# Keluaa/Armon.jl

Measured on AMD Instinct MI355X. Metric: Mcells/sec per sweep (fp64), higher is better.
Workload: dtype f64; 1 GPU; Sod 16384x16384 fp64, GAD+minmod+euler_2nd, Sequential X,Y splitting, nghost 4, 1x1 tiles of 16384x16384 cells (strong scaling); arithmetic=tuned (shared 1-ulp reciprocals + FMA; within the reference's golden tolerance), cells_per_gpu=268435456, transport=single block, device=AMD GPU gfx950 (gfx950:sramecc+:xnack-, 256 CUs), halo_exchange_downgraded=False, full=False

## Files before the change

### armon.jl_amd/_lib.py

```python
import ctypes as C
import os

_HERE = os.path.dirname(os.path.abspath(__file__))
LIB_PATH = os.environ.get("ARMON_HIP_LIB") or os.path.join(_HERE, "libarmon_hip.so")

FIELDS = ("x", "y", "rho", "u", "v", "E", "p", "c", "g", "us", "ps",
          "work_1", "work_2", "work_3", "work_4", "mask")


class SolverException(Exception):

    def __init__(self, category, msg):
        super().__init__(f"{category}: {msg}")
        self.category = category
        self.msg = msg


def solver_error(category, msg):
    raise SolverException(category, msg)


class Range(C.Structure):
    _fields_ = [("col_start", C.c_int64), ("col_step", C.c_int64), ("col_len", C.c_int64),
                ("row_start", C.c_int64), ("row_len", C.c_int64)]
# ... 41 lines not shown


class ProfileBin(C.Structure):
    _fields_ = [("n", C.c_uint64), ("n_bad", C.c_uint64), ("sum", (C.c_int64 * 3) * 5),
                ("rho_min", C.c_uint64), ("rho_max", C.c_uint64), ("p_min", C.c_uint64), ("p_max", C.c_uint64),
                ("reserved", C.c_uint64 * 3)]


class ProfileSpec(C.Structure):
    _fields_ = [("kind", C.c_int32), ("eos", C.c_int32), ("nbins", C.c_int64), ("width", C.c_int64),
                ("cx", C.c_double), ("cy", C.c_double), ("dx", C.c_double), ("dy", C.c_double), ("inv_dr", C.c_double),
                ("gamma", C.c_double), ("scale_exp", C.c_int32 * 5)]


class ExactSpec(C.Structure):
    _fields_ = [("form", C.c_int32), ("coord", C.c_int32), ("samples", C.c_int32), ("eos", C.c_int32), ("global_nx", C.c_int64),
                ("cx", C.c_double), ("cy", C.c_double), ("dx", C.c_double), ("dy", C.c_double), ("gamma", C.c_double),
                ("coord_min", C.c_double), ("coord_max", C.c_double), ("scale_exp", (C.c_int32 * 2) * 4),
                ("time", C.c_double), ("side", (C.c_double * 4) * 2), ("star", C.c_double * 4), ("speed", C.c_double * 5),
                ("g1", C.c_double), ("g2", C.c_double * 2), ("g3", C.c_double),
                ("inv_scale", C.c_double), ("M", C.c_int64), ("outer", C.c_double * 3), ("table", C.c_void_p)]


class ExactNorm(C.Structure):
    _fields_ = [("n", C.c_uint64), ("n_bad", C.c_uint64), ("sum_d", C.c_int64 * 3), ("sum_abs", C.c_int64 * 3),
                ("sum_sq", C.c_int64 * 3), ("max_abs", C.c_uint64), ("max_abs_at", C.c_uint64), ("reserved", C.c_uint64 * 3)]


class HistoryRecord(C.Structure):
    _fields_ = [("n", C.c_uint64), ("n_bad", C.c_uint64), ("sum", (C.c_int64 * 3) * 6), ("ext", (C.c_uint64 * 2) * 8),
                ("reserved", C.c_uint64 * 4)]


class HistorySpec(C.Structure):
    _fields_ = [("eos", C.c_int32), ("reserved", C.c_int32), ("gamma", C.c_double), ("global_nx", C.c_int64),
                ("scale_exp", C.c_int32 * 6)]


class DeriveSpec(C.Structure):
    _fields_ = [("nq", C.c_int32), ("quantity", C.c_int32 * 8), ("reduce", C.c_int32 * 8), ("eos", C.c_int32),
                ("neighbours", C.c_int32), ("gamma", C.c_double), ("dx", C.c_double), ("dy", C.c_double)]


class Region(C.Structure):
    _fields_ = [("kind", C.c_int32), ("reserved", C.c_int32), ("a", C.c_double * 4),
                ("rho", C.c_double), ("u", C.c_double), ("v", C.c_double), ("E", C.c_double)]


class RegionF32(C.Structure):
    _fields_ = [("kind", C.c_int32), ("reserved", C.c_int32), ("a", C.c_float * 4),
                ("rho", C.c_float), ("u", C.c_float), ("v", C.c_float), ("E", C.c_float)]


class HaloDesc(C.Structure):
    _fields_ = [("nx", C.c_int64), ("ny", C.c_int64), ("nghost", C.c_int32), ("nvars", C.c_int32),
                ("vars", C.c_void_p * 8)]


class CyclePlan(C.Structure):
    _fields_ = [("n_sweeps", C.c_int32), ("emit_p", C.c_int32), ("emit_dt", C.c_int32), ("overlap", C.c_int32),
                ("axis", C.c_int32 * 4), ("dt", C.c_double * 4), ("next_axis", C.c_int32), ("event_slot", C.c_int32),
                ("event_ctx", C.c_void_p), ("dt_host", C.c_void_p), ("dt_event_slot", C.c_int32), ("reserved", C.c_int32)]


class TileCycle(C.Structure):
    _fields_ = [("x", SweepDesc), ("y", SweepDesc)]


MGPU_ID_BYTES = 256

_lib = None

_dp, _i64, _dbl, _ci, _vp = C.c_void_p, C.c_int64, C.c_double, C.c_int, C.c_void_p
SIGNATURES = {
    "armon_hip_flt_size": (_ci, []),
    "armon_hip_idx_size": (_ci, []),
    "armon_hip_version": (C.c_char_p, []),
    "armon_hip_last_error": (C.c_char_p, []),
    "armon_hip_device_count": (_ci, [C.POINTER(_ci)]),
    "armon_hip_init": (_ci, [_ci, _vp, C.POINTER(_vp)]),
    "armon_hip_destroy": (_ci, [_vp]),
    "armon_hip_sync": (_ci, [_vp]),
    "armon_hip_device_memory_info": (_ci, [_vp, C.POINTER(C.c_size_t), C.POINTER(C.c_size_t)]),
    "armon_hip_device_name": (_ci, [_vp, C.c_char_p, C.c_size_t]),
    "armon_hip_stream": (_vp, [_vp]),
    "armon_hip_set_tuning": (_ci, [_vp, C.c_char_p, _ci]),
    "armon_hip_get_tuning": (_ci, [_vp, C.c_char_p, C.POINTER(_ci)]),
    "armon_hip_malloc": (_ci, [_vp, C.c_size_t, C.POINTER(_vp)]),
    "armon_hip_free": (_ci, [_vp, _vp]),
    "armon_hip_memcpy": (_ci, [_vp, _vp, _vp, C.c_size_t, _ci]),
    "armon_hip_memset": (_ci, [_vp, _vp, _ci, C.c_size_t]),
    "armon_hip_malloc_host": (_ci, [_vp, C.c_size_t, C.POINTER(_vp)]),
    "armon_hip_free_host": (_ci, [_vp, _vp]),
    "armon_hip_memcpy_async": (_ci, [_vp, _vp, _vp, C.c_size_t, _ci]),
    "armon_hip_event_sync": (_ci, [_vp, _ci]),
    "armon_hip_stream_copy4": (_ci, [_vp, C.POINTER(_vp * 4), C.POINTER(_vp * 4), C.c_size_t]),
    "armon_hip_timer_start": (_ci, [_vp]),
    "armon_hip_timer_stop": (_ci, [_vp, C.POINTER(_dbl)]),
    "armon_hip_event_record": (_ci, [_vp, _ci]),
    "armon_hip_event_elapsed_ms": (_ci, [_vp, _ci, _ci, C.POINTER(_dbl)]),
    "armon_hip_perfect_gas_EOS": (_ci, [_vp, Range, _dbl] + [_dp] * 7),
    "armon_hip_bizarrium_EOS": (_ci, [_vp, Range] + [_dp] * 7),
    "armon_hip_acoustic": (_ci, [_vp, Range, _i64] + [_dp] * 6),
    "armon_hip_acoustic_GAD": (_ci, [_vp, Range, _i64, _dbl, _dbl] + [_dp] * 6 + [_ci]),
    "armon_hip_cell_update": (_ci, [_vp, Range, _i64, _dbl, _dbl] + [_dp] * 5),
    "armon_hip_advection_first_order": (_ci, [_vp, Range, _i64, _dbl] + [_dp] * 9),
    "armon_hip_advection_second_order": (_ci, [_vp, Range, _i64, _dbl, _dbl] + [_dp] * 9),
    "armon_hip_euler_projection": (_ci, [_vp, Range, _i64, _dbl, _dbl] + [_dp] * 9),
    "armon_hip_boundary_conditions": (_ci, [_vp, Range, _i64, _ci, _dbl, _dbl] + [_dp] * 7),
    "armon_hip_pack_to_array": (_ci, [_vp, Range, _ci, _i64, _dp, _ci, C.POINTER(_dp)]),
    "armon_hip_unpack_from_array": (_ci, [_vp, Range, _ci, _i64, _dp, _ci, C.POINTER(_dp)]),
    "armon_hip_dtCFL_async": (_ci, [_vp, Range, _dbl, _dbl] + [_dp] * 4),
    "armon_hip_dtCFL": (_ci, [_vp, Range, _dbl, _dbl] + [_dp] * 3 + [C.POINTER(_dbl)]),
    "armon_hip_conservation_vars": (_ci, [_vp, Range, _dbl, _dp, _dp, C.POINTER(_dbl * 2)]),
    "armon_hip_init_test": (_ci, [_vp, Range, _ci, _i64, _i64, _ci, C.POINTER(_i64 * 2),
                                  C.POINTER(_i64 * 2), C.POINTER(_dbl * 2), C.POINTER(_dbl * 2),
                                  _dbl, C.POINTER(BlockDataPtrs)]),
    "armon_hip_init_regions": (_ci, [_vp, Range, _i64, _ci, C.POINTER(_i64 * 2), C.POINTER(_dbl * 2), C.POINTER(_dbl * 2), _ci,
                                     C.POINTER(_dbl * 4), _ci, C.POINTER(Region)] + [_dp] * 4),
    "armon_hip_init_regions_f32": (_ci, [_vp, Range, _i64, _ci, C.POINTER(_i64 * 2), C.POINTER(C.c_float * 2),
                                         C.POINTER(C.c_float * 2), _ci, C.POINTER(C.c_float * 4), _ci, C.POINTER(RegionF32)]
                                   + [_dp] * 4),
    "armon_hip_coarsen": (_ci, [_vp, _i64, _ci] + [_i64] * 4 + [_dp] * 6),
    "armon_hip_derive": (_ci, [_vp, _i64, _ci] + [_i64] * 4 + [_dp] * 4 + [C.POINTER(DeriveSpec), _dp]),
    "armon_hip_gather_strided": (_ci, [_vp, _i64, _ci, C.POINTER(_dp), _i64, _i64, _i64, _dp]),
    "armon_hip_state_pack": (_ci, [_vp, _i64, _ci, _i64, _i64, _ci, C.POINTER(_dp)] + [_i64] * 6 + [_dp, _dp]),
    "armon_hip_state_unpack": (_ci, [_vp, _i64, _ci, _i64, _i64, _ci, C.POINTER(_dp)] + [_i64] * 6 + [_dp, _dp]),
    "armon_hip_plane_encode_bound": (C.c_uint64, [_ci, _i64, _i64]),
    "armon_hip_plane_encode": (_ci, [_vp, _dp, _ci, _i64, _i64, _dp, C.c_uint64, _dp]),
    "armon_hip_plane_decode": (_ci, [_vp, _dp, C.c_uint64] + [_i64] * 6 + [_dp, _dp]),
    "armon_hip_state_diff_reset": (_ci, [_vp, _ci, _dp]),
    "armon_hip_state_compare": (_ci, [_vp, _i64, _ci, _i64, _i64, _ci, C.POINTER(_dp)] + [_i64] * 6 + [_dp, _dbl, _dbl, _dp, _dp]),
    "armon_hip_profile_reset": (_ci, [_vp, _i64, _dp]),
    "armon_hip_profile": (_ci, [_vp, _i64, _ci, _i64, _i64] + [_dp] * 4 + [_i64] * 6 + [C.POINTER(ProfileSpec), _dp]),
    "armon_hip_profile_bounds": (_ci, [_vp, _i64, _ci, _i64, _i64] + [_dp] * 4 + [_i64] * 6 + [C.POINTER(ProfileSpec), _dp]),
    "armon_hip_exact_norms_reset": (_ci, [_vp, _dp]),
    "armon_hip_exact_norms": (_ci, [_vp, _i64, _ci, _i64, _i64] + [_dp] * 4 + [_i64] * 6 + [C.POINTER(ExactSpec), _dp]),
    "armon_hip_exact_fill": (_ci, [_vp, _i64, _ci, _i64, _i64] + [_dp] * 4 + [_i64] * 6 + [C.POINTER(ExactSpec)]),
    "armon_hip_history_create": (_ci, [_vp, _ci, _ci, C.POINTER(_vp)]),
    "armon_hip_history_destroy": (_ci, [_vp, _vp]),
    "armon_hip_history_set_gauges": (_ci, [_vp, _vp, C.POINTER(_i64), _ci]),
    "armon_hip_history_sample": (_ci, [_vp, _vp, _ci, C.POINTER(HistorySpec), _i64, _ci, _i64, _i64] + [_dp] * 4 + [_i64] * 6),
    "armon_hip_history_read": (_ci, [_vp, _vp, _ci, _ci, _dp, _dp]),
    "armon_hip_sweep": (_ci, [_vp, C.POINTER(SweepDesc)]),
    "armon_hip_dt_state_step": (_ci, [_vp, _vp, _vp, _dbl, _dbl, _i64, _ci, _dbl]),
    "armon_hip_dt_state_step_f32": (_ci, [_vp, _vp, _vp, _dbl, _dbl, _i64, _ci, _dbl]),
    "armon_hip_graph_begin": (_ci, [_vp]),
    "armon_hip_graph_end": (_ci, [_vp, C.POINTER(_vp)]),
    "armon_hip_graph_launch": (_ci, [_vp, _vp]),
    "armon_hip_graph_destroy": (_ci, [_vp]),
    "armon_hip_tune_placement": (_ci, [_vp, C.POINTER(SweepDesc), C.POINTER(SweepDesc), C.POINTER(_vp), _ci,
                                       C.c_size_t, _ci, C.POINTER(_ci * 8), C.POINTER(_dbl)]),
    "armon_hip_cycle_xy": (_ci, [_vp, C.POINTER(SweepDesc), C.POINTER(SweepDesc)]),
    "armon_hip_choose_placement": (_ci, [_vp, C.POINTER(SweepDesc), C.POINTER(SweepDesc), C.POINTER(_vp), _ci,
                                         C.c_size_t, _ci, _dbl, C.POINTER(_ci * 8), C.POINTER(_dbl), C.POINTER(_ci)]),
    "armon_hip_mgpu_init": (_ci, [_ci, _ci, C.POINTER(_ci), C.POINTER(_vp)]),
    "armon_hip_mgpu_unique_id": (_ci, [_vp]),
    "armon_hip_mgpu_init_rank": (_ci, [_ci, _ci, _ci, _ci, _vp, _vp, C.POINTER(_vp)]),
    "armon_hip_mgpu_prepare_rank": (_ci, [_ci, _ci, _ci, _ci, _vp, C.POINTER(_vp)]),
    "armon_hip_mgpu_connect": (_ci, [_vp, _vp]),
    "armon_hip_mgpu_destroy": (_ci, [_vp]),
    "armon_hip_mgpu_set_periodic": (_ci, [_vp, _ci, _ci]),
    "armon_hip_mgpu_force_peer_copy": (_ci, [_vp, _ci]),
    "armon_hip_mgpu_set_chaos": (_ci, [_vp, C.c_uint, C.c_uint64]),
    "armon_hip_mgpu_n_local": (_ci, [_vp]),
    "armon_hip_mgpu_ctx": (_vp, [_vp, _ci]),
    "armon_hip_mgpu_tile_info": (_ci, [_vp, _ci, C.POINTER(_ci), C.POINTER(_ci * 2), C.POINTER(_ci * 4)]),
    "armon_hip_halo_exchange_start": (_ci, [_vp, _ci, C.POINTER(HaloDesc)]),
    "armon_hip_halo_exchange_finish": (_ci, [_vp, _ci, C.POINTER(HaloDesc)]),
    "armon_hip_halo_exchange": (_ci, [_vp, _ci, C.POINTER(HaloDesc)]),
    "armon_hip_dt_allreduce": (_ci, [_vp, C.POINTER(_vp)]),
    "armon_hip_mgpu_edge_ctx": (_vp, [_vp, _ci]),
    "armon_hip_mgpu_edge_dt": (_vp, [_vp, _ci]),
    "armon_hip_halo_exchange_finish_edge": (_ci, [_vp, _ci, C.POINTER(HaloDesc)]),
    "armon_hip_mgpu_edge_join": (_ci, [_vp, C.POINTER(_vp)]),
    "armon_hip_mgpu_allreduce_host": (_ci, [_vp, _ci, _ci, C.POINTER(_dbl)]),
    "armon_hip_mgpu_cycle": (_ci, [_vp, C.POINTER(CyclePlan), C.POINTER(TileCycle)]),
    "armon_hip_mgpu_drain": (_ci, [_vp, C.POINTER(TileCycle)]),
    "armon_hip_mgpu_set_threads": (_ci, [_vp, _ci]),
    "armon_hip_mgpu_sync": (_ci, [_vp]),
    "armon_hip_halo_ranges": (_ci, [_i64, _i64, _ci, _ci, C.POINTER(Range), C.POINTER(Range), C.POINTER(_i64)]),
}


def _add_f32_signatures():
    flt = C.c_float
    for name in ("perfect_gas_EOS", "bizarrium_EOS", "acoustic", "acoustic_GAD", "cell_update",
                 "advection_first_order", "advection_second_order", "euler_projection", "boundary_conditions",
                 "pack_to_array", "unpack_from_array", "dtCFL_async", "dtCFL", "conservation_vars", "init_test",
                 "coarsen", "gather_strided", "state_pack", "state_unpack", "plane_encode", "plane_decode"):
        res, args = SIGNATURES["armon_hip_" + name]
        conv = []
        for a in args:
            if a is _dbl:
                conv.append(flt)
            elif a is C.POINTER(_dbl):
                conv.append(C.POINTER(flt))
            elif a is C.POINTER(_dbl * 2):
                conv.append(C.POINTER(flt * 2))
            else:
                conv.append(a)
        SIGNATURES["armon_hip_" + name + "_f32"] = (res, conv)
    for name in ("halo_exchange_start", "halo_exchange_finish", "halo_exchange", "dt_allreduce",
                 "halo_exchange_finish_edge", "mgpu_edge_join", "mgpu_cycle", "mgpu_drain"):
        SIGNATURES["armon_hip_" + name + "_f32"] = SIGNATURES["armon_hip_" + name]
    SIGNATURES["armon_hip_sweep_f32"] = SIGNATURES["armon_hip_sweep"]
    SIGNATURES["armon_hip_state_compare_f32"] = SIGNATURES["armon_hip_state_compare"]
    SIGNATURES["armon_hip_derive_f32"] = SIGNATURES["armon_hip_derive"]
    SIGNATURES["armon_hip_profile_f32"] = SIGNATURES["armon_hip_profile"]
    SIGNATURES["armon_hip_profile_bounds_f32"] = SIGNATURES["armon_hip_profile_bounds"]
    SIGNATURES["armon_hip_exact_norms_f32"] = SIGNATURES["armon_hip_exact_norms"]
    SIGNATURES["armon_hip_exact_fill_f32"] = SIGNATURES["armon_hip_exact_fill"]
    SIGNATURES["armon_hip_history_sample_f32"] = SIGNATURES["armon_hip_history_sample"]
    SIGNATURES["armon_hip_tune_placement_f32"] = SIGNATURES["armon_hip_tune_placement"]
    SIGNATURES["armon_hip_choose_placement_f32"] = SIGNATURES["armon_hip_choose_placement"]


_add_f32_signatures()


def load_at(path):
    if not os.path.exists(path):
        raise RuntimeError(
            f"{path} is missing: build it with `python armon.jl_amd/build.py` "
            "(there is no CPU fallback for the device backend)")
    L = C.CDLL(path)
    for name, (res, args) in SIGNATURES.items():
        fn = getattr(L, name)
        fn.restype = res
        fn.argtypes = args
    if L.armon_hip_flt_size() != 8 or L.armon_hip_idx_size() != 8:
        raise RuntimeError("libarmon_hip.so: unexpected flt_size/idx_size")
    return L


def lib():
    global _lib
    if _lib is None:
        _lib = load_at(LIB_PATH)
    return _lib


ALT_LIB_PATH = os.path.join(_HERE, "libarmon_hip_alt.so")
_alt = None


class alt_kernels:

    def __enter__(self):
        global _lib, _alt
        if _alt is None:
            _alt = load_at(ALT_LIB_PATH)
        self._saved, _lib = _lib, _alt
        return _alt

    def __exit__(self, *exc):
        global _lib
        _lib = self._saved
        return False


def check(rc):
    if rc != 0:
        msg = lib().armon_hip_last_error().decode(errors="replace")
        raise SolverException("cpp" if rc != 4 else "time", f"[{rc}] {msg}")
```

### armon.jl_amd/blocking.py

```python
from dataclasses import dataclass
from enum import IntEnum

from ._lib import Range


class Axis(IntEnum):
    X = 1
    Y = 2


class Side(IntEnum):
    Left = 1
    Right = 2
    Bottom = 3
    Top = 4


def first_sides():
    return (Side.Left, Side.Bottom)


def first_side(axis):
    return Side.Left if axis == Axis.X else Side.Bottom


def last_side(axis):
    return Side.Right if axis == Axis.X else Side.Top


def sides_along(axis):
    return (first_side(axis), last_side(axis))


def axis_of(side):
    return Axis.X if side in (Side.Left, Side.Right) else Axis.Y


def opposite_of(side):
    return {Side.Left: Side.Right, Side.Right: Side.Left, Side.Bottom: Side.Top, Side.Top: Side.Bottom}[side]


@dataclass(frozen=True)
class StepRange:
    first: int
    step: int
    last: int

    def __len__(self):
        if self.step > 0:
            return max(0, (self.last - self.first) // self.step + 1)
        return max(0, (self.first - self.last) // (-self.step) + 1)

    def __iter__(self):
        return iter(range(self.first, self.last + (1 if self.step > 0 else -1), self.step))

    @property
    def stop(self):
        n = len(self)
        return self.first + (n - 1) * self.step if n else self.first - self.step

    def shift(self, n=1):
        return StepRange(self.first + self.step * n, self.step, self.last + self.step * n)

    def expand(self, n=1):
        return StepRange(self.first, self.step, self.last + self.step * n)

    def prepend(self, n=1):
        return StepRange(self.first - self.step * n, self.step, self.last)

    def inflate(self, n=1):
        return StepRange(self.first - self.step * n, self.step, self.last + self.step * n)


@dataclass(frozen=True)
class DomainRange:
    col: StepRange
    row: StepRange

    def __len__(self):
        return len(self.col) * len(self.row)

    @property
    def size(self):
        return (len(self.row), len(self.col))

    def first(self):
        return self.col.first + self.row.first - 1

    def last(self):
        return self.col.stop + self.row.stop - 1

    def __contains__(self, x):
        if not (self.first() <= x <= self.last()):
            return False
        ix = x - self.col.first + 1
        idc = ix // self.col.step
        ix -= idc * self.col.step
        return self.row.first <= ix <= self.row.stop

    def __iter__(self):
        for j in self.col:
            for i in self.row:
                yield j + i - 1

    def _along(self, axis, fname, n):
        if axis == Axis.X:
            return DomainRange(self.col, getattr(self.row, fname)(n))
        return DomainRange(getattr(self.col, fname)(n), self.row)

    def shift_dir(self, axis, n=1):
        return self._along(axis, "shift", n)

    def prepend_dir(self, axis, n=1):
        return self._along(axis, "prepend", n)

    def expand_dir(self, axis, n=1):
        return self._along(axis, "expand", n)

    def inflate_dir(self, axis, n=1):
        return self._along(axis, "inflate", n)

    def to_c(self):
        assert self.row.step == 1
        return Range(self.col.first - 1, self.col.step, len(self.col), self.row.first - 1, len(self.row))


@dataclass(frozen=True)
class BlockSize:
    size: tuple
    ghosts: int

    @property
    def real_size(self):
        return (self.size[0] - 2 * self.ghosts, self.size[1] - 2 * self.ghosts)

    @property
    def n_cells(self):
        return self.size[0] * self.size[1]

    def domain_range(self, bottom_left=(0, 0), top_right=(0, 0)):
        g, row = self.ghosts, self.size[0]
        block_start = row * (g - 1) + g

        def block_idx(I):
            return block_start + I[1] * row + I[0]

        first_I = (bottom_left[0] + 1, bottom_left[1] + 1)
        last_I = (top_right[0] + self.real_size[0], top_right[1] + self.real_size[1])
        col = StepRange(block_idx(first_I), row, block_idx(last_I))
        rowr = StepRange(1, 1, last_I[0] - first_I[0] + 1)
        return DomainRange(col, rowr)

    def position(self, i):
        iy, ix = divmod(i - 1, self.size[0])
        return (ix - self.ghosts + 1, iy - self.ghosts + 1)

    def lin_position(self, I):
        return (I[1] + self.ghosts - 1) * self.size[0] + (I[0] + self.ghosts)

    def is_ghost(self, i, o=0):
        I = self.position(i)
        rs = self.real_size
        return not all(1 - o <= I[d] <= rs[d] + o for d in range(2))

    def border_domain(self, side, single_strip=True):
        rs = self.real_size
        if side == Side.Left:
            bl, tr = (0, 0), (1 - rs[0], 0)
        elif side == Side.Right:
            bl, tr = (rs[0] - 1, 0), (0, 0)
        elif side == Side.Bottom:
            bl, tr = (0, 0), (0, 1 - rs[1])
        else:
            bl, tr = (0, rs[1] - 1), (0, 0)
        domain = self.domain_range(bl, tr)
        if single_strip:
            return domain
        if side in first_sides():
            return domain.expand_dir(axis_of(side), self.ghosts - 1)
        return domain.prepend_dir(axis_of(side), self.ghosts - 1)

    def ghost_domain(self, side, single_strip=True):
        domain = self.border_domain(side)
        domain = domain.shift_dir(axis_of(side), -self.ghosts if side in first_sides() else self.ghosts)
        if single_strip:
            return domain
        if side in first_sides():
            return domain.expand_dir(axis_of(side), self.ghosts - 1)
        return domain.prepend_dir(axis_of(side), self.ghosts - 1)

    def stride_along(self, axis):
        return 1 if axis == Axis.X else self.size[0]

    def size_along(self, axis_or_side):
        ax = axis_or_side if isinstance(axis_or_side, Axis) else axis_of(axis_or_side)
        return self.size[int(ax) - 1]

    def real_size_along(self, axis_or_side):
        ax = axis_or_side if isinstance(axis_or_side, Axis) else axis_of(axis_or_side)
        return self.real_size[int(ax) - 1]

    def real_face_size(self, axis_or_side):
        rs = self.real_size
        return (rs[0] * rs[1]) // self.real_size_along(axis_or_side)


@dataclass(frozen=True)
class StepsRanges:
    direction: Axis
    real_domain: tuple
    full_domain: tuple
    EOS: tuple
    fluxes: tuple
    cell_update: tuple
    advection: tuple
    projection: tuple


def compute_steps_ranges(axis, ghosts, projection_stencil_width):
    extra = projection_stencil_width
    real = ((0, 0), (0, 0))
    full = ((-ghosts, -ghosts), (ghosts, ghosts))
    if axis == Axis.X:
        fl = ((-extra, 0), (extra + 1, 0))
        cu = ((-extra, 0), (extra, 0))
        ad = ((0, 0), (1, 0))
    else:
        fl = ((0, -extra), (0, extra + 1))
        cu = ((0, -extra), (0, extra))
        ad = ((0, 0), (0, 1))
    return StepsRanges(axis, real, full, real, fl, cu, ad, real)
```

### armon.jl_amd/csrc/common.hpp

```cpp
#pragma once

#include <hip/hip_runtime.h>

#include <cstdarg>
#include <cstdint>
#include <cstdio>
#include <cstring>

#include "../../include/armon_hip.h"

struct armon_graph;
struct armon_ctx {
    int device = 0;
    hipStream_t stream = nullptr;
    bool owns_stream = false;
    double* partials = nullptr;
    size_t partials_cap = 0;
    double* scalars = nullptr;
    double* host_scalars = nullptr;
    hipEvent_t ev_start = nullptr, ev_stop = nullptr;
    hipEvent_t* ev_pool = nullptr;
    int n_cu = 256;
    int tune_xs_niter = 0;
    int tune_y_seg = 0;
    int tune_align = 1;
    int tune_y_cols1 = 0;
    int tune_x_xcd = -1;
    int tune_x_rows = 0;
    int tune_copy_nt = 0;
    int tune_y_sx = 0;
    int tune_profile_wgs = 0;
    int64_t seg_nx = -1, seg_ny = -1;
    int seg_lag = -1, seg_cols = -1, seg_value = 0;
    int live_graphs = 0;
    armon_graph* graphs = nullptr;
    bool capturing = false;
};

namespace armon {

void set_error(const char* fmt, ...);

inline int fail_hip(hipError_t e, const char* what)
{
    set_error("%s: %s", what, hipGetErrorString(e));
    return ARMON_ERR_HIP;
}

#define ARMON_HIP_TRY(expr)                                             \
    do {                                                                \
        hipError_t e_ = (expr);                                         \
        if (e_ != hipSuccess) return ::armon::fail_hip(e_, #expr);      \
    } while (0)

#define ARMON_REQUIRE(cond, ...)                                        \
    do {                                                                \
        if (!(cond)) {                                                  \
            ::armon::set_error(__VA_ARGS__);                            \
            return ARMON_ERR_INVALID_ARG;                               \
        }                                                               \
    } while (0)

inline int check_launch(const char* name)
{
    hipError_t e = hipGetLastError();
    if (e != hipSuccess) {
        set_error("launch of %s failed: %s", name, hipGetErrorString(e));
        return ARMON_ERR_HIP;
    }
    return ARMON_OK;
}

inline bool range_ok(const armon_range& r)
{
    return r.col_len >= 0 && r.row_len >= 0 && r.col_start + r.row_start >= 0 && r.col_step >= 0;
}
inline bool range_empty(const armon_range& r) { return r.col_len == 0 || r.row_len == 0; }

constexpr int kBlock = 256;

inline void range_grid(const armon_range& r, int cells_per_thread, dim3& grid, dim3& block)
{
    block = dim3(kBlock, 1, 1);
    int64_t per_block = (int64_t)kBlock * cells_per_thread;
    int64_t gx = (r.row_len + 15 + per_block - 1) / per_block;
    int64_t gy = r.col_len < 65535 ? r.col_len : 65535;
    grid = dim3((unsigned)gx, (unsigned)gy, 1);
}

int ensure_partials(armon_ctx* ctx, size_t n);
template <typename T>
int pack_pair(armon_ctx* ctx, const armon_range r[2], int nghost, int64_t face, T* const array[2], int nvars, T* const* vars, bool pack);
void disown_graphs(armon_ctx* ctx);

}
```

### armon.jl_amd/csrc/context.hip

```cpp
#include "common.hpp"

#include <cstdlib>

namespace armon {

static thread_local char g_error[512] = "";

void set_error(const char* fmt, ...)
{
    va_list ap;
    va_start(ap, fmt);
    vsnprintf(g_error, sizeof(g_error), fmt, ap);
    va_end(ap);
}

int ensure_partials(armon_ctx* ctx, size_t n)
{
    if (n <= ctx->partials_cap) return ARMON_OK;
    ARMON_REQUIRE(!ctx->capturing, "the reduction scratch would have to grow (%zu -> %zu doubles) inside a stream capture: "
                  "run this launch once before armon_hip_graph_begin", ctx->partials_cap, n);
    ARMON_REQUIRE(ctx->live_graphs == 0, "the reduction scratch would have to grow (%zu -> %zu doubles) while %d captured graph(s) of "
                  "this context point into it: destroy them first, or run the larger launch before capturing",
                  ctx->partials_cap, n, ctx->live_graphs);
    ARMON_HIP_TRY(hipStreamSynchronize(ctx->stream));
    if (ctx->partials) ARMON_HIP_TRY(hipFree(ctx->partials));
    ctx->partials = nullptr;
    ctx->partials_cap = 0;
    ARMON_HIP_TRY(hipMalloc((void**)&ctx->partials, n * sizeof(double)));
    ctx->partials_cap = n;
    return ARMON_OK;
}

}

using namespace armon;

extern "C" {

int armon_hip_flt_size(void) { return (int)sizeof(double); }
int armon_hip_idx_size(void) { return (int)sizeof(int64_t); }
const char* armon_hip_version(void) { return "armon_hip 0.1.0 (gfx950)"; }
const char* armon_hip_last_error(void) { return g_error; }

int armon_hip_device_count(int* count)
{
    ARMON_REQUIRE(count, "count is NULL");
    hipError_t e = hipGetDeviceCount(count);
    if (e != hipSuccess) {
        *count = 0;
        return fail_hip(e, "hipGetDeviceCount");
    }
    return ARMON_OK;
}

int armon_hip_init(int device_id, void* stream, armon_ctx** out)
{
    ARMON_REQUIRE(out, "ctx out pointer is NULL");
    *out = nullptr;
    int n = 0;
    hipError_t e = hipGetDeviceCount(&n);
    if (e != hipSuccess || n == 0) {
        set_error("no HIP device available (%s)", e != hipSuccess ? hipGetErrorString(e) : "count = 0");
        return ARMON_ERR_NO_DEVICE;
    }
    ARMON_REQUIRE(device_id >= 0 && device_id < n, "device_id %d out of range [0,%d)", device_id, n);
    ARMON_HIP_TRY(hipSetDevice(device_id));

    hipDeviceProp_t prop;
    ARMON_HIP_TRY(hipGetDeviceProperties(&prop, device_id));
    if (strncmp(prop.gcnArchName, "gfx950", 6) != 0) {
        set_error("device %d is %s; this library holds gfx950 code objects only", device_id, prop.gcnArchName);
        return ARMON_ERR_NO_DEVICE;
    }

    armon_ctx* ctx = new armon_ctx();
    ctx->device = device_id;
    ctx->n_cu = prop.multiProcessorCount;
    if (stream) {
        ctx->stream = (hipStream_t)stream;
        ctx->owns_stream = false;
    } else {
        e = hipStreamCreateWithFlags(&ctx->stream, hipStreamNonBlocking);
        if (e != hipSuccess) { delete ctx; return fail_hip(e, "hipStreamCreate"); }
        ctx->owns_stream = true;
    }
    if ((e = hipMalloc((void**)&ctx->scalars, 16 * sizeof(double))) != hipSuccess ||
        (e = hipHostMalloc((void**)&ctx->host_scalars, 16 * sizeof(double), hipHostMallocDefault)) != hipSuccess ||
        (e = hipEventCreate(&ctx->ev_start)) != hipSuccess ||
        (e = hipEventCreate(&ctx->ev_stop)) != hipSuccess) {
        armon_hip_destroy(ctx);
        return fail_hip(e, "context allocation");
    }
    int rc = ensure_partials(ctx, 8192);
    if (rc != ARMON_OK) { armon_hip_destroy(ctx); return rc; }
    for (const char* knob : {"ARMON_XS_NITER", "ARMON_Y_SEG", "ARMON_SWEEP_ALIGN", "ARMON_Y_COLS1", "ARMON_X_XCD", "ARMON_X_ROWS", "ARMON_Y_SX", "ARMON_COPY_NT"}) {
        const char* v = getenv(knob);
        if (v && *v) (void)armon_hip_set_tuning(ctx, knob, atoi(v));
    }
    *out = ctx;
    return ARMON_OK;
}

int armon_hip_set_tuning(armon_ctx* ctx, const char* knob, int value)
{
    ARMON_REQUIRE(ctx && knob, "NULL argument");
    if (!strcmp(knob, "ARMON_XS_NITER")) ctx->tune_xs_niter = value > 0 ? value : 0;
    else if (!strcmp(knob, "ARMON_Y_SEG")) ctx->tune_y_seg = value > 0 ? value : 0;
    else if (!strcmp(knob, "ARMON_SWEEP_ALIGN")) ctx->tune_align = value < 0 ? 1 : (value != 0);
    else if (!strcmp(knob, "ARMON_Y_COLS1")) ctx->tune_y_cols1 = value > 0;
    else if (!strcmp(knob, "ARMON_X_XCD")) ctx->tune_x_xcd = value < 0 ? -1 : (value > 0);
    else if (!strcmp(knob, "ARMON_X_ROWS")) ctx->tune_x_rows = (value == 1 || value == 2) ? value : 0;
    else if (!strcmp(knob, "ARMON_Y_SX")) ctx->tune_y_sx = (value == 1 || value == 2) ? value : 0;
    else if (!strcmp(knob, "ARMON_COPY_NT")) ctx->tune_copy_nt = value & 3;
    else if (!strcmp(knob, "PROFILE_WGS")) ctx->tune_profile_wgs = value > 0 ? value : 0;
    else ARMON_REQUIRE(false, "unknown tuning knob '%s'", knob);
    return ARMON_OK;
}

int armon_hip_get_tuning(armon_ctx* ctx, const char* knob, int* value)
{
    ARMON_REQUIRE(ctx && knob && value, "NULL argument");
    if (!strcmp(knob, "ARMON_XS_NITER")) *value = ctx->tune_xs_niter;
    else if (!strcmp(knob, "ARMON_Y_SEG")) *value = ctx->tune_y_seg;
    else if (!strcmp(knob, "ARMON_SWEEP_ALIGN")) *value = ctx->tune_align;
    else if (!strcmp(knob, "ARMON_Y_COLS1")) *value = ctx->tune_y_cols1;
    else if (!strcmp(knob, "ARMON_X_XCD")) *value = ctx->tune_x_xcd;
    else if (!strcmp(knob, "ARMON_X_ROWS")) *value = ctx->tune_x_rows;
    else if (!strcmp(knob, "ARMON_Y_SX")) *value = ctx->tune_y_sx;
    else if (!strcmp(knob, "ARMON_COPY_NT")) *value = ctx->tune_copy_nt;
    else if (!strcmp(knob, "PROFILE_WGS")) *value = ctx->tune_profile_wgs;
    else if (!strcmp(knob, "Y_RUN_ROWS")) *value = ctx->tune_y_seg > 0 ? ctx->tune_y_seg : ctx->seg_value;
    else ARMON_REQUIRE(false, "unknown tuning knob '%s'", knob);
    return ARMON_OK;
}

int armon_hip_destroy(armon_ctx* ctx)
{
    if (!ctx) return ARMON_OK;
    (void)hipSetDevice(ctx->device);
    if (ctx->stream) (void)hipStreamSynchronize(ctx->stream);
    disown_graphs(ctx);
    if (ctx->partials) (void)hipFree(ctx->partials);
    if (ctx->scalars) (void)hipFree(ctx->scalars);
    if (ctx->host_scalars) (void)hipHostFree(ctx->host_scalars);
    if (ctx->ev_pool) {
        for (int i = 0; i < ARMON_HIP_MAX_EVENTS; i++)
            if (ctx->ev_pool[i]) (void)hipEventDestroy(ctx->ev_pool[i]);
        delete[] ctx->ev_pool;
    }
    if (ctx->ev_start) (void)hipEventDestroy(ctx->ev_start);
    if (ctx->ev_stop) (void)hipEventDestroy(ctx->ev_stop);
    if (ctx->owns_stream && ctx->stream) (void)hipStreamDestroy(ctx->stream);
    delete ctx;
    return ARMON_OK;
}

int armon_hip_sync(armon_ctx* ctx)
{
    ARMON_REQUIRE(ctx, "ctx is NULL");
    ARMON_HIP_TRY(hipStreamSynchronize(ctx->stream));
    return ARMON_OK;
}

void* armon_hip_stream(armon_ctx* ctx) { return ctx ? (void*)ctx->stream : nullptr; }

int armon_hip_device_memory_info(armon_ctx* ctx, size_t* free_bytes, size_t* total_bytes)
{
    ARMON_REQUIRE(ctx && free_bytes && total_bytes, "NULL argument");
    ARMON_HIP_TRY(hipSetDevice(ctx->device));
    ARMON_HIP_TRY(hipMemGetInfo(free_bytes, total_bytes));
    return ARMON_OK;
}

int armon_hip_device_name(armon_ctx* ctx, char* buf, size_t buf_len)
{
    ARMON_REQUIRE(ctx && buf && buf_len > 0, "NULL argument");
    hipDeviceProp_t prop;
    ARMON_HIP_TRY(hipGetDeviceProperties(&prop, ctx->device));
    snprintf(buf, buf_len, "%s (%s, %d CUs)", prop.name[0] ? prop.name : "AMD GPU gfx950", prop.gcnArchName, prop.multiProcessorCount);
    return ARMON_OK;
}

int armon_hip_malloc(armon_ctx* ctx, size_t bytes, void** ptr)
{
    ARMON_REQUIRE(ctx && ptr, "NULL argument");
    *ptr = nullptr;
    if (bytes == 0) return ARMON_OK;
    ARMON_HIP_TRY(hipSetDevice(ctx->device));
    ARMON_HIP_TRY(hipMalloc(ptr, bytes));
    return ARMON_OK;
}

int armon_hip_free(armon_ctx* ctx, void* ptr)
{
    ARMON_REQUIRE(ctx, "ctx is NULL");
    if (!ptr) return ARMON_OK;
    ARMON_HIP_TRY(hipStreamSynchronize(ctx->stream));
    ARMON_HIP_TRY(hipFree(ptr));
    return ARMON_OK;
}

int armon_hip_memcpy(armon_ctx* ctx, void* dst, const void* src, size_t bytes, int kind)
{
    ARMON_REQUIRE(ctx, "ctx is NULL");
    if (bytes == 0) return ARMON_OK;
    ARMON_REQUIRE(dst && src, "NULL pointer in memcpy");
    hipMemcpyKind k;
    switch (kind) {
    case ARMON_MEMCPY_H2D: k = hipMemcpyHostToDevice; break;
    case ARMON_MEMCPY_D2H: k = hipMemcpyDeviceToHost; break;
    case ARMON_MEMCPY_D2D: k = hipMemcpyDeviceToDevice; break;
    default: ARMON_REQUIRE(false, "unknown memcpy kind %d", kind);
    }
    ARMON_HIP_TRY(hipMemcpyAsync(dst, src, bytes, k, ctx->stream));
    if (k != hipMemcpyDeviceToDevice) ARMON_HIP_TRY(hipStreamSynchronize(ctx->stream));
    return ARMON_OK;
}

int armon_hip_malloc_host(armon_ctx* ctx, size_t bytes, void** ptr)
{
    ARMON_REQUIRE(ctx && ptr, "NULL argument");
    *ptr = nullptr;
    if (bytes == 0) return ARMON_OK;
    ARMON_HIP_TRY(hipHostMalloc(ptr, bytes, hipHostMallocDefault));
    return ARMON_OK;
}

int armon_hip_free_host(armon_ctx* ctx, void* ptr)
{
    ARMON_REQUIRE(ctx, "ctx is NULL");
    if (ptr) ARMON_HIP_TRY(hipHostFree(ptr));
    return ARMON_OK;
}

int armon_hip_memcpy_async(armon_ctx* ctx, void* dst, const void* src, size_t bytes, int kind)
{
    ARMON_REQUIRE(ctx, "ctx is NULL");
    if (bytes == 0) return ARMON_OK;
    ARMON_REQUIRE(dst && src, "NULL pointer in memcpy_async");
    hipMemcpyKind k;
    switch (kind) {
    case ARMON_MEMCPY_H2D: k = hipMemcpyHostToDevice; break;
    case ARMON_MEMCPY_D2H: k = hipMemcpyDeviceToHost; break;
    case ARMON_MEMCPY_D2D: k = hipMemcpyDeviceToDevice; break;
    default: ARMON_REQUIRE(false, "unknown memcpy kind %d", kind);
    }
    ARMON_HIP_TRY(hipMemcpyAsync(dst, src, bytes, k, ctx->stream));
    return ARMON_OK;
}

int armon_hip_memset(armon_ctx* ctx, void* dst, int byte_value, size_t bytes)
{
    ARMON_REQUIRE(ctx, "ctx is NULL");
    if (bytes == 0) return ARMON_OK;
    ARMON_REQUIRE(dst, "NULL pointer in memset");
    ARMON_HIP_TRY(hipMemsetAsync(dst, byte_value, bytes, ctx->stream));
    return ARMON_OK;
}

}

namespace {
struct copy4_args { const double2* in[4]; double2* out[4]; };

typedef double vdouble2 __attribute__((ext_vector_type(2)));
template <int NT>
__global__ void __launch_bounds__(256) k_stream_copy4(copy4_args p, size_t n2)
{
    const size_t i = (size_t)blockIdx.x * 256 + threadIdx.x;
    if (i >= n2) return;
    vdouble2 v[4];
#pragma unroll
    for (int k = 0; k < 4; k++) {
        const vdouble2* q = reinterpret_cast<const vdouble2*>(p.in[k] + i);
        v[k] = (NT & 1) ? __builtin_nontemporal_load(q) : *q;
    }
#pragma unroll
    for (int k = 0; k < 4; k++) {
        vdouble2* q = reinterpret_cast<vdouble2*>(p.out[k] + i);
        if (NT & 2) __builtin_nontemporal_store(v[k], q);
        else *q = v[k];
// ... 79 lines not shown
```

### armon.jl_amd/csrc/fused_sweep.hpp

```cpp
#pragma once
#include "sweep_device.hpp"
#include "sweep_y_kernel.hpp"
#include "sweep_x_kernel.hpp"

namespace {

#ifdef ARMON_ALT_KERNELS
#include "fused_sweep_alt_kernels.hpp"
#endif

struct y_shape {
    int cols = 1;
    int block = kYBlock;
    bool sx = false;
};
y_shape y_launch_shape(const armon_ctx* ctx, const ARMON_SWEEP_DESC* d)
{
    y_shape s;
    if (std::is_same<real, float>::value && !d->exact && d->nx % 2 == 0 && d->nghost % 2 == 0 && d->nx >= 2 && !ctx->tune_y_cols1)
        s.cols = 2;
    if (ctx->tune_align != 0 && ctx->tune_y_sx != 2 && !d->exact) {
        const uintptr_t outs = (uintptr_t)d->rho_out | (uintptr_t)d->u_out | (uintptr_t)d->v_out | (uintptr_t)d->E_out;
        const int64_t row_len = d->nx + 2 * (int64_t)d->nghost;
        s.sx = outs % 64 == 0 && ((row_len * (int64_t)sizeof(real)) % 64 != 0 || ctx->tune_y_sx == 1);
    }
    s.block = s.sx ? kYSxBlock : kYBlock;
    return s;
}

template <class PIPE, bool TRACK>
int launch(armon_ctx* ctx, const sweep_args& a, int axis, const y_shape& ys, int64_t* n_blocks)
{
    const int64_t n_out = a.o_hi - a.o_lo;
    if (axis == ARMON_AXIS_Y) {
        const int64_t per_block = (int64_t)ys.block * ys.cols;
        dim3 grid((unsigned)((a.nx + a.xshift + per_block - 1) / per_block), (unsigned)((n_out + a.seg - 1) / a.seg));
        *n_blocks = (int64_t)grid.x * grid.y;
        if constexpr (std::is_same<real, float>::value && !PIPE::kExact) {
            if (ys.cols == 2) {
                if (ys.sx)
                    hipLaunchKernelGGL((k_sweep_y<PIPE, TRACK, kYSxBlock, true, 2>), grid, dim3(ys.block), 0, ctx->stream, a);
                else
                    hipLaunchKernelGGL((k_sweep_y<PIPE, TRACK, kYBlock, false, 2>), grid, dim3(ys.block), 0, ctx->stream, a);
                return check_launch("sweep_y2");
            }
        }
        if constexpr (!PIPE::kExact) {
            if (ys.sx) {
                hipLaunchKernelGGL((k_sweep_y<PIPE, TRACK, kYSxBlock, true>), grid, dim3(ys.block), 0, ctx->stream, a);
                return check_launch("sweep_y (store exchange)");
            }
        }
        hipLaunchKernelGGL((k_sweep_y<PIPE, TRACK>), grid, dim3(ys.block), 0, ctx->stream, a);
        return check_launch("sweep_y");
    }
#if defined(ARMON_ALT_KERNELS) && !defined(ARMON_ONLY_HEADLINE)
    if (a.x_kernel == 2) {
        dim3 grid((unsigned)((n_out + a.seg - 1) / a.seg), (unsigned)((a.ny + kXRows - 1) / kXRows));
        *n_blocks = (int64_t)grid.x * grid.y;
        const size_t lds = (size_t)(a.emit ? 6 : 4) * kXRows * (kXChunk + 1) * sizeof(real);
        hipLaunchKernelGGL((k_sweep_x_lds<PIPE, kXChunk, TRACK>), grid, dim3(kXRows), lds, ctx->stream, a);
        return check_launch("sweep_x_lds");
    }
#endif
    int niter = 1;
#if defined(ARMON_ALT_KERNELS) && !defined(ARMON_ONLY_HEADLINE)
    if (ctx->tune_xs_niter > 1) niter = ctx->tune_xs_niter;
#elif defined(ARMON_XS_MULTI)
    niter = ctx->tune_xs_niter > 0 ? ctx->tune_xs_niter : 2;
#endif
    const bool k1 = a.x_kernel == 3;
    if (a.x_kernel == 0 && a.o_hi - a.o_lo <= 8) {
        const int64_t per_block = 16 - 2 * PIPE::LAG;
        dim3 grid((unsigned)((a.o_hi - a.x_first + per_block - 1) / per_block), (unsigned)((a.ny + 4 * kXSRows - 1) / (4 * kXSRows)));
        *n_blocks = (int64_t)grid.x * grid.y * kXSRows;
        sweep_args b = a;
        b.gx = (int32_t)grid.x;
        b.gy = (int32_t)grid.y;
        hipLaunchKernelGGL((k_sweep_x_dpp<PIPE::SCHEME, PIPE::LIM, PIPE::PROJ, PIPE::EOS, PIPE::kExact, 1, TRACK, true, 1>),
                           grid, dim3(64, kXSRows), 0, ctx->stream, b, 1);
        return check_launch("sweep_x_dpp (narrow)");
    }
    const int halo = k1 ? PIPE::LAG : 4;
    const int64_t per_block = (int64_t)niter * (64 * (k1 ? 1 : 2) - 2 * halo);
    const int64_t x_lowest = a.x_row_align ? a.o_lo - (64 / (int64_t)sizeof(real) - 1) : a.x_first;
    dim3 grid((unsigned)((a.o_hi - x_lowest + per_block - 1) / per_block), (unsigned)((a.ny + kXSRows - 1) / kXSRows));
    if (a.x_wg_along_x && !k1 && niter == 1)
        grid = dim3((unsigned)((a.o_hi - x_lowest + kXSRows * per_block - 1) / (kXSRows * per_block)), (unsigned)a.ny);
    *n_blocks = (int64_t)grid.x * grid.y * kXSRows;
    sweep_args b = a;
    b.gx = (int32_t)grid.x;
    b.gy = (int32_t)grid.y;
#if defined(ARMON_ALT_KERNELS) && !defined(ARMON_ONLY_HEADLINE)
    if (k1)
        hipLaunchKernelGGL((k_sweep_x_dpp<PIPE::SCHEME, PIPE::LIM, PIPE::PROJ, PIPE::EOS, PIPE::kExact, 1, TRACK, false>),
                           grid, dim3(64, kXSRows), 0, ctx->stream, b, niter);
    else if (niter > 1)
        hipLaunchKernelGGL((k_sweep_x_dpp<PIPE::SCHEME, PIPE::LIM, PIPE::PROJ, PIPE::EOS, PIPE::kExact, 2, TRACK, false>),
                           grid, dim3(64, kXSRows), 0, ctx->stream, b, niter);
    else
#endif
#ifdef ARMON_XS_MULTI
        hipLaunchKernelGGL((k_sweep_x_dpp<PIPE::SCHEME, PIPE::LIM, PIPE::PROJ, PIPE::EOS, PIPE::kExact, 2, TRACK, false>),
                           grid, dim3(64, kXSRows), 0, ctx->stream, b, niter);
#else
        hipLaunchKernelGGL((k_sweep_x_dpp<PIPE::SCHEME, PIPE::LIM, PIPE::PROJ, PIPE::EOS, PIPE::kExact, 2, TRACK, true>),
                           grid, dim3(64, kXSRows), 0, ctx->stream, b, niter);
#endif
    return check_launch("sweep_x_dpp");
}

int y_run_length(int n_cu, int64_t nx, int64_t ny, int lag, int cols_per_lane, int block)
{
    const double slots = (double)n_cu * ARMON_Y_WAVES * 4 / (block / 64);
    const int64_t cols = (nx + 16 + (int64_t)block * cols_per_lane - 1) / ((int64_t)block * cols_per_lane);
    int best = (int)(ny < 32 ? ny : 32);
    double best_cost = 1e300;
    for (int64_t nruns = 1; nruns <= ny; nruns++) {
        const int64_t seg = (ny + nruns - 1) / nruns;
        if (seg < 32) break;
        if ((ny + seg - 1) / seg != nruns) continue;
        const double rounds = (double)(cols * nruns) / slots;
        const bool full_single_round = rounds <= 1. && rounds >= 0.93;
        if (rounds < 2. && !full_single_round) continue;
        const double cost = (full_single_round ? 1. : 0.5 * (rounds + std::ceil(rounds))) * (double)(seg + 2 * lag);
        if (cost < best_cost) {
            best_cost = cost;
            best = (int)seg;
        }
    }
    return best;
}

int64_t max_blocks(const sweep_args& a)
{
    const int64_t by = (a.nx + 16 + kYBlock - 1) / kYBlock * ((a.ny + a.seg - 1) / a.seg);
#ifdef ARMON_ALT_KERNELS
    const int64_t bx_lds = (a.nx + a.seg - 1) / a.seg * ((a.ny + kXRows - 1) / kXRows);
#else
    const int64_t bx_lds = 0;
#endif
    const int64_t bx_dpp = ((a.nx + 8) / 56 + 1 + kXSRows) * ((a.ny + kXSRows - 1) / kXSRows) * kXSRows;
    int64_t m = by > bx_lds ? by : bx_lds;
    m = m > bx_dpp ? m : bx_dpp;
    return m + kFoldBlocks;
}

template <class PIPE>
int dispatch_track(armon_ctx* ctx, const sweep_args& a, int axis, const y_shape& ys, bool track, int64_t* n_blocks)
{
    if (track) return launch<PIPE, true>(ctx, a, axis, ys, n_blocks);
    return launch<PIPE, false>(ctx, a, axis, ys, n_blocks);
}

template <int SCHEME, int LIM, int PROJ, int EOS>
int dispatch_exact(armon_ctx* ctx, const sweep_args& a, int axis, const y_shape& ys, bool exact, bool track, int64_t* nb)
{
    if (exact) return dispatch_track<fused::Pipe<SCHEME, LIM, PROJ, EOS, real>>(ctx, a, axis, ys, track, nb);
    return dispatch_track<fused::PipeFast<SCHEME, LIM, PROJ, EOS, real>>(ctx, a, axis, ys, track, nb);
}

template <int SCHEME, int LIM, int PROJ>
int dispatch_eos(armon_ctx* ctx, const sweep_args& a, int axis, const y_shape& ys, int eos, bool exact, bool track, int64_t* nb)
{
    if (eos == ARMON_EOS_BIZARRIUM)
        return dispatch_exact<SCHEME, LIM, PROJ, ARMON_EOS_BIZARRIUM>(ctx, a, axis, ys, exact, track, nb);
    return dispatch_exact<SCHEME, LIM, PROJ, ARMON_EOS_PERFECT_GAS>(ctx, a, axis, ys, exact, track, nb);
}

template <int SCHEME, int LIM>
int dispatch_proj(armon_ctx* ctx, const sweep_args& a, int axis, const y_shape& ys, int eos, int proj, bool exact, bool track, int64_t* nb)
{
    if (proj == ARMON_PROJECTION_EULER_2ND)
        return dispatch_eos<SCHEME, LIM, ARMON_PROJECTION_EULER_2ND>(ctx, a, axis, ys, eos, exact, track, nb);
    return dispatch_eos<SCHEME, LIM, ARMON_PROJECTION_EULER>(ctx, a, axis, ys, eos, exact, track, nb);
}

}

extern "C" int ARMON_SWEEP_FN(armon_ctx* ctx, const ARMON_SWEEP_DESC* d)
{
    ARMON_REQUIRE(ctx && d, "NULL argument");
    ARMON_REQUIRE(d->axis == ARMON_AXIS_X || d->axis == ARMON_AXIS_Y, "invalid axis %d", d->axis);
    ARMON_REQUIRE(d->scheme == ARMON_SCHEME_GODUNOV || d->scheme == ARMON_SCHEME_GAD, "unknown scheme %d", d->scheme);
    ARMON_REQUIRE(d->projection == ARMON_PROJECTION_EULER || d->projection == ARMON_PROJECTION_EULER_2ND,
                  "unknown projection %d", d->projection);
    ARMON_REQUIRE(d->eos == ARMON_EOS_PERFECT_GAS || d->eos == ARMON_EOS_BIZARRIUM, "unknown EOS %d", d->eos);
    ARMON_REQUIRE(d->scheme != ARMON_SCHEME_GAD || (d->limiter >= ARMON_LIMITER_NONE && d->limiter <= ARMON_LIMITER_SUPERBEE),
                  "unknown limiter tag %d", d->limiter);
    ARMON_REQUIRE(d->nx > 0 && d->ny > 0, "empty block %lld x %lld", (long long)d->nx, (long long)d->ny);
    ARMON_REQUIRE(d->ny < (1ll << 30) && d->nx < (1ll << 30), "block too large (%lld x %lld)", (long long)d->nx, (long long)d->ny);
    const int lag = (d->scheme == ARMON_SCHEME_GAD ? 1 : 0) + (d->projection == ARMON_PROJECTION_EULER_2ND ? 1 : 0) + 2;
    ARMON_REQUIRE(d->nghost >= lag, "nghost = %d but this scheme/projection reads %d cells past the block", d->nghost, lag);
    const int64_t n_axis = d->axis == ARMON_AXIS_X ? d->nx : d->ny;
    ARMON_REQUIRE(!(d->bc_low || d->bc_high) || n_axis >= lag,
                  "mirror boundary needs at least %d cells along the sweep axis", lag);
    ARMON_REQUIRE(!d->bc_low || (std::fabs(d->u_factor_low) == 1. && std::fabs(d->v_factor_low) == 1.),
                  "mirror factors of the low side must be +1 or -1 (got %g, %g)", d->u_factor_low, d->v_factor_low);
    ARMON_REQUIRE(!d->bc_high || (std::fabs(d->u_factor_high) == 1. && std::fabs(d->v_factor_high) == 1.),
                  "mirror factors of the high side must be +1 or -1 (got %g, %g)", d->u_factor_high, d->v_factor_high);
    ARMON_REQUIRE(d->rho_in && d->u_in && d->v_in && d->E_in && d->rho_out && d->u_out && d->v_out && d->E_out,
                  "NULL state array");
    ARMON_REQUIRE(d->rho_in != d->rho_out && d->u_in != d->u_out && d->v_in != d->v_out && d->E_in != d->E_out,
                  "in and out arrays must not alias (ping-pong)");
#ifdef ARMON_ALT_KERNELS
    ARMON_REQUIRE(d->x_kernel == 0 || d->x_kernel == 2 || d->x_kernel == 3, "unknown x_kernel form %d", d->x_kernel);
#else
    ARMON_REQUIRE(d->x_kernel == 0, "x_kernel form %d is a measured alternative: only libarmon_hip_alt.so (-DARMON_ALT_KERNELS) carries it",
                  d->x_kernel);
#endif
    ARMON_REQUIRE(!d->dt_state || d->x_kernel == 0 || d->x_kernel == 3,
                  "dt_state is not honoured by x_kernel form %d (only the DPP X sweeps and the Y march read it)", d->x_kernel);
    const bool exact = d->exact != 0;
    const bool track = d->dt_cfl_out != nullptr;
    ARMON_REQUIRE(!track || (d->cfl_dx > 0 && d->cfl_dy > 0), "dt_cfl_out needs cfl_dx, cfl_dy > 0");

    sweep_args a;
    a.nx = d->nx;
    a.ny = d->ny;
    a.row_len = d->nx + 2 * (int64_t)d->nghost;
    a.g = d->nghost;
    a.bc_low = d->bc_low;
    a.bc_high = d->bc_high;
    a.emit = (d->p_out ? 1 : 0) | (d->c_out ? 2 : 0);
    a.dt = (real)d->dt;
    a.dx = (real)d->dx;
    a.gamma = (real)d->gamma;
    a.inv_dx = real(1) / a.dx;
    a.dt_dx = a.dt / a.dx;
    const bool X = d->axis == ARMON_AXIS_X;
    a.fa_low = (real)(X ? d->u_factor_low : d->v_factor_low);
    a.ft_low = (real)(X ? d->v_factor_low : d->u_factor_low);
    a.fa_high = (real)(X ? d->u_factor_high : d->v_factor_high);
    a.ft_high = (real)(X ? d->v_factor_high : d->u_factor_high);
    a.rho_in = d->rho_in;
    a.ua_in = X ? d->u_in : d->v_in;
    a.ut_in = X ? d->v_in : d->u_in;
    a.E_in = d->E_in;
    a.rho_out = d->rho_out;
    a.ua_out = X ? d->u_out : d->v_out;
    a.ut_out = X ? d->v_out : d->u_out;
    a.E_out = d->E_out;
    a.p_out = d->p_out;
    a.c_out = d->c_out;
    a.st = d->dt_state;
    const bool align = ctx->tune_align != 0;
    const y_shape ys = X ? y_shape{} : y_launch_shape(ctx, d);
    a.y_sx = ys.sx;
    if (X) {
        a.seg = 512;
    } else if (ctx->tune_y_seg > 0) {
        a.seg = ctx->tune_y_seg;
    } else {
        if (ctx->seg_nx != d->nx || ctx->seg_ny != n_axis || ctx->seg_lag != lag || ctx->seg_cols != ys.cols * ys.block) {
            ctx->seg_value = y_run_length(ctx->n_cu, d->nx, n_axis, lag, ys.cols, ys.block);
            ctx->seg_cols = ys.cols * ys.block;
            ctx->seg_nx = d->nx;
            ctx->seg_ny = n_axis;
            ctx->seg_lag = lag;
        }
        a.seg = ctx->seg_value;
    }
    ARMON_REQUIRE(X || a.row_len * (int64_t)sizeof(real) * (a.seg + 2 * lag + 16) < (1ll << 32),
                  "block too wide for 32-bit row offsets (%lld cells per row, runs of %d rows)", (long long)d->nx, a.seg);
    a.x_kernel = d->x_kernel;
    a.o_lo = 0;
    a.o_hi = n_axis;
    if (d->out_hi != 0) {
        ARMON_REQUIRE(d->out_lo >= 0 && d->out_lo < d->out_hi && d->out_hi <= n_axis,
                      "invalid partial sweep [%lld, %lld) of %lld cells", (long long)d->out_lo, (long long)d->out_hi, (long long)n_axis);
        a.o_lo = d->out_lo;
        a.o_hi = d->out_hi;
    }
    a.xshift = (X || !align) ? 0 : d->nghost % 16;
    a.x_first = X ? (align ? a.o_lo - (a.o_lo + d->nghost) % 8 : a.o_lo) : 0;
    const bool want_along_x = ctx->tune_x_rows == 2 || (ctx->tune_x_rows == 0 && sizeof(real) == 4);
    const bool along_x = X && want_along_x && d->ny <= 65535 && ctx->tune_x_xcd <= 0;
    const bool eight_xcds = ctx->n_cu == 256;
    a.xcd_remap = (ctx->tune_x_xcd < 0 ? sizeof(real) == 8 : ctx->tune_x_xcd != 0) && !along_x && eight_xcds;
    a.x_row_align = 0;
#ifndef ARMON_XS_MULTI
    {
        const uintptr_t bases = (uintptr_t)d->rho_in | (uintptr_t)d->u_in | (uintptr_t)d->v_in | (uintptr_t)d->E_in |
                                (uintptr_t)d->rho_out | (uintptr_t)d->u_out | (uintptr_t)d->v_out | (uintptr_t)d->E_out |
                                (uintptr_t)d->p_out | (uintptr_t)d->c_out;
        a.x_row_align = X && align && d->x_kernel == 0 && ctx->tune_xs_niter <= 1 && a.row_len % (64 / (int64_t)sizeof(real)) != 0 &&
                        bases % 64 == 0;
    }
#endif
    a.x_wg_along_x = along_x ? 1 : 0;
    a.partials = nullptr;
    if (track) {
        int rc = ensure_partials(ctx, (size_t)(2 * max_blocks(a)));
        if (rc != ARMON_OK) return rc;
        a.partials = reinterpret_cast<real*>(ctx->partials);
    }

    int64_t n_blocks = 0;
    int rc;
#ifdef ARMON_ONLY_HEADLINE
#ifndef ARMON_ONLY_EOS
#define ARMON_ONLY_EOS ARMON_EOS_PERFECT_GAS
#endif
    ARMON_REQUIRE(d->scheme == ARMON_SCHEME_GAD && d->limiter == ARMON_LIMITER_MINMOD && d->projection == ARMON_PROJECTION_EULER_2ND &&
                  d->eos == ARMON_ONLY_EOS && d->x_kernel == 0, "headline-only variant build");
    rc = dispatch_exact<ARMON_SCHEME_GAD, ARMON_LIMITER_MINMOD, ARMON_PROJECTION_EULER_2ND, ARMON_ONLY_EOS>(ctx, a, d->axis, ys, exact, track, &n_blocks);
    if (rc != ARMON_OK || !track) return rc;
    return fold_dt_launch(ctx, a.partials, n_blocks, (real)d->cfl_dx, (real)d->cfl_dy, d->dt_cfl_out, d->dt_accumulate, d->dt_state);
#else
    if (d->scheme == ARMON_SCHEME_GODUNOV) {
        rc = dispatch_proj<ARMON_SCHEME_GODUNOV, ARMON_LIMITER_NONE>(ctx, a, d->axis, ys, d->eos, d->projection, exact, track, &n_blocks);
    } else {
        switch (d->limiter) {
        case ARMON_LIMITER_MINMOD:
            rc = dispatch_proj<ARMON_SCHEME_GAD, ARMON_LIMITER_MINMOD>(ctx, a, d->axis, ys, d->eos, d->projection, exact, track, &n_blocks);
            break;
        case ARMON_LIMITER_SUPERBEE:
            rc = dispatch_proj<ARMON_SCHEME_GAD, ARMON_LIMITER_SUPERBEE>(ctx, a, d->axis, ys, d->eos, d->projection, exact, track, &n_blocks);
            break;
        default:
            rc = dispatch_proj<ARMON_SCHEME_GAD, ARMON_LIMITER_NONE>(ctx, a, d->axis, ys, d->eos, d->projection, exact, track, &n_blocks);
        }
    }
    if (rc != ARMON_OK || !track) return rc;
    return fold_dt_launch(ctx, a.partials, n_blocks, (real)d->cfl_dx, (real)d->cfl_dy, d->dt_cfl_out, d->dt_accumulate, d->dt_state);
#endif
}

#if defined(ARMON_CYCLE_FN) && !defined(ARMON_ALT_KERNELS)
extern "C" int ARMON_CYCLE_FN(armon_ctx* ctx, const ARMON_SWEEP_DESC* x, const ARMON_SWEEP_DESC* y)
{
    ARMON_REQUIRE(ctx && x && y, "NULL argument");
    ARMON_REQUIRE(false, "the whole-cycle kernel is a measured alternative (slower than the two sweeps, DESIGN.md section 4.2): "
                         "only libarmon_hip_alt.so (-DARMON_ALT_KERNELS) carries it");
    return ARMON_ERR_INVALID_ARG;
}
#endif
#if defined(ARMON_CYCLE_FN) && defined(ARMON_ALT_KERNELS)
#include "fused_sweep_alt_cycle.hpp"
#endif
```

### armon.jl_amd/csrc/fused_sweep_f64.hip

```cpp
#define ARMON_SWEEP_REAL double
#define ARMON_SWEEP_FN armon_hip_sweep
#define ARMON_SWEEP_DESC armon_sweep_desc
#define ARMON_CYCLE_FN armon_hip_cycle_xy
#include "fused_sweep.hpp"
```

### armon.jl_amd/csrc/placement.hip

```cpp
#include "common.hpp"

#include <cstdint>
#include <utility>
#include <vector>

using namespace armon;

namespace {

template <typename real>
__global__ void __launch_bounds__(256) k_fill_uniform(real* __restrict__ p, size_t n, real value)
{
    const size_t i = (size_t)blockIdx.x * 256 + threadIdx.x;
    if (i < n) p[i] = value;
}

template <class DESC, class SWEEP, class PREPARE, class STOP>
int placement_search(armon_ctx* ctx, SWEEP sweep, const DESC* x_desc, const DESC* y_desc, void* const* pool, int n_pool,
                     int tries, int* best, double* times_ms, int* tries_done, PREPARE prepare, STOP stop)
{
    hipEvent_t e0 = nullptr, e1 = nullptr;
    auto cleanup = [&]() {
        if (e0) (void)hipEventDestroy(e0);
        if (e1) (void)hipEventDestroy(e1);
    };
#define PLACEMENT_TRY(expr) do { hipError_t e_ = (expr); if (e_ != hipSuccess) { cleanup(); return fail_hip(e_, #expr); } } while (0)
    PLACEMENT_TRY(hipEventCreate(&e0));
    PLACEMENT_TRY(hipEventCreate(&e1));
    std::vector<int> idx(n_pool);
    std::vector<double> seen;
    double best_ms = 1e300;
    uint64_t rng = 0x9E3779B97F4A7C15ull;
    int t = 0;
    for (; t < tries; t++) {
        for (int k = 0; k < n_pool; k++) idx[k] = k;
        if (t > 0)
            for (int k = 0; k < 8; k++) {
                rng ^= rng << 13; rng ^= rng >> 7; rng ^= rng << 17;
                std::swap(idx[k], idx[k + (int)(rng % (uint64_t)(n_pool - k))]);
            }
        int rc = prepare(idx.data());
        if (rc != ARMON_OK) { cleanup(); return rc; }
        DESC dx = *x_desc, dy = *y_desc;
        using ptr_t = decltype(dx.rho_out);
        auto P = [&](int role) { return static_cast<ptr_t>(pool[idx[role]]); };
        dx.rho_in = P(0); dx.u_in = P(1); dx.v_in = P(2); dx.E_in = P(3);
        dx.rho_out = P(4); dx.u_out = P(5); dx.v_out = P(6); dx.E_out = P(7);
        dy.rho_in = P(4); dy.u_in = P(5); dy.v_in = P(6); dy.E_in = P(7);
        dy.rho_out = P(0); dy.u_out = P(1); dy.v_out = P(2); dy.E_out = P(3);
        double ms_min = 1e300;
        for (int rep = 0; rep < 3; rep++) {
            PLACEMENT_TRY(hipEventRecord(e0, ctx->stream));
            rc = sweep(ctx, &dx);
            if (rc == ARMON_OK) rc = sweep(ctx, &dy);
            if (rc != ARMON_OK) { cleanup(); return rc; }
            PLACEMENT_TRY(hipEventRecord(e1, ctx->stream));
            PLACEMENT_TRY(hipEventSynchronize(e1));
            float ms = 0.f;
            PLACEMENT_TRY(hipEventElapsedTime(&ms, e0, e1));
            if (rep > 0 && ms < ms_min) ms_min = ms;
        }
        if (times_ms) times_ms[t] = ms_min;
        seen.push_back(ms_min);
        if (ms_min < best_ms) {
            best_ms = ms_min;
            for (int k = 0; k < 8; k++) best[k] = idx[k];
        }
        if (stop(seen, best_ms)) { t++; break; }
    }
#undef PLACEMENT_TRY
    if (tries_done) *tries_done = t;
    cleanup();
    return ARMON_OK;
}

template <class DESC, class SWEEP>
int tune_placement(armon_ctx* ctx, SWEEP sweep, const DESC* x_desc, const DESC* y_desc, void* const* pool, int n_pool,
                   size_t bytes, int tries, int* picks, double* times_ms)
{
    ARMON_REQUIRE(ctx && x_desc && y_desc && pool && picks, "NULL argument");
    ARMON_REQUIRE(n_pool >= 8 && tries >= 1 && bytes > 0, "need at least 8 vectors and 1 try (n_pool = %d, tries = %d)", n_pool, tries);
    for (int k = 0; k < n_pool; k++) ARMON_REQUIRE(pool[k], "pool[%d] is NULL", k);
    void* master[4] = {nullptr, nullptr, nullptr, nullptr};
    bool parked = false;
    auto cleanup = [&]() {
        if (parked) {
            for (int k = 0; k < 4; k++)
                (void)hipMemcpyAsync(pool[k], master[k], bytes, hipMemcpyDeviceToDevice, ctx->stream);
            (void)hipStreamSynchronize(ctx->stream);
        }
        for (void* m : master)
            if (m) (void)hipFree(m);
    };
#define TUNE_TRY(expr) do { hipError_t e_ = (expr); if (e_ != hipSuccess) { cleanup(); return fail_hip(e_, #expr); } } while (0)
    for (int k = 0; k < 4; k++) {
        TUNE_TRY(hipMalloc(&master[k], bytes));
        TUNE_TRY(hipMemcpyAsync(master[k], pool[k], bytes, hipMemcpyDeviceToDevice, ctx->stream));
    }
    parked = true;
    auto copy_in = [&](const int* idx, const char* what) {
        for (int k = 0; k < 4; k++) {
            hipError_t e = hipMemcpyAsync(pool[idx[k]], master[k], bytes, hipMemcpyDeviceToDevice, ctx->stream);
            if (e != hipSuccess) return fail_hip(e, what);
        }
        return (int)ARMON_OK;
    };
    int best[8] = {};
    int rc = placement_search(ctx, sweep, x_desc, y_desc, pool, n_pool, tries, best, times_ms, nullptr,
                              [&](const int* idx) { return copy_in(idx, "hipMemcpyAsync(pool[idx[k]], master[k], bytes, hipMemcpyDeviceToDevice, ctx->stream)"); },
                              [](const std::vector<double>&, double) { return false; });
    if (rc == ARMON_OK) rc = copy_in(best, "hipMemcpyAsync(pool[best[k]], master[k], bytes, hipMemcpyDeviceToDevice, ctx->stream)");
    if (rc != ARMON_OK) { cleanup(); return rc; }
    TUNE_TRY(hipStreamSynchronize(ctx->stream));
#undef TUNE_TRY
    for (int k = 0; k < 8; k++) picks[k] = best[k];
    parked = false;
    cleanup();
    return ARMON_OK;
}

template <typename real, class DESC, class SWEEP>
int choose_placement(armon_ctx* ctx, SWEEP sweep, const DESC* x_desc, const DESC* y_desc, void* const* pool, int n_pool,
                     size_t bytes, int tries, double tolerance, int* picks, double* times_ms, int* tries_done)
{
    ARMON_REQUIRE(ctx && x_desc && y_desc && pool && picks, "NULL argument");
    ARMON_REQUIRE(n_pool >= 8 && tries >= 1 && bytes >= sizeof(real), "need at least 8 vectors and 1 try (n_pool = %d, tries = %d)", n_pool, tries);
    for (int k = 0; k < n_pool; k++) ARMON_REQUIRE(pool[k], "pool[%d] is NULL", k);
    const size_t n = bytes / sizeof(real);
    const real uniform[4] = {real(1), real(0), real(0), real(2.5)};
    auto fill = [&](const int* idx) {
        for (int k = 0; k < 4; k++)
            hipLaunchKernelGGL(k_fill_uniform<real>, dim3((unsigned)((n + 255) / 256)), dim3(256), 0, ctx->stream,
                               static_cast<real*>(pool[idx[k]]), n, uniform[k]);
        return (int)ARMON_OK;
    };
    auto plateau = [&](const std::vector<double>& seen, double best_ms) {
        int near = 0;
        double worst = 0;
        for (double v : seen) {
            near += v <= best_ms * (1. + tolerance);
            worst = v > worst ? v : worst;
        }
        return tolerance > 0 && seen.size() >= 12 && near >= 2 && best_ms <= 0.93 * worst;
    };
    int best[8] = {};
    int rc = placement_search(ctx, sweep, x_desc, y_desc, pool, n_pool, tries, best, times_ms, tries_done, fill, plateau);
    if (rc != ARMON_OK) return rc;
    for (int k = 0; k < 8; k++) picks[k] = best[k];
    return ARMON_OK;
}

}

extern "C" int armon_hip_tune_placement(armon_ctx* ctx, const armon_sweep_desc* x_desc, const armon_sweep_desc* y_desc,
                                        void* const* pool, int n_pool, size_t bytes, int tries, int* picks, double* times_ms)
{
    return tune_placement(ctx, armon_hip_sweep, x_desc, y_desc, pool, n_pool, bytes, tries, picks, times_ms);
}

extern "C" int armon_hip_tune_placement_f32(armon_ctx* ctx, const armon_sweep_desc_f32* x_desc, const armon_sweep_desc_f32* y_desc,
                                            void* const* pool, int n_pool, size_t bytes, int tries, int* picks, double* times_ms)
{
    return tune_placement(ctx, armon_hip_sweep_f32, x_desc, y_desc, pool, n_pool, bytes, tries, picks, times_ms);
}

extern "C" int armon_hip_choose_placement(armon_ctx* ctx, const armon_sweep_desc* x_desc, const armon_sweep_desc* y_desc,
                                          void* const* pool, int n_pool, size_t bytes, int tries, double tolerance, int* picks,
                                          double* times_ms, int* tries_done)
{
    return choose_placement<double>(ctx, armon_hip_sweep, x_desc, y_desc, pool, n_pool, bytes, tries, tolerance, picks, times_ms,
                                    tries_done);
}

extern "C" int armon_hip_choose_placement_f32(armon_ctx* ctx, const armon_sweep_desc_f32* x_desc, const armon_sweep_desc_f32* y_desc,
                                              void* const* pool, int n_pool, size_t bytes, int tries, double tolerance, int* picks,
                                              double* times_ms, int* tries_done)
{
    return choose_placement<float>(ctx, armon_hip_sweep_f32, x_desc, y_desc, pool, n_pool, bytes, tries, tolerance, picks,
                                   times_ms, tries_done);
}
```

### armon.jl_amd/csrc/sweep_device.hpp

```cpp
#pragma once
#include "common.hpp"
#include "dt_state.hpp"
#include "reduce.hpp"
#include "sweep_pipeline.hpp"
#include "sweep_spatial.hpp"

#include <cmath>
#include <cstdint>
#include <cstdlib>
#include <type_traits>
#include <utility>

using namespace armon;

#ifndef ARMON_SWEEP_REAL
#error "include through fused_sweep_f64.hip / fused_sweep_f32.hip"
#endif

namespace {

using real = ARMON_SWEEP_REAL;
using vec2 = std::conditional<std::is_same<real, double>::value, double2, float2>::type;

#ifdef ARMON_NT
#define ARMON_NT_X ARMON_NT
#define ARMON_NT_Y ARMON_NT
#endif
#ifndef ARMON_NT_X
#define ARMON_NT_X 3
#endif
#ifndef ARMON_NT_Y
#define ARMON_NT_Y 2
#endif
typedef real vreal2 __attribute__((ext_vector_type(2)));
template <bool NT = false>
__device__ __forceinline__ vec2 ld2(const real* p)
{
    const vreal2* q = reinterpret_cast<const vreal2*>(p);
    const vreal2 v = NT ? __builtin_nontemporal_load(q) : *q;
    return vec2{v.x, v.y};
}
constexpr bool x_nt_loads(int eos, bool exact)
{
    return (ARMON_NT_X & 1) && sizeof(real) == 8 && eos == ARMON_EOS_PERFECT_GAS && !exact;
}
__device__ __forceinline__ void st2(real* p, real x, real y)
{
    vreal2* q = reinterpret_cast<vreal2*>(p);
    const vreal2 v = {x, y};
    if (ARMON_NT_X & 2) __builtin_nontemporal_store(v, q);
    else *q = v;
}

struct sweep_args {
    int64_t nx, ny, row_len;
    int32_t g;
    int32_t bc_low, bc_high;
    int32_t emit;
    int32_t seg;
    int32_t x_kernel;
    int64_t o_lo, o_hi;
    int64_t x_first;
    int32_t xshift;
    int32_t xcd_remap;
    int32_t gx = 0, gy = 0;
    int32_t x_wg_along_x = 0;
    int32_t x_row_align = 0;
    int32_t y_sx = 0;
    armon_dt_state* st = nullptr;
    real dt, dx, gamma;
    real inv_dx, dt_dx;
    real fa_low, ft_low, fa_high, ft_high;
    const real *rho_in, *ua_in, *ut_in, *E_in;
    real *rho_out, *ua_out, *ut_out, *E_out;
    real *p_out, *c_out;
    real* partials;
    int32_t bc_low_t = 0, bc_high_t = 0;
    real tu_low = 1, tv_low = 1, tu_high = 1, tv_high = 1;
};

__device__ __forceinline__ int64_t bc_source(const sweep_args& a, int64_t n, int64_t j, real& fa, real& ft)
{
    fa = 1;
    ft = 1;
    if (j < 0 && a.bc_low) {
        fa = a.fa_low;
        ft = a.ft_low;
        return -1 - j;
    }
    if (j >= n && a.bc_high) {
        fa = a.fa_high;
        ft = a.ft_high;
        return 2 * n - 1 - j;
    }
    return j;
}

__device__ __forceinline__ bool sweep_begin(sweep_args& a)
{
    if (a.st) {
        const auto* st = (const __attribute__((address_space(4))) armon_dt_state*)a.st;
        if (st->done) return false;
        a.dt = (real)st->current_dt * a.dt;
        a.dt_dx = a.dt / a.dx;
        if (!st->emit_p) a.emit &= ~1;
    }
    return true;
}

template <int... Is, class F>
__device__ __forceinline__ void static_for(std::integer_sequence<int, Is...>, F&& f)
{
    (f(std::integral_constant<int, Is>{}), ...);
}

typedef unsigned int v2u __attribute__((ext_vector_type(2)));
using rsrc_t = __amdgpu_buffer_rsrc_t;

__device__ __forceinline__ rsrc_t make_rsrc(const void* p)
{
    return __builtin_amdgcn_make_buffer_rsrc(const_cast<void*>(p), 0, 0xFFFFFFFFu, 0x00020000);
}
#ifndef ARMON_Y_AUX_LD
#define ARMON_Y_AUX_LD ((ARMON_NT_Y & 1) ? 2 : 0)
#endif
#ifndef ARMON_Y_AUX_ST
#define ARMON_Y_AUX_ST ((ARMON_NT_Y & 2) ? 2 : 0)
#endif
constexpr int kAuxLoad = ARMON_Y_AUX_LD, kAuxStore = ARMON_Y_AUX_ST;
template <typename T> __device__ __forceinline__ T buf_load(rsrc_t r, unsigned voff, unsigned soff);
template <>
__device__ __forceinline__ double buf_load<double>(rsrc_t r, unsigned voff, unsigned soff)
{
    const v2u v = __builtin_amdgcn_raw_buffer_load_b64(r, voff, soff, kAuxLoad);
    return __builtin_bit_cast(double, v);
}
template <>
__device__ __forceinline__ float buf_load<float>(rsrc_t r, unsigned voff, unsigned soff)
{
    return __builtin_bit_cast(float, __builtin_amdgcn_raw_buffer_load_b32(r, voff, soff, kAuxLoad));
}
__device__ __forceinline__ float2 buf_load2(rsrc_t r, unsigned voff, unsigned soff)
{
    typedef float v2f __attribute__((ext_vector_type(2)));
    const v2f v = __builtin_bit_cast(v2f, __builtin_amdgcn_raw_buffer_load_b64(r, voff, soff, kAuxLoad));
    return float2{v.x, v.y};
}
__device__ __forceinline__ void buf_store2(rsrc_t r, unsigned voff, unsigned soff, float x, float y)
{
    const v2u v = {__builtin_bit_cast(unsigned int, x), __builtin_bit_cast(unsigned int, y)};
    __builtin_amdgcn_raw_buffer_store_b64(v, r, voff, soff, kAuxStore);
}
__device__ __forceinline__ void buf_store(rsrc_t r, unsigned voff, unsigned soff, double x)
{
    __builtin_amdgcn_raw_buffer_store_b64(__builtin_bit_cast(v2u, x), r, voff, soff, kAuxStore);
}
__device__ __forceinline__ void buf_store(rsrc_t r, unsigned voff, unsigned soff, float x)
{
    __builtin_amdgcn_raw_buffer_store_b32(__builtin_bit_cast(unsigned int, x), r, voff, soff, kAuxStore);
}

struct cfl_track {
    real au = 0, av = 0;
    __device__ __forceinline__ void add(real u, real v, real c)
    {
#ifdef ARMON_CFL_PLAIN_MAX
        au = phys::mx(au, phys::abs_(phys::mx(phys::abs_(u + c), phys::abs_(u - c))));
        av = phys::mx(av, phys::abs_(phys::mx(phys::abs_(v + c), phys::abs_(v - c))));
#else
#ifdef ARMON_CFL_TWO_SUMS
        au = phys::amax(au, phys::abs_(phys::mx(phys::abs_(u + c), phys::abs_(u - c))));
        av = phys::amax(av, phys::abs_(phys::mx(phys::abs_(v + c), phys::abs_(v - c))));
#else
        au = phys::amax(au, phys::abs_(u) + phys::abs_(c));
        av = phys::amax(av, phys::abs_(v) + phys::abs_(c));
#endif
#endif
    }
};

template <int NWAVES>
__device__ __forceinline__ void cfl_block_store(const cfl_track& t, real* partials, int64_t block, int tid)
{
    __shared__ real lds[NWAVES];
    const real au = red::block_reduce<red::op_max, NWAVES>(t.au, lds, tid);
    const real av = red::block_reduce<red::op_max, NWAVES>(t.av, lds, tid);
    if (tid == 0) {
        partials[2 * block] = au;
        partials[2 * block + 1] = av;
    }
}

constexpr int kFoldBlocks = 512;

__global__ void __launch_bounds__(256)
k_fold_pairs(const real* __restrict__ partials, int64_t n, real* __restrict__ out)
{
    __shared__ real lds[4];
    real au = 0, av = 0;
    for (int64_t k = (int64_t)blockIdx.x * blockDim.x + threadIdx.x; k < n; k += (int64_t)gridDim.x * blockDim.x) {
        const vec2 v = ld2(partials + 2 * k);
        au = phys::amax(au, v.x);
        av = phys::amax(av, v.y);
    }
    au = red::block_reduce<red::op_max, 4>(au, lds, threadIdx.x);
    av = red::block_reduce<red::op_max, 4>(av, lds, threadIdx.x);
    if (threadIdx.x == 0) {
        out[2 * blockIdx.x] = au;
        out[2 * blockIdx.x + 1] = av;
    }
}

__global__ void __launch_bounds__(256)
k_fold_dt(const real* __restrict__ partials, int64_t n_blocks, real dx, real dy, real* __restrict__ out,
          int accumulate, armon_dt_state* st = nullptr)
{
    if (st && st->done) return;
    __shared__ real lds[4];
    real au = 0, av = 0;
    for (int64_t k = threadIdx.x; k < n_blocks; k += blockDim.x) {
        au = phys::amax(au, partials[2 * k]);
        av = phys::amax(av, partials[2 * k + 1]);
    }
    au = red::block_reduce<red::op_max, 4>(au, lds, threadIdx.x);
    av = red::block_reduce<red::op_max, 4>(av, lds, threadIdx.x);
    if (threadIdx.x == 0) {
        const real dt = phys::mn_nan(dx / au, dy / av);
        out[0] = accumulate ? phys::mn_nan(out[0], dt) : dt;
        if (st && st->auto_step && !accumulate)
            dt_state_step<real>(st, dt, (real)st->cfl, (real)st->maxtime, st->maxcycle, st->cst_dt, (real)st->Dt);
    }
}

int fold_dt_launch(armon_ctx* ctx, real* partials, int64_t n, real dx, real dy, real* out, int accumulate,
                   armon_dt_state* st = nullptr)
{
    if (n > 16384) {
        real* level1 = partials + 2 * n;
        hipLaunchKernelGGL(k_fold_pairs, dim3(kFoldBlocks), dim3(256), 0, ctx->stream, partials, n, level1);
        int rc = check_launch("fold_pairs");
        if (rc != ARMON_OK) return rc;
        partials = level1;
        n = kFoldBlocks;
    }
    hipLaunchKernelGGL(k_fold_dt, dim3(1), dim3(256), 0, ctx->stream, partials, n, dx, dy, out, accumulate, st);
    return check_launch("fold_dt");
}

}
```

### armon.jl_amd/csrc/sweep_x_kernel.hpp

```cpp
#pragma once
#include "sweep_device.hpp"

namespace {

#ifndef ARMON_XS_ROWS
#define ARMON_XS_ROWS 4
#endif
constexpr int kXSRows = ARMON_XS_ROWS;
#ifndef ARMON_X_PRIO
#define ARMON_X_PRIO 3
#endif
constexpr int kXSNiter = 1;
template <int SCHEME, int LIM, int PROJ, int EOS, bool EXACT, int K, bool TRACK, bool SINGLE, int ROW = 0>
__device__ __forceinline__ void sweep_x_dpp_body(const sweep_args& a, int niter)
{
    using SW = fused::SpatialSweep<SCHEME, LIM, PROJ, EOS, EXACT, K, real, ROW>;
    using St = fused::Strip<K, real>;
    constexpr int LAG = SW::LAG;
    static_assert(ROW == 0 || K == 1, "the narrow form holds one cell per lane");
    constexpr int HALO = (K == 1) ? LAG : 4;
    static_assert(LAG <= 4, "strip halo");
    constexpr int WIDTH = ROW ? 16 : 64 * K;
    constexpr int STRIDE = WIDTH - 2 * HALO;
    constexpr int RW = ROW ? 4 : 1;

    const int lane = ROW ? (threadIdx.x & 15) : threadIdx.x;
    unsigned vbx = blockIdx.x, vby = blockIdx.y;
    if (a.xcd_remap) {
        const unsigned G = (unsigned)a.gx, chunk = vby & ~7u;
        if (chunk + 8 <= (unsigned)a.gy) {
            const unsigned local = (vby - chunk) * G + vbx;
            vby = chunk + (local & 7u);
            vbx = local >> 3;
        }
    }
    const bool along_x = SINGLE && ROW == 0 && a.x_wg_along_x;
    const int64_t strip0 = along_x ? (int64_t)vbx * kXSRows + threadIdx.y : (int64_t)vbx * niter;
    const int64_t row_r = along_x ? (int64_t)vby
                                  : ((int64_t)vby * kXSRows + threadIdx.y) * RW + (ROW ? (threadIdx.x >> 4) : 0);
    const bool row_ok = row_r < a.ny;
    const int64_t row = row_ok ? row_r : a.ny - 1;
    const int64_t row_off = (row + a.g) * a.row_len + a.g;
    const real* in[4] = {a.rho_in + row_off, a.ua_in + row_off, a.ut_in + row_off, a.E_in + row_off};
    real* out[4] = {a.rho_out + row_off, a.ua_out + row_off, a.ut_out + row_off, a.E_out + row_off};
    bool vec_ok = (K == 2) && (a.row_len % 2 == 0) && ((a.x_first + a.g) % 2 == 0);
    int64_t x_first = a.x_first;
    if (ROW == 0 && a.x_row_align) {
        x_first = a.o_lo - __builtin_amdgcn_readfirstlane((int)(row_off + a.o_lo) & (64 / (int)sizeof(real) - 1));
        vec_ok = (K == 2);
    }

    SW sw{a.dt, a.dx, a.gamma, a.inv_dx, a.dt_dx};
    cfl_track cfl;
    const int64_t w_first = x_first + strip0 * STRIDE;
    St buf[2][4];
    auto load_strip = [&](auto slot, int it) {
        constexpr int B = decltype(slot)::value;
        St& rho = buf[B][0];
        St& ua = buf[B][1];
        St& ut = buf[B][2];
        St& E = buf[B][3];
        const int64_t cb = w_first + (int64_t)it * STRIDE - HALO;
        const int64_t j0 = cb + (int64_t)lane * K;
        const bool interior = cb >= 0 && cb + WIDTH <= a.nx;
        if (interior && (K == 1 || vec_ok)) {
            if (K == 2) {
                constexpr bool NT = x_nt_loads(EOS, EXACT);
                const vec2 r = ld2<NT>(in[0] + j0);
                const vec2 u = ld2<NT>(in[1] + j0);
                const vec2 v = ld2<NT>(in[2] + j0);
                const vec2 e = ld2<NT>(in[3] + j0);
                rho.v[0] = r.x; rho.v[K - 1] = r.y;
                ua.v[0] = u.x; ua.v[K - 1] = u.y;
                ut.v[0] = v.x; ut.v[K - 1] = v.y;
                E.v[0] = e.x; E.v[K - 1] = e.y;
            } else {
                rho.v[0] = in[0][j0]; ua.v[0] = in[1][j0]; ut.v[0] = in[2][j0]; E.v[0] = in[3][j0];
            }
        } else {
#pragma unroll
            for (int k = 0; k < K; k++) {
                int64_t j = j0 + k;
                j = j < -(int64_t)a.g ? -(int64_t)a.g : (j > a.nx + a.g - 1 ? a.nx + a.g - 1 : j);
                real fa, ft;
                const int64_t src = bc_source(a, a.nx, j, fa, ft);
                rho.v[k] = in[0][src];
                ua.v[k] = in[1][src] * fa;
                ut.v[k] = in[2][src] * ft;
                E.v[k] = in[3][src];
            }
        }
    };
    auto strip_exists = [&](int it) { return it < niter && w_first + (int64_t)it * STRIDE < a.o_hi; };
    auto do_strip = [&](auto slot, int it) {
        constexpr int B = decltype(slot)::value;
        if (!SINGLE && strip_exists(it + 1)) load_strip(std::integral_constant<int, 1 - B>{}, it + 1);
        const int64_t w0 = w_first + (int64_t)it * STRIDE;
        const int64_t j0 = w0 - HALO + (int64_t)lane * K;

        St o_rho, o_u, o_v, o_E, p, cs;
#ifdef ARMON_PROBE_NOCOMPUTE
        o_rho = buf[B][0]; o_u = buf[B][1]; o_v = buf[B][2]; o_E = buf[B][3]; p = buf[B][0]; cs = buf[B][0];
#else
        sw.run(buf[B][0], buf[B][1], buf[B][2], buf[B][3], o_rho, o_u, o_v, o_E, p, cs);
#endif

        const int64_t hi = (w0 + STRIDE < a.o_hi) ? w0 + STRIDE : a.o_hi;
        const int64_t lo = w0 > a.o_lo ? w0 : a.o_lo;
        if (K == 2 && vec_ok && j0 >= lo && j0 + 1 < hi) {
            st2(out[0] + j0, o_rho.v[0], o_rho.v[K - 1]);
            st2(out[1] + j0, o_u.v[0], o_u.v[K - 1]);
            st2(out[2] + j0, o_v.v[0], o_v.v[K - 1]);
            st2(out[3] + j0, o_E.v[0], o_E.v[K - 1]);
            if (a.emit) {
                if (a.emit & 1) st2(a.p_out + row_off + j0, p.v[0], p.v[K - 1]);
                if (a.emit & 2) st2(a.c_out + row_off + j0, cs.v[0], cs.v[K - 1]);
            }
            if (TRACK) {
                cfl.add(o_u.v[0], o_v.v[0], cs.v[0]);
                cfl.add(o_u.v[K - 1], o_v.v[K - 1], cs.v[K - 1]);
            }
        } else {
#pragma unroll
            for (int k = 0; k < K; k++) {
                const int64_t j = j0 + k;
                if (j >= lo && j < hi) {
                    out[0][j] = o_rho.v[k];
                    out[1][j] = o_u.v[k];
                    out[2][j] = o_v.v[k];
                    out[3][j] = o_E.v[k];
                    if (a.emit & 1) (a.p_out + row_off)[j] = p.v[k];
                    if (a.emit & 2) (a.c_out + row_off)[j] = cs.v[k];
                    if (TRACK) cfl.add(o_u.v[k], o_v.v[k], cs.v[k]);
                }
            }
        }
    };
    if (SINGLE) {
        if (row_ok && strip_exists(0)) {
            load_strip(std::integral_constant<int, 0>{}, 0);
#if ARMON_X_PRIO
            __builtin_amdgcn_s_setprio(0);
#endif
            do_strip(std::integral_constant<int, 0>{}, 0);
        }
    } else if (row_ok && strip_exists(0)) {
        load_strip(std::integral_constant<int, 0>{}, 0);
#if ARMON_X_PRIO
        __builtin_amdgcn_s_setprio(0);
#endif
        for (int it = 0; strip_exists(it); it += 2) {
            do_strip(std::integral_constant<int, 0>{}, it);
            if (!strip_exists(it + 1)) break;
            do_strip(std::integral_constant<int, 1>{}, it + 1);
        }
    }
    if (TRACK) {
        const real au = red::wave_reduce<red::op_max>(cfl.au), av = red::wave_reduce<red::op_max>(cfl.av);
        if (threadIdx.x == 0) {
            const int64_t wave_id = ((int64_t)blockIdx.y * a.gx + blockIdx.x) * kXSRows + threadIdx.y;
            st2(a.partials + 2 * wave_id, au, av);
        }
    }
}

#ifndef ARMON_XS_WAVES
#define ARMON_XS_WAVES 1
#endif
#ifndef ARMON_X_PRELOAD
#define ARMON_X_PRELOAD 1
#endif
__device__ __forceinline__ void preload_x_args(const sweep_args& a, int niter)
{
#if ARMON_X_PRELOAD
    asm volatile("" ::"s"(a.nx), "s"(a.ny), "s"(a.row_len), "s"(a.g), "s"(a.bc_low), "s"(a.bc_high), "s"(a.emit), "s"(a.o_lo),
                 "s"(a.o_hi), "s"(a.x_first), "s"(a.xcd_remap), "s"(a.x_wg_along_x), "s"(a.x_row_align), "s"(niter), "s"(a.gx), "s"(a.gy));
    asm volatile("" ::"s"(a.dt), "s"(a.dx), "s"(a.gamma), "s"(a.inv_dx), "s"(a.dt_dx), "s"(a.rho_in), "s"(a.ua_in), "s"(a.ut_in),
                 "s"(a.E_in), "s"(a.rho_out), "s"(a.ua_out), "s"(a.ut_out), "s"(a.E_out));
#endif
}

template <int SCHEME, int LIM, int PROJ, int EOS, bool EXACT, int K, bool TRACK, bool SINGLE = true, int ROW = 0>
__global__ void __launch_bounds__(64 * kXSRows, ARMON_XS_WAVES)
k_sweep_x_dpp(sweep_args a, int niter)
{
#if ARMON_X_PRIO
    __builtin_amdgcn_s_setprio(ARMON_X_PRIO);
#endif
    preload_x_args(a, niter);
    if (!sweep_begin(a)) return;
    sweep_x_dpp_body<SCHEME, LIM, PROJ, EOS, EXACT, K, TRACK, SINGLE, ROW>(a, niter);
}

}
```

### armon.jl_amd/csrc/sweep_y_kernel.hpp

```cpp
#pragma once
#include "sweep_device.hpp"

namespace {

#ifndef ARMON_Y_BLOCK
#define ARMON_Y_BLOCK 256
#endif
constexpr int kYBlock = ARMON_Y_BLOCK;
constexpr int kYSxBlock = 512;
#ifndef ARMON_Y_PF
#define ARMON_Y_PF 4
#endif
#ifndef ARMON_Y_PRIO
#define ARMON_Y_PRIO 0
#endif
#ifndef ARMON_Y_WAVES
#define ARMON_Y_WAVES 2
#endif

template <int COLS, class PIPE> struct y_lane;
template <class PIPE> struct y_lane<1, PIPE> {
    using V = real;
    using pipe_t = PIPE;
    using lds_t = real;
    static __device__ __forceinline__ V load(rsrc_t r, unsigned voff, unsigned soff) { return buf_load<real>(r, voff, soff); }
    static __device__ __forceinline__ void store(rsrc_t r, unsigned voff, unsigned soff, V v) { buf_store(r, voff, soff, v); }
    static __device__ __forceinline__ void track(cfl_track& t, const V& u, const V& v, const V& c) { t.add(u, v, c); }
};
template <class PIPE> struct y_lane<2, PIPE> {
    using V = fused::fast::float2v;
    using pipe_t = fused::PipeFast<PIPE::SCHEME, PIPE::LIM, PIPE::PROJ, PIPE::EOS, V>;
    using lds_t = float2;
    static __device__ __forceinline__ void store(rsrc_t r, unsigned voff, unsigned soff, V v) { buf_store2(r, voff, soff, v.x, v.y); }
    static __device__ __forceinline__ void store(rsrc_t r, unsigned voff, unsigned soff, float2 q) { buf_store2(r, voff, soff, q.x, q.y); }
    static __device__ __forceinline__ void track(cfl_track& t, const V& u, const V& v, const V& c)
    {
        t.add(u.x, v.x, c.x);
        t.add(u.y, v.y, c.y);
    }
};

template <class PIPE, bool TRACK, int BLOCK = kYBlock, bool SX = false, int COLS = 1>
__global__ void __launch_bounds__(BLOCK, ARMON_Y_WAVES)
k_sweep_y(sweep_args a)
{
    if (!sweep_begin(a)) return;
    using lane_t = y_lane<COLS, PIPE>;
    using V = typename lane_t::V;
    constexpr int LAG = PIPE::LAG;
    constexpr int PF = ARMON_Y_PF;
    const int nx = (int)a.nx, ny = (int)a.ny, g = a.g;
    const int xr = (int)(blockIdx.x * BLOCK + threadIdx.x) * COLS - a.xshift;
    const bool active = xr >= 0 && xr < nx;
    const int x = active ? xr : (xr < 0 ? 0 : nx - COLS);
    const int o_hi = (int)a.o_hi;
    const int o0 = (int)a.o_lo + (int)blockIdx.y * a.seg;
    const int o1 = (o0 + a.seg < o_hi) ? o0 + a.seg : o_hi;
    const int jb = o0 - LAG, je = o1 + LAG;

    const unsigned colb = (unsigned)(x + g) * (unsigned)sizeof(real);
    const unsigned pitchb = (unsigned)a.row_len * (unsigned)sizeof(real);
    const int64_t in_base = (int64_t)(jb + g) * a.row_len, out_base = (int64_t)(o0 + g) * a.row_len;
    const rsrc_t r_rho = make_rsrc(a.rho_in + in_base), r_ua = make_rsrc(a.ua_in + in_base);
    const rsrc_t r_ut = make_rsrc(a.ut_in + in_base), r_E = make_rsrc(a.E_in + in_base);
    const rsrc_t w_rho = make_rsrc(a.rho_out + out_base), w_ua = make_rsrc(a.ua_out + out_base);
    const rsrc_t w_ut = make_rsrc(a.ut_out + out_base), w_E = make_rsrc(a.E_out + out_base);

    typename lane_t::pipe_t pipe(a.dt, a.dx, a.gamma, a.inv_dx, a.dt_dx);
    cfl_track cfl;

    int lj = jb;
    unsigned lo_off = 0;
    unsigned so_off = (unsigned)(jb - LAG - o0) * pitchb;

    __shared__ typename lane_t::lds_t sx_lds[SX ? 2 : 1][SX ? 4 : 1][SX ? BLOCK : 1];
    static_assert((BLOCK & (BLOCK - 1)) == 0, "the store exchange wraps columns with a mask");
    constexpr int kSec = 64 / (COLS * (int)sizeof(real));
    const int c0 = (int)(blockIdx.x * BLOCK) * COLS - a.xshift;
    int sx_r = (int)((((int64_t)(jb - LAG + g) * a.row_len + g + c0) >> (COLS - 1)) & (kSec - 1));
    const int sx_dr = (int)((a.row_len >> (COLS - 1)) & (kSec - 1));
    int sx_buf = 0;

    auto load = [&](auto slot, auto checked) {
        constexpr int K = decltype(slot)::value & 7;
        constexpr bool CHECKED = decltype(checked)::value;
        auto& dst = pipe.c[K];
        if constexpr (COLS == 2) {
            auto vec = [](float2 q) { return V{q.x, q.y}; };
            auto put = [&](unsigned off, real fa, real ft) {
                dst.rho = vec(buf_load2(r_rho, colb, off));
                dst.ua = vec(buf_load2(r_ua, colb, off)) * fa;
                dst.ut = vec(buf_load2(r_ut, colb, off)) * ft;
                dst.E = vec(buf_load2(r_E, colb, off));
            };
            if (CHECKED) {
                const bool m_lo = lj < 0 && a.bc_low, m_hi = lj >= ny && a.bc_high;
                const int src = m_lo ? -1 - lj : (m_hi ? 2 * ny - 1 - lj : lj);
                const unsigned off = (unsigned)(src - jb) * pitchb;
                const real fa = m_lo ? a.fa_low : (m_hi ? a.fa_high : real(1));
                const real ft = m_lo ? a.ft_low : (m_hi ? a.ft_high : real(1));
                put(off, fa, ft);
                if (lj + 1 < je) {
                    lj++;
                    lo_off += pitchb;
                }
            } else {
                dst.rho = vec(buf_load2(r_rho, colb, lo_off));
                dst.ua = vec(buf_load2(r_ua, colb, lo_off));
                dst.ut = vec(buf_load2(r_ut, colb, lo_off));
                dst.E = vec(buf_load2(r_E, colb, lo_off));
                lj++;
                lo_off += pitchb;
            }
        } else {
            if (CHECKED) {
                const bool m_lo = lj < 0 && a.bc_low, m_hi = lj >= ny && a.bc_high;
                const int src = m_lo ? -1 - lj : (m_hi ? 2 * ny - 1 - lj : lj);
                const unsigned off = (unsigned)(src - jb) * pitchb;
                const real fa = m_lo ? a.fa_low : (m_hi ? a.fa_high : real(1));
                const real ft = m_lo ? a.ft_low : (m_hi ? a.ft_high : real(1));
                dst.rho = lane_t::load(r_rho, colb, off);
                dst.ua = lane_t::load(r_ua, colb, off) * fa;
                dst.ut = lane_t::load(r_ut, colb, off) * ft;
                dst.E = lane_t::load(r_E, colb, off);
                if (lj + 1 < je) {
                    lj++;
                    lo_off += pitchb;
                }
            } else {
                dst.rho = lane_t::load(r_rho, colb, lo_off);
                dst.ua = lane_t::load(r_ua, colb, lo_off);
                dst.ut = lane_t::load(r_ut, colb, lo_off);
                dst.E = lane_t::load(r_E, colb, lo_off);
                lj++;
                lo_off += pitchb;
            }
        }
    };
    using std::integral_constant;
    auto step = [&](auto ph, auto checked, int j) {
        constexpr int PH8 = decltype(ph)::value;
        constexpr bool CHECKED = decltype(checked)::value;
#if ARMON_Y_PRIO
        __builtin_amdgcn_s_setprio(ARMON_Y_PRIO);
#endif
        load(integral_constant<int, PH8 + PF>{}, checked);
#if ARMON_Y_PRIO
        __builtin_amdgcn_s_setprio(0);
#endif
        V p, c, c_lag;
#ifdef ARMON_PROBE_NOCOMPUTE
        p = c = c_lag = V(real(0));
        const auto& cc = pipe.c[PH8 & 7];
        const fused::Out4<V> out{cc.rho, cc.ua, cc.ut, cc.E};
#else
        const fused::Out4<V> out = pipe.template advance<true, PH8>(p, c, c_lag);
#endif
        const int o = j - LAG;
        if (CHECKED) {
            if (a.emit && j >= o0 && j < o1 && active) {
                const unsigned off = so_off + LAG * pitchb;
                if (a.emit & 1) lane_t::store(make_rsrc(a.p_out + out_base), colb, off, p);
                if (a.emit & 2) lane_t::store(make_rsrc(a.c_out + out_base), colb, off, c);
            }
        }
        if (!CHECKED || (o >= o0 && o < o1)) {
            if constexpr (SX) {
                auto& L = sx_lds[sx_buf];
                if constexpr (COLS == 2) {
                    L[0][threadIdx.x] = float2{out.rho.x, out.rho.y};
                    L[1][threadIdx.x] = float2{out.ua.x, out.ua.y};
                    L[2][threadIdx.x] = float2{out.ut.x, out.ut.y};
                    L[3][threadIdx.x] = float2{out.E.x, out.E.y};
                } else {
                    L[0][threadIdx.x] = out.rho;
                    L[1][threadIdx.x] = out.ua;
                    L[2][threadIdx.x] = out.ut;
                    L[3][threadIdx.x] = out.E;
                }
                __syncthreads();
                const int ci = ((int)threadIdx.x - sx_r) & (BLOCK - 1);
                const int cx = c0 + COLS * ci;
                if (cx >= 0 && cx < nx) {
                    const unsigned cb = (unsigned)(cx + g) * (unsigned)sizeof(real);
                    if constexpr (COLS == 2) {
                        const float2 q0 = L[0][ci], q1 = L[1][ci], q2 = L[2][ci], q3 = L[3][ci];
                        lane_t::store(w_rho, cb, so_off, q0);
                        lane_t::store(w_ua, cb, so_off, q1);
                        lane_t::store(w_ut, cb, so_off, q2);
                        lane_t::store(w_E, cb, so_off, q3);
                    } else {
                        lane_t::store(w_rho, cb, so_off, L[0][ci]);
                        lane_t::store(w_ua, cb, so_off, L[1][ci]);
                        lane_t::store(w_ut, cb, so_off, L[2][ci]);
                        lane_t::store(w_E, cb, so_off, L[3][ci]);
                    }
                }
                sx_buf ^= 1;
            } else if (active) {
                lane_t::store(w_rho, colb, so_off, out.rho);
                lane_t::store(w_ua, colb, so_off, out.ua);
                lane_t::store(w_ut, colb, so_off, out.ut);
                lane_t::store(w_E, colb, so_off, out.E);
            }
            if (TRACK) lane_t::track(cfl, out.ut, out.ua, c_lag);
        }
        so_off += pitchb;
        sx_r = (sx_r + sx_dr) & (kSec - 1);
    };
    auto run = [&](auto checked, int t0, int t1) {
        for (int t = t0; t < t1; t += 8)
            static_for(std::make_integer_sequence<int, 8>{}, [&](auto ph) { step(ph, checked, jb + t + decltype(ph)::value); });
    };

    const int T = je - jb;
    const int T8 = (T + 7) & ~7;
    const int P = (2 * LAG + 7) & ~7;
    const int plain_end = (a.bc_high && ny < je ? ny : je) - jb - PF;
    int M = (T < plain_end ? T : plain_end) & ~7;
    if (M < P || (a.emit & 3)) M = P;

    const bool wave_idle = COLS == 1 && !SX && (int)(blockIdx.x * BLOCK + (threadIdx.x & ~63u)) - a.xshift >= nx;
    if (!wave_idle) {
        static_for(std::make_integer_sequence<int, PF>{}, [&](auto k) { load(k, std::true_type{}); });
        run(std::true_type{}, 0, P < T8 ? P : T8);
        run(std::false_type{}, P, M);
        run(std::true_type{}, M, T8);
    }

    if (TRACK) cfl_block_store<BLOCK / 64>(cfl, a.partials, (int64_t)blockIdx.y * gridDim.x + blockIdx.x, threadIdx.x);
}

}
```

### armon.jl_amd/device.py

```python
import ctypes as C

import numpy as np

from . import _lib
from ._lib import check


class HIPDevice:

    def __init__(self, device_id=0, stream=None):
        L = _lib.lib()
        ctx = C.c_void_p()
        check(L.armon_hip_init(int(device_id), C.c_void_p(stream) if stream else None, C.byref(ctx)))
        self._L = L
        self.ctx = ctx
        self.device_id = int(device_id)
        self.owns_ctx = True

    @classmethod
    def adopt(cls, ctx, device_id=0):
        d = cls.__new__(cls)
        d._L = _lib.lib()
        d.ctx = ctx if isinstance(ctx, C.c_void_p) else C.c_void_p(ctx)
        d.device_id = int(device_id)
        d.owns_ctx = False
        return d

    def close(self):
        if self.ctx:
            if self.owns_ctx:
                self._L.armon_hip_destroy(self.ctx)
            self.ctx = None

    def __del__(self):
        try:
            self.close()
        except Exception:
            pass

    def wait(self):
        check(self._L.armon_hip_sync(self.ctx))

    def memory_info(self):
        free, total = C.c_size_t(), C.c_size_t()
        check(self._L.armon_hip_device_memory_info(self.ctx, C.byref(free), C.byref(total)))
        return free.value, total.value

    @property
    def name(self):
        buf = C.create_string_buffer(256)
        check(self._L.armon_hip_device_name(self.ctx, buf, 256))
        return buf.value.decode()

    @property
    def stream(self):
        return self._L.armon_hip_stream(self.ctx)

    def timer_start(self):
        check(self._L.armon_hip_timer_start(self.ctx))

    def timer_stop(self):
        ms = C.c_double()
        check(self._L.armon_hip_timer_stop(self.ctx, C.byref(ms)))
        return ms.value

    def stream_copy4(self, src, dst, nbytes):
        a = (C.c_void_p * 4)(*[x.ptr for x in src])
        b = (C.c_void_p * 4)(*[x.ptr for x in dst])
        check(self._L.armon_hip_stream_copy4(self.ctx, C.byref(a), C.byref(b), int(nbytes)))

    def event_sync(self, slot):
        check(self._L.armon_hip_event_sync(self.ctx, int(slot)))

    def get_tuning(self, knob):
        v = C.c_int()
        check(self._L.armon_hip_get_tuning(self.ctx, knob.encode(), C.byref(v)))
        return v.value

    def y_run_rows(self):
        return self.get_tuning("Y_RUN_ROWS")

    def pinned(self, n, dtype=np.float64):
        return PinnedArray(self, n, dtype)

    def event_record(self, slot):
        check(self._L.armon_hip_event_record(self.ctx, int(slot)))

    def event_elapsed_ms(self, a, b):
        ms = C.c_double()
        check(self._L.armon_hip_event_elapsed_ms(self.ctx, int(a), int(b), C.byref(ms)))
        return ms.value

    def empty(self, n, dtype=np.float64):
        return DeviceArray(self, n, dtype)

    def zeros(self, n, dtype=np.float64):
        a = DeviceArray(self, n, dtype)
        a.fill_bytes(0)
        return a

    def from_host(self, host):
        host = np.ascontiguousarray(host)
        a = DeviceArray(self, host.size, host.dtype)
        a.copy_from_host(host)
        return a


class DeviceArray:

    def __init__(self, device, n, dtype=np.float64):
        self.device = device
        self.n = int(n)
        self.dtype = np.dtype(dtype)
        self.nbytes = self.n * self.dtype.itemsize
        p = C.c_void_p()
        check(device._L.armon_hip_malloc(device.ctx, self.nbytes, C.byref(p)))
        self.ptr = p.value or 0

    @classmethod
    def view(cls, owner, byte_offset, n, dtype):
        a = cls.__new__(cls)
        a.device, a.n, a.dtype = owner.device, int(n), np.dtype(dtype)
        a.nbytes = a.n * a.dtype.itemsize
        assert byte_offset % 256 == 0 and byte_offset + a.nbytes <= owner.nbytes
        a.ptr = owner.ptr + byte_offset
        a.owner = owner
        return a

    def __len__(self):
        return self.n

    @property
    def __cuda_array_interface__(self):
        return {"shape": (self.n,), "typestr": self.dtype.str, "data": (self.ptr, False), "version": 2}

    def free(self):
        if getattr(self, "owner", None) is not None:
            self.ptr, self.owner = 0, None
            return
        if self.ptr and self.device.ctx:
            self.device._L.armon_hip_free(self.device.ctx, C.c_void_p(self.ptr))
        self.ptr = 0

    def __del__(self):
        try:
            self.free()
        except Exception:
            pass

    def fill_bytes(self, byte):
        check(self.device._L.armon_hip_memset(self.device.ctx, C.c_void_p(self.ptr), byte, self.nbytes))

    def copy_from_host(self, host):
        host = np.ascontiguousarray(host, dtype=self.dtype)
        assert host.size == self.n, (host.size, self.n)
        check(self.device._L.armon_hip_memcpy(self.device.ctx, C.c_void_p(self.ptr),
                                              host.ctypes.data_as(C.c_void_p), self.nbytes,
                                              _lib_kind("H2D")))

    def to_host(self, out=None):
        if out is None:
            out = np.empty(self.n, dtype=self.dtype)
        assert out.size == self.n and out.dtype == self.dtype and out.flags["C_CONTIGUOUS"]
        check(self.device._L.armon_hip_memcpy(self.device.ctx, out.ctypes.data_as(C.c_void_p),
                                              C.c_void_p(self.ptr), self.nbytes, _lib_kind("D2H")))
        return out

    def copy_from_device(self, other):
        assert other.nbytes == self.nbytes
        check(self.device._L.armon_hip_memcpy(self.device.ctx, C.c_void_p(self.ptr),
                                              C.c_void_p(other.ptr), self.nbytes, _lib_kind("D2D")))


def _lib_kind(k):
    return {"H2D": 1, "D2H": 2, "D2D": 3}[k]


class PinnedArray:

    def __init__(self, device, n, dtype=np.float64):
        self.device, self.dtype = device, np.dtype(dtype)
        self.nbytes = int(n) * self.dtype.itemsize
        p = C.c_void_p()
        check(device._L.armon_hip_malloc_host(device.ctx, self.nbytes, C.byref(p)))
        self.ptr = p.value
        self.array = np.frombuffer((C.c_char * self.nbytes).from_address(self.ptr), dtype=self.dtype)

    def copy_from_device_async(self, src, n=None, dst_offset=0, src_offset=0):
        n = len(src) - src_offset if n is None else n
        sz = self.dtype.itemsize
        check(self.device._L.armon_hip_memcpy_async(self.device.ctx, C.c_void_p(self.ptr + dst_offset * sz),
                                                    C.c_void_p(src.ptr + src_offset * sz), n * sz, _lib_kind("D2H")))

    def copy_to_device_async(self, dst, n=None, src_offset=0, dst_offset=0):
        n = len(dst) - dst_offset if n is None else n
        sz = self.dtype.itemsize
        check(self.device._L.armon_hip_memcpy_async(self.device.ctx, C.c_void_p(dst.ptr + dst_offset * sz),
                                                    C.c_void_p(self.ptr + src_offset * sz), n * sz, _lib_kind("H2D")))

    def free(self):
        if self.ptr and self.device.ctx:
            self.array = None
            self.device._L.armon_hip_free_host(self.device.ctx, C.c_void_p(self.ptr))
        self.ptr = 0

    def __del__(self):
        try:
            self.free()
        except Exception:
            pass
```

### armon.jl_amd/solver.py

```python
import ctypes as C
import math
import time as _time
from dataclasses import dataclass, field

import numpy as np

from . import _lib
from ._lib import BlockDataPtrs, FIELDS, SweepDesc, check, solver_error
from .blocking import Axis, Side, first_side, last_side, sides_along
from .parameters import LIMITERS, PROC_NULL, PROJECTIONS, SCHEMES

MAIN_VARS = ("x", "y", "rho", "u", "v", "E", "p", "c", "g", "us", "ps")
SAVED_VARS = ("x", "y", "rho", "u", "v", "p")
COMM_VARS = ("rho", "u", "v", "E", "p", "c", "g")
STATE_VARS = ("rho", "u", "v", "E")


@dataclass
class SolverStats:
    final_time: float
    last_dt: float
    cycles: int
    solve_time: float
    cell_count: int
    giga_cells_per_sec: float
    data: object = None
    timer: object = None
    grid_log: object = None
    state_diffs: list = field(default_factory=list)
    profiles: list = field(default_factory=list)
    error_norms: list = field(default_factory=list)
    history: object = None
    images: list = field(default_factory=list)

    def __str__(self):
        return (f"Solver stats:\n - final time:  {self.final_time}\n - last Δt:     {self.last_dt}\n"
                f" - cycles:      {self.cycles}\n - performance: {self.giga_cells_per_sec} ×10⁹ cell-cycles/sec "
                f"({self.solve_time} sec, {self.cell_count} cells)")


class GlobalTimeStep:

    def __init__(self, params):
        self.params = params
        self.reset()

    def reset(self):
        p = self.params
        T = p.T
        self.cycle = 0
        self.time = T(0.)
        self.current_dt = T(p.Dt) if p.cst_dt else T(0.)
        self.next_cycle_dt = T(math.inf)

    def update_dt(self, new_dt):
        p = self.params
        T = p.T
        new_dt = T(new_dt)
        previous_dt = self.current_dt
        if not math.isfinite(new_dt) or new_dt <= 0:
            solver_error("time", f"Invalid time step for cycle {self.cycle}: {new_dt}")
        elif previous_dt == 0:
            new_dt = T(p.cfl) * new_dt
        else:
            new_dt = T(min(float(T(p.cfl) * new_dt), 1.05 * float(previous_dt)))
        self.next_cycle_dt = new_dt
        if self.current_dt == 0:
            self.current_dt = self.next_cycle_dt

    def next_cycle(self):
        p = self.params
        T = p.T
        self.cycle += 1
        self.time = T(self.time + self.current_dt)
        if p.cst_dt:
            self.current_dt = self.next_cycle_dt = T(p.Dt)
            return
        self.current_dt = self.next_cycle_dt
        self.next_cycle_dt = T(math.inf)


def split_axes(splitting, cycle):
    even = cycle % 2 == 0
    if splitting == "Sequential":
        return ((Axis.X, 1.0), (Axis.Y, 1.0))
    if splitting in ("Godunov", "SequentialSym"):
        return ((Axis.X, 1.0), (Axis.Y, 1.0)) if even else ((Axis.Y, 1.0), (Axis.X, 1.0))
    if splitting == "Strang":
        return (((Axis.X, 0.5), (Axis.Y, 1.0), (Axis.X, 0.5)) if even
                else ((Axis.Y, 0.5), (Axis.X, 1.0), (Axis.Y, 0.5)))
    if splitting == "X_only":
        return ((Axis.X, 1.0),)
    if splitting == "Y_only":
        return ((Axis.Y, 1.0),)
    solver_error("config", f"Unknown splitting method: '{splitting}'")


FUSED_FIELDS = ("x", "y", "rho", "u", "v", "E", "p")


class _Fields(dict):

    def __init__(self, grid, names):
        super().__init__()
        import weakref
        self._grid_ref = weakref.ref(grid)
        for f in names:
            self[f] = grid.params.device.empty(grid.size.n_cells, grid.params.data_type)

    def __missing__(self, key):
        if key not in FIELDS:
            raise KeyError(key)
        grid = self._grid_ref()
        a = grid.params.device.zeros(grid.size.n_cells, grid.params.data_type)
        if key == "mask" and grid.initialised:
            g = grid.size.ghosts
            nx, ny = grid.size.real_size
            m = np.zeros((ny + 2 * g, nx + 2 * g), dtype=grid.params.data_type)
            m[g:g + ny, g:g + nx] = 1
            a.copy_from_host(m.ravel())
        self[key] = a
        grid.lazy.add(key)
        return a


class BlockGrid:

    def __init__(self, params):
        self.params = params
        self.size = params.block_size
        dev = params.device
        n = self.size.n_cells
        dt_ = params.data_type
        self.initialised = False
        self.lazy = set()
        self.data = _Fields(self, FUSED_FIELDS if params.use_fused_sweep else FIELDS)
        self.alt = {f: dev.empty(n, dt_) for f in STATE_VARS} if params.use_fused_sweep else None
        self.placement = None
        self.global_dt = GlobalTimeStep(params)
        self.dt_scalar = dev.zeros(2, dt_)
        self.dt = DtReadback(params)
        self.dt_inflight = self.dt.inflight
        self.comm = None
        self.halo_prefetch = None
        self._coarse_xy = {}
        self.state_diffs = []
        self.profiles = []
        self.error_norms_taken = []
        self.history = None
        self.images = []

    def ptr(self, name):
        return C.c_void_p(self.data[name].ptr)

    def block_data_ptrs(self):
        bd = BlockDataPtrs()
        for f in FIELDS:
            if f in self.data:
                setattr(bd, f, self.data[f].ptr)
        return bd

    def release_scratch(self, names=("c", "g")):
        for f in names:
            if f in self.lazy and f in self.data:
                self.params.wait()
                self.data.pop(f).free()
                self.lazy.discard(f)

    def swap_state(self):
        for f in STATE_VARS:
            self.data[f], self.alt[f] = self.alt[f], self.data[f]

    def tune_placement(self, min_bytes=None, spare=None, keep_state=True):
        params, dev = self.params, self.params.device
        tries = params.placement_tries
        nbytes = self.data["rho"].nbytes
        if min_bytes is None:
            min_bytes = params.placement_min_bytes
        if spare is None:
            spare = 8
        if self.alt is None or tries <= 1 or nbytes < min_bytes:
            return None
        free, _total = dev.memory_info()
        spare = int(min(spare, (free * 0.8) // max(nbytes, 1) - (4 if keep_state else 0)))
        if spare < 1:
            return None
        dx = params.cell_size(0)
        dt = 1e-3 * dx
        n, dt_ = self.data["rho"].n, self.data["rho"].dtype
        pool = [self.data[f] for f in STATE_VARS] + [self.alt[f] for f in STATE_VARS]
        try:
            for _ in range(spare):
                pool.append(dev.empty(n, dt_))
        except _lib.SolverException:
            for v in pool[8:]:
                v.free()
            return None
        d_x = sweep_desc(params, self, Axis.X, dt, dx)
        d_y = sweep_desc(params, self, Axis.Y, dt, params.cell_size(1), emit_dt=True)
        rounds = max(1, params.placement_rounds) if not keep_state else 1
        fast_frac = 0.88 if np.dtype(params.data_type).itemsize == 4 else 0.93
        fast_ms = 2 * 8 * nbytes / (fast_frac * 6.29e12) * 1e3
        losers, all_times, report_rounds = [], [], 0
        best = pool[:8]
        while True:
            report_rounds += 1
            ptrs = (C.c_void_p * len(pool))(*[v.ptr for v in pool])
            picks, times, done = (C.c_int * 8)(), (C.c_double * tries)(), C.c_int(tries)
            try:
                if keep_state:
                    check(params.fn("tune_placement")(dev.ctx, C.byref(d_x), C.byref(d_y), ptrs, len(pool), nbytes, tries,
                                                      C.byref(picks), times))
                else:
                    check(params.fn("choose_placement")(dev.ctx, C.byref(d_x), C.byref(d_y), ptrs, len(pool), nbytes,
                                                        tries, 0.004, C.byref(picks), times, C.byref(done)))
            except _lib.SolverException:
                for k, f in enumerate(STATE_VARS):
                    self.data[f], self.alt[f] = best[k], best[4 + k]
                for v in pool[8:] + losers:
                    v.free()
                return None
            picks, times = list(picks), list(times)[:done.value]
            all_times.append([round(t, 3) for t in times])
            best = [pool[k] for k in picks]
            losers += [v for i, v in enumerate(pool) if i not in set(picks)]
            if min(times) <= fast_ms or report_rounds >= rounds:
                break
            free, _total = dev.memory_info()
            if free < (spare + 2) * nbytes:
                break
            try:
                pool = best + [dev.empty(n, dt_) for _ in range(spare)]
            except _lib.SolverException:
                break
        for k, f in enumerate(STATE_VARS):
            self.data[f], self.alt[f] = best[k], best[4 + k]
        for v in losers:
            v.free()
        flat = [t for r in all_times for t in r]
        self.placement = {"tries": len(flat), "max_tries": tries, "pool": 8 + spare, "rounds": report_rounds,
                          "x_plus_y_ms": all_times[0] if report_rounds == 1 else all_times,
                          "chosen_ms": round(min(all_times[-1]), 3), "fast_level_ms": round(fast_ms, 3),
                          "transient_GB": round((report_rounds * spare + (4 if keep_state else 0)) * nbytes / 1e9, 2)}
        return self.placement

    def device_to_host(self, names=MAIN_VARS):
        self.params.wait()
        return {f: self.data[f].to_host() for f in names}

    def gather(self, names, start, stride, count):
        params, dev = self.params, self.params.device
        names = tuple(names)
        out = dev.empty(max(len(names) * count, 1), params.data_type)
        try:
            vars_ = (C.c_void_p * len(names))(*[self.ptr(f) for f in names])
            check(params.fn("gather_strided")(dev.ctx, self.size.n_cells, len(names), vars_, int(start), int(stride),
                                              int(count), C.c_void_p(out.ptr)))
            host = out.to_host()[:len(names) * count].reshape(len(names), count)
        finally:
            out.free()
        return {f: host[k] for k, f in enumerate(names)}

    def coarse_coordinates(self, factor):
        from .parameters import coarse_shape
        if factor not in self._coarse_xy:
            fx, fy = factor
            nx, ny = self.size.real_size
            g, pitch = self.size.ghosts, self.size.size[0]
            cnx, cny = coarse_shape((nx, ny), factor)
            first = g * pitch + g
            xs = self.gather(("x",), first, min(fx, nx), cnx)["x"]
            ys = self.gather(("y",), first, min(fy, ny) * pitch, cny)["y"]
            x, y = np.broadcast_to(xs[None, :], (cny, cnx)).copy(), np.broadcast_to(ys[:, None], (cny, cnx)).copy()
            x.flags.writeable = y.flags.writeable = False
            self._coarse_xy[factor] = (x, y)
        return self._coarse_xy[factor]

    def coarsen(self, factor, with_p=True):
        from .parameters import coarse_shape, normalize_coarsen_factor
        params, dev = self.params, self.params.device
        factor = normalize_coarsen_factor(factor)
        if factor is None:
            solver_error("config", "coarsen needs a factor >= 1")
        fx, fy = factor
        nx, ny = self.size.real_size
        cnx, cny = coarse_shape((nx, ny), factor)
        names = STATE_VARS + (("p",) if with_p else ())
        out = dev.empty(len(names) * cnx * cny, params.data_type)
        try:
            check(params.fn("coarsen")(dev.ctx, self.size.size[0], self.size.ghosts, nx, ny, fx, fy,
                                       *[self.ptr(f) for f in STATE_VARS], self.ptr("p") if with_p else None,
                                       C.c_void_p(out.ptr)))
            planes = out.to_host().reshape(len(names), cny, cnx)
        finally:
            out.free()
        res = {f: planes[k] for k, f in enumerate(names)}
        res["x"], res["y"] = self.coarse_coordinates(factor)
        return res

    def state_digest(self, names=STATE_VARS):
        from . import checkpoint
        return checkpoint.state_digest([(self.params, self)], tuple(names))

    def save_state(self, path, band_rows=None, compress=None):
        from . import checkpoint
        return checkpoint.save([(self.params, self)], self.global_dt, self.dt, path, band_rows=band_rows, compress=compress)

    def load_state(self, path, band_rows=None):
        from . import checkpoint
        return checkpoint.load([(self.params, self)], self.global_dt, self.dt, path, band_rows=band_rows)

    def host_to_device(self, host):
        for f, a in host.items():
            self.data[f].copy_from_host(a)
        if "x" in host or "y" in host:
            self._coarse_xy.clear()

    def compare_state(self, ref, rtol=None, atol=0.0, names=None, limit=20, band_rows=None):
        from . import compare
        return compare.compare_state([(self.params, self)], ref, rtol=rtol, atol=atol, names=names, limit=limit, band_rows=band_rows)

    def profile(self, kind, bins=None, width=1, centre=None, dr=None, with_p=True, scale_exp=None):
        from . import profile
        self.params.wait()
        return profile.profile_state([(self.params, self)], kind, bins=bins, width=width, centre=centre, dr=dr, with_p=with_p,
                                     scale_exp=scale_exp)

    def derive(self, quantities, factor=1, reduce="mean"):
        from . import derived
        from .parameters import normalize_coarsen_factor
        self.params.wait()
        res = derived.derive_state([(self.params, self)], quantities, factor=factor, reduce=reduce, neighbours=[0])
        res["x"], res["y"] = self.coarse_coordinates(normalize_coarsen_factor(factor))
        return res

    def error_norms(self, reference=None, time=None, samples=1, coord_range=None, window=None, scale_exp=None):
        from . import analytic
        self.params.wait()
        return analytic.error_norms_state([(self.params, self)], reference, time=time, samples=samples, coord_range=coord_range,
                                          windows=None if window is None else [tuple(window)], scale_exp=scale_exp)

    def fill_exact(self, reference=None, time=None, samples=1, coord_range=None, window=None):
        from . import analytic
        self.params.wait()
        return analytic.fill_state([(self.params, self)], reference, time=time, samples=samples, coord_range=coord_range,
                                   windows=None if window is None else [tuple(window)])

    def history_sample(self, gauges=(), scale_exp=None):
        from . import history
        self.params.wait()
        return history.sample_state([(self.params, self)], gauges=gauges, scale_exp=scale_exp)

    def real_view(self, a):
        g = self.size.ghosts
        nx, ny = self.size.real_size
        return a.reshape(self.size.size[1], self.size.size[0])[g:g + ny, g:g + nx]

    def memory_required(self):
        n = self.size.n_cells * np.dtype(self.params.data_type).itemsize
        return n * (len(self.data) + (4 if self.alt else 0))



class _KernelSection:
    __slots__ = ("cbs", "name")

    def __init__(self, params, name):
        self.cbs = params.kernel_callbacks
        self.name = name

    def __enter__(self):
        for cb in self.cbs:
            cb.start(self.name)

    def __exit__(self, *exc):
        for cb in self.cbs:
            cb.end(self.name)
        return False


def _k(params, name):
    return _KernelSection(params, name)


def _range(params, corners):
    return params.block_size.domain_range(*corners).to_c()


def init_test(params, grid, tune=True):
    if tune and grid.placement is None:
        if params.use_fused_sweep:
            grid.tune_placement(keep_state=False)
        else:
            tune_staged_placement(params, grid)
    _init_test_kernel(params, grid)
    grid.initialised = True


def tune_staged_placement(params, grid, min_bytes=None):
    import random
    tries = params.placement_tries
    nbytes = grid.data["rho"].nbytes
    if min_bytes is None:
        min_bytes = params.placement_min_bytes
    if tries <= 1 or nbytes < min_bytes or params.use_MPI or any(n != PROC_NULL for n in params.neighbours.values()):
        return None
    dev = params.device
    vectors = [grid.data[f] for f in FIELDS]
    free, _total = dev.memory_info()
    try:
        n_spare = int(min(8, (free * 0.5) // max(nbytes, 1)))
        vectors += [dev.empty(vectors[0].n, vectors[0].dtype) for _ in range(max(n_spare, 0))]
    except _lib.SolverException:
        pass
    tries = min(12, params.placement_tries)
    rng = random.Random(0x5EED)
    dx = params.cell_size(0)
    dt = params.T(0.2) * dx
    times, perms = [], []
    callbacks, params.kernel_callbacks = params.kernel_callbacks, []
    for t in range(tries):
        perm = list(range(len(FIELDS))) if t == 0 else rng.sample(range(len(vectors)), len(FIELDS))
        for f, k in zip(FIELDS, perm):
            grid.data[f] = vectors[k]
        _init_test_kernel(params, grid)
        update_EOS(params, grid)
        dev.event_record(1002)
        for axis in (Axis.X, Axis.Y):
            update_EOS(params, grid, axis)
            block_ghost_exchange(params, grid, axis)
            numerical_fluxes(params, grid, axis, dt, params.cell_size(int(axis) - 1))
            cell_update(params, grid, axis, dt, params.cell_size(int(axis) - 1))
            projection_remap(params, grid, axis, dt, params.cell_size(int(axis) - 1))
        dev.event_record(1003)
        times.append(dev.event_elapsed_ms(1002, 1003))
        perms.append(perm)
    params.kernel_callbacks = callbacks
    k = times.index(min(times))
    for f, i in zip(FIELDS, perms[k]):
        grid.data[f] = vectors[i]
    for i, v in enumerate(vectors):
        if i not in perms[k]:
            v.free()
    grid.placement = {"staged": True, "tries": tries, "pool": len(vectors), "cycle_ms": [round(t, 3) for t in times], "chosen": k,
                      "chosen_ms": round(times[k], 3)}
    return grid.placement


def _init_test_kernel(params, grid):
    bs = params.block_size
    full = params.steps_ranges[Axis.X].full_domain
    gpos = (C.c_int64 * 2)(params.N_origin[0] - 1, params.N_origin[1] - 1)
    gN = (C.c_int64 * 2)(*params.global_grid)
    real = C.c_float if params.data_type == np.float32 else C.c_double
    origin = (real * 2)(*params.origin)
    dX = (real * 2)(params.cell_size(0), params.cell_size(1))
    bd = grid.block_data_ptrs()
    check(params.fn("init_test")(params.device.ctx, _range(params, full), params.test.tag,
                                   bs.size[0], bs.size[1], bs.ghosts, C.byref(gpos), C.byref(gN),
                                   C.byref(origin), C.byref(dX), params.test.r, C.byref(bd)))
    if getattr(params.test, "is_problem", False):
        from .problem import init_state
        init_state(params, grid)


def update_EOS(params, grid, axis=Axis.X):
    r = _range(params, params.steps_ranges[axis].EOS)
    p = grid.ptr
    if params.test.eos == "bizarrium":
        with _k(params, "bizarrium_EOS"):
            check(params.fn("bizarrium_EOS")(params.device.ctx, r, p("rho"), p("u"), p("v"), p("E"),
                                               p("p"), p("c"), p("g")))
    else:
        with _k(params, "perfect_gas_EOS"):
            check(params.fn("perfect_gas_EOS")(params.device.ctx, r, params.test.gamma, p("rho"), p("E"),
                                                 p("u"), p("v"), p("p"), p("c"), p("g")))


def boundary_conditions(params, grid, axis, side):
    bs = params.block_size
    uf, vf = params.test.boundary_condition(side)
    domain = bs.border_domain(side).to_c()
    incr = bs.stride_along(axis)
    if side in (Side.Left, Side.Bottom):
        incr = -incr
    p = grid.ptr
    check(params.fn("boundary_conditions")(params.device.ctx, domain, incr, bs.ghosts, uf, vf,
                                             p("rho"), p("u"), p("v"), p("p"), p("c"), p("g"), p("E")))


def block_ghost_exchange(params, grid, axis):
    remote = [s for s in sides_along(axis) if params.neighbours[s] != PROC_NULL]
    if remote:
        from .halo_exchange import exchange_sides
        exchange_sides(params, grid, axis, remote, COMM_VARS)
    for side in sides_along(axis):
        if params.neighbours[side] == PROC_NULL:
            boundary_conditions(params, grid, axis, side)


def numerical_fluxes(params, grid, axis, dt, dx):
    r = _range(params, params.steps_ranges[axis].fluxes)
    s = params.block_size.stride_along(axis)
    p = grid.ptr
    ua = p("u") if axis == Axis.X else p("v")
    if params.riemann_scheme == "GAD":
        with _k(params, "acoustic_GAD"):
            check(params.fn("acoustic_GAD")(params.device.ctx, r, s, dt, dx, p("us"), p("ps"), p("rho"), ua,
                                              p("p"), p("c"), LIMITERS[params.riemann_limiter]))
    else:
        with _k(params, "acoustic"):
            check(params.fn("acoustic")(params.device.ctx, r, s, p("us"), p("ps"), p("rho"), ua, p("p"), p("c")))


def cell_update(params, grid, axis, dt, dx):
    r = _range(params, params.steps_ranges[axis].cell_update)
    s = params.block_size.stride_along(axis)
    p = grid.ptr
    ua = p("u") if axis == Axis.X else p("v")
    with _k(params, "cell_update"):
        check(params.fn("cell_update")(params.device.ctx, r, s, dx, dt, p("us"), p("ps"), p("rho"), ua, p("E")))


def projection_remap(params, grid, axis, dt, dx):
    s = params.block_size.stride_along(axis)
    p = grid.ptr
    ra = _range(params, params.steps_ranges[axis].advection)
    w = (p("work_1"), p("work_2"), p("work_3"), p("work_4"))
    if params.projection_scheme == "euler_2nd":
        with _k(params, "advection_second_order"):
            check(params.fn("advection_second_order")(params.device.ctx, ra, s, dx, dt, p("us"), p("rho"),
                                                        p("u"), p("v"), p("E"), *w))
    else:
        with _k(params, "advection_first_order"):
            check(params.fn("advection_first_order")(params.device.ctx, ra, s, dt, p("us"), p("rho"),
                                                       p("u"), p("v"), p("E"), *w))
    rp = _range(params, params.steps_ranges[axis].projection)
    with _k(params, "euler_projection"):
        check(params.fn("euler_projection")(params.device.ctx, rp, s, dx, dt, p("us"), p("rho"), p("u"),
                                              p("v"), p("E"), *w))


def local_time_step(params, grid):
    r = _range(params, params.steps_ranges[Axis.X].real_domain)
    dx, dy = params.cell_size(0), params.cell_size(1)
    out = (C.c_float if params.data_type == np.float32 else C.c_double)()
    p = grid.ptr
    with _k(params, "dtCFL"):
        check(params.fn("dtCFL")(params.device.ctx, r, dx, dy, p("u"), p("v"), p("c"), C.byref(out)))
    return out.value


def conservation_vars(params, grid):
    r = _range(params, params.steps_ranges[Axis.X].real_domain)
    ds = params.cell_size(0) * params.cell_size(1)
    out = ((C.c_float if params.data_type == np.float32 else C.c_double) * 2)()
    check(params.fn("conservation_vars")(params.device.ctx, r, ds, grid.ptr("rho"), grid.ptr("E"), C.byref(out)))
    mass, energy = out[0], out[1]
    if params.use_MPI:
        from .halo_exchange import allreduce_sum
        mass, energy = allreduce_sum(params, (mass, energy))
    return mass, energy


def global_min(params, local_dt):
    if params.use_MPI:
        from .halo_exchange import allreduce_min
        return allreduce_min(params, local_dt)
    return local_dt



def sweep_lag(params):
    return 2 + (params.riemann_scheme == "GAD") + (params.projection_scheme == "euler_2nd")


def fused_sweep(params, grid, axis, dt, dx, emit_p=False, emit_c=False, emit_dt=False,
                out_range=None, dt_accumulate=False, swap=True, ctx=None, dt_out=None):
    d = sweep_desc(params, grid, axis, dt, dx, emit_p, emit_c, emit_dt, out_range, dt_accumulate)
    if emit_dt and dt_out is not None:
        d.dt_cfl_out = dt_out
    if ctx is not None:
        check(params.fn("sweep")(ctx, C.byref(d)))
    else:
        with _k(params, "sweep_x" if axis == Axis.X else "sweep_y"):
            check(params.fn("sweep")(params.device.ctx, C.byref(d)))
    if swap:
        grid.swap_state()


def sweep_desc(params, grid, axis, dt, dx, emit_p=False, emit_c=False, emit_dt=False, out_range=None,
               dt_accumulate=False):
    d = SweepDesc()
    d.axis = 0 if axis == Axis.X else 1
    d.scheme = SCHEMES[params.riemann_scheme]
    d.limiter = LIMITERS[params.riemann_limiter]
    d.projection = PROJECTIONS[params.projection_scheme]
    d.eos = 1 if params.test.eos == "bizarrium" else 0
    d.nghost = params.nghost
    lo, hi = first_side(axis), last_side(axis)
    d.bc_low = int(params.neighbours[lo] == PROC_NULL)
    d.bc_high = int(params.neighbours[hi] == PROC_NULL)
    d.exact = int(params.exact_arithmetic)
    d.x_kernel = int(getattr(params, "x_kernel", 0))
    d.nx, d.ny = params.N
    d.dt, d.dx, d.gamma = dt, dx, params.test.gamma
    d.u_factor_low, d.v_factor_low = params.test.boundary_condition(lo)
    d.u_factor_high, d.v_factor_high = params.test.boundary_condition(hi)
    d.rho_in, d.u_in, d.v_in, d.E_in = (grid.data[f].ptr for f in STATE_VARS)
    d.rho_out, d.u_out, d.v_out, d.E_out = (grid.alt[f].ptr for f in STATE_VARS)
    d.p_out = grid.data["p"].ptr if emit_p else None
    d.c_out = grid.data["c"].ptr if emit_c else None
    if emit_dt:
        d.dt_cfl_out = grid.dt_scalar.ptr
        d.cfl_dx = params.cell_size(0)
        d.cfl_dy = params.cell_size(1)
        d.dt_accumulate = int(dt_accumulate)
    if out_range is not None:
        d.out_lo, d.out_hi = out_range
    return d


def overlapped_sweep(tiles, link, axis, dt, dx, prefetched=None, **emit):
    p0 = tiles[0][0]
    lag = sweep_lag(p0)
    i_ax = int(axis) - 1
    handle = prefetched if prefetched is not None else link.start(sides_along(axis), STATE_VARS)
    late = []
    for k, (p, g) in enumerate(tiles):
        lo_r = p.neighbours[first_side(axis)] != PROC_NULL
        hi_r = p.neighbours[last_side(axis)] != PROC_NULL
        n = p.N[i_ax]
        if not (lo_r or hi_r):
            fused_sweep(p, g, axis, dt, dx, swap=False, **emit)
        elif n < 2 * lag + 1 or not p.overlap_halo:
            late.append((k, p, g, None))
        else:
            lo, hi = (lag if lo_r else 0), (n - lag if hi_r else n)
            fused_sweep(p, g, axis, dt, dx, out_range=(lo, hi), swap=False, **emit)
            late.append((k, p, g, ((0, lo), (hi, n))))
    on_edge = bool(late) and link.edges is not None and p0.edge_stream and all(strips is not None for *_, strips in late)
    if on_edge:
        link.finish_edge(handle)
    else:
        link.finish(handle)
    sz = np.dtype(p0.data_type).itemsize
    for k, p, g, strips in late:
        if strips is None:
            fused_sweep(p, g, axis, dt, dx, swap=False, **emit)
            continue
        for side, rng in enumerate(strips):
            if rng[0] == rng[1]:
                continue
            if on_edge:
                ctx, edge_dt = link.edges[k]
                fused_sweep(p, g, axis, dt, dx, out_range=rng, swap=False, ctx=ctx, dt_out=edge_dt + side * sz, **emit)
            else:
                fused_sweep(p, g, axis, dt, dx, out_range=rng, swap=False, dt_accumulate=True, **emit)
    if on_edge:
        link.edge_join(bool(emit.get("emit_dt")))
    for _, g in tiles:
        g.swap_state()


def rank_sweep(params, grid, axis, dt, dx, **emit):
    handle = None
    if grid.halo_prefetch is not None and grid.halo_prefetch[0] == axis:
        handle, grid.halo_prefetch = grid.halo_prefetch[1], None
    else:
        drain_halo(grid)
    overlapped_sweep([(params, grid)], grid.comm, axis, dt, dx, prefetched=handle, **emit)


def prefetch_halo(params, grid):
    if not (params.use_MPI and params.use_fused_sweep) or grid.comm is None or not params.overlap_halo:
        return
    axis = split_axes(params.axis_splitting, grid.global_dt.cycle + 1)[0][0]
    remote = [s for s in sides_along(axis) if params.neighbours[s] != PROC_NULL]
    if not remote or params.N[int(axis) - 1] < 2 * sweep_lag(params) + 1:
        return
    drain_halo(grid)
    grid.halo_prefetch = (axis, grid.comm.start(sides_along(axis), STATE_VARS))


def drain_halo(grid):
    if getattr(grid.comm, "native", False):
        grid.comm.drain()
    if grid.halo_prefetch is not None:
        grid.comm.finish(grid.halo_prefetch[1])
        grid.halo_prefetch = None



def next_time_step(params, grid):
    gdt = grid.global_dt
    if params.cst_dt:
        return
    gdt.update_dt(global_min(params, local_time_step(params, grid)))


DT_EVENT_SLOT = 1012


class DtReadback:

    def __init__(self, params):
        self.params, self.host, self.inflight = params, None, {}

    def landing(self):
        if self.host is None:
            self.host = self.params.device.pinned(2, self.params.data_type)
        return self.host

    def post(self, cycle, scalar):
        dev = self.params.device
        self.landing().copy_from_device_async(scalar, n=1, dst_offset=cycle & 1)
        dev.event_record(DT_EVENT_SLOT + (cycle & 1))
        self.inflight[cycle] = dev.ctx

    def take(self, cycle):
        check(self.params.device._L.armon_hip_event_sync(self.inflight.pop(cycle), DT_EVENT_SLOT + (cycle & 1)))
        return float(self.host.array[cycle & 1])

    def prime(self, cycle, value):
        dev = self.params.device
        self.landing().array[cycle & 1] = value
        dev.event_record(DT_EVENT_SLOT + (cycle & 1))
        self.inflight[cycle] = dev.ctx

    def free(self):
        if self.host is not None:
            self.host.free()
            self.host = None


def post_dt_readback(params, grid):
    if getattr(grid.comm, "stream_ordered", False):
        grid.comm.allreduce_min_device_async(grid.dt_scalar)
    grid.dt.post(grid.global_dt.cycle, grid.dt_scalar)


def take_dt_readback(params, grid, posted_in_cycle):
    local_dt = grid.dt.take(posted_in_cycle)
    if getattr(grid.comm, "stream_ordered", False):
        return local_dt
    return global_min(params, local_dt)


def native_cycle_usable(params):
    return params.use_fused_sweep and params.native_cycle and (not params.overlap_halo or params.edge_stream)


def _checkpoint(params, grid, label, axis=Axis.X):
    if not params.compare:
        return False
    from .io import step_checkpoint
    return step_checkpoint(params, grid, label, axis.name)


def solver_cycle(params, grid, last_cycle=True):
    gdt = grid.global_dt
    deferred = (gdt.cycle - 1) in grid.dt_inflight
    if gdt.cycle == 0:
        if _checkpoint(params, grid, "init_test"):
            return True
        update_EOS(params, grid)
        if _checkpoint(params, grid, "EOS_init"):
            return True
    if not deferred:
        next_time_step(params, grid)
        if params.use_fused_sweep and gdt.cycle == 0:
            grid.release_scratch()
    if _checkpoint(params, grid, "time_step"):
        return True
    if params.use_MPI and getattr(grid.comm, "native", False) and native_cycle_usable(params):
        grid.comm.native_cycle(gdt, last_cycle)
        return False
    sweeps = split_axes(params.axis_splitting, gdt.cycle)
    for k, (axis, dt_factor) in enumerate(sweeps):
        i_ax = int(axis) - 1
        dx = params.cell_size(i_ax)
        dt = gdt.current_dt * params.T(dt_factor)
        if params.use_fused_sweep:
            last = k == len(sweeps) - 1
            sweep = rank_sweep if params.use_MPI else fused_sweep
            sweep(params, grid, axis, dt, dx, emit_p=last and last_cycle, emit_dt=last and not params.cst_dt)
            if last and not last_cycle:
                prefetch_halo(params, grid)
            if last and not params.cst_dt:
                post_dt_readback(params, grid)
                if deferred:
                    gdt.update_dt(take_dt_readback(params, grid, gdt.cycle - 1))
        else:
            update_EOS(params, grid, axis)
            if _checkpoint(params, grid, "EOS", axis):
                return True
            block_ghost_exchange(params, grid, axis)
            if _checkpoint(params, grid, "boundary_conditions", axis):
                return True
            numerical_fluxes(params, grid, axis, dt, dx)
            if _checkpoint(params, grid, "numerical_fluxes", axis):
                return True
            cell_update(params, grid, axis, dt, dx)
            if _checkpoint(params, grid, "cell_update", axis):
                return True
            projection_remap(params, grid, axis, dt, dx)
            if _checkpoint(params, grid, "projection_remap", axis):
                return True
    return False


GRAPH_BATCH = 8
GRAPH_EVENT_SLOT = 1014


def graph_cycles_usable(params):
    if not (params.use_fused_sweep and params.graph_cycles):
        return False
    if params.checkpoint_step != 0 or params.checkpoint_at_end or params.restart_from is not None:
        return False
    if params.state_compare or params.compare_dir is not None:
        return False
    if params.state_profile:
        return False
    if params.exact_solution:
        return False
    if params.history_step != 0:
        return False
    if params.state_image:
        return False
    if params.use_MPI or any(n != PROC_NULL for n in params.neighbours.values()):
        return False
    if not params.device.owns_ctx:
        return False
    return params.silent > 1 and params.animation_step == 0 and not params.compare and not params.kernel_callbacks


def _graph_sweep_descs(params, grid, cycle_parity, state_ptr):
    descs = []
    sweeps = split_axes(params.axis_splitting, cycle_parity)
    for k, (axis, dt_factor) in enumerate(sweeps):
        last = k == len(sweeps) - 1
        d = sweep_desc(params, grid, axis, float(params.T(dt_factor)), params.cell_size(int(axis) - 1),
                       emit_p=last, emit_dt=last and not params.cst_dt)
        d.dt_state = state_ptr
        descs.append(d)
        grid.swap_state()
    return descs


def time_loop_graph(params, grid, _after_handover=None):
    dev, gdt, T = params.device, grid.global_dt, params.T
    gdt.reset()
    grid.dt_inflight.clear()
    params.wait()
    t1 = _time.perf_counter_ns()
    maxtime = T(params.maxtime)

    while gdt.time < maxtime and gdt.cycle < params.maxcycle and gdt.cycle < 2:
        if solver_cycle(params, grid, last_cycle=cycle_ends(params, gdt)):
            break
        gdt.next_cycle()
    n_parities = 1 if params.axis_splitting in ("Sequential", "X_only", "Y_only") else 2
    swaps_per_cycle = len(split_axes(params.axis_splitting, 0))
    if gdt.time < maxtime and gdt.cycle < params.maxcycle:
        L_prev = 0.0
        if not params.cst_dt:
            L_prev = take_dt_readback(params, grid, gdt.cycle - 1)
        auto = not params.cst_dt
        st = _lib.DtState(current_dt=float(gdt.current_dt), time=float(gdt.time), L_prev=float(L_prev), cycle=gdt.cycle,
                          done=0, invalid=0, emit_p=int(cycle_ends(params, gdt)), auto_step=int(auto), cst_dt=int(params.cst_dt),
                          maxcycle=params.maxcycle, cfl=float(params.cfl), maxtime=float(params.maxtime), Dt=float(params.Dt))
        state = dev.empty(C.sizeof(_lib.DtState) // 8, np.float64)
        host_state = dev.pinned(C.sizeof(_lib.DtState) // 8 * 2, np.float64)
        check(dev._L.armon_hip_memcpy(dev.ctx, C.c_void_p(state.ptr), C.byref(st), C.sizeof(st), 1))
        step = params.fn("dt_state_step")
        L_new = C.c_void_p(grid.dt_scalar.ptr)
        dummy = dev.empty(C.sizeof(_lib.DtState) // 8, np.float64)
        over = _lib.DtState(done=1)
        check(dev._L.armon_hip_memcpy(dev.ctx, C.c_void_p(dummy.ptr), C.byref(over), C.sizeof(over), 1))
        check(step(dev.ctx, C.c_void_p(dummy.ptr), L_new, float(params.cfl), float(params.maxtime), params.maxcycle,
                   int(params.cst_dt), float(params.Dt)))
        params.wait()
        dummy.free()

        def enqueue_cycle(parity):
            for d in _graph_sweep_descs(params, grid, parity, state.ptr):
                check(params.fn("sweep")(dev.ctx, C.byref(d)))
            if not auto:
                check(step(dev.ctx, C.c_void_p(state.ptr), L_new, float(params.cfl), float(params.maxtime), params.maxcycle,
                           int(params.cst_dt), float(params.Dt)))

        graphs, origin = {}, grid.data["rho"].ptr

        def launch_cycle(cycle):
            key = (cycle % n_parities, grid.data["rho"].ptr == origin)
            if key not in graphs:
                check(dev._L.armon_hip_graph_begin(dev.ctx))
                held, g = grid.data["rho"].ptr, C.c_void_p()
                try:
                    enqueue_cycle(cycle)
                except BaseException:
                    if dev._L.armon_hip_graph_end(dev.ctx, C.byref(g)) == 0 and g:
                        dev._L.armon_hip_graph_destroy(g)
                    if grid.data["rho"].ptr != held:
                        grid.swap_state()
                    raise
                check(dev._L.armon_hip_graph_end(dev.ctx, C.byref(g)))
                graphs[key] = g
                for _ in range(swaps_per_cycle):
                    grid.swap_state()
            check(dev._L.armon_hip_graph_launch(dev.ctx, graphs[key]))
            for _ in range(swaps_per_cycle):
                grid.swap_state()

        def read_state(slot):
            check(dev._L.armon_hip_memcpy_async(dev.ctx, C.c_void_p(host_state.ptr + slot * C.sizeof(_lib.DtState)),
                                               C.c_void_p(state.ptr), C.sizeof(_lib.DtState), 2))
            dev.event_record(GRAPH_EVENT_SLOT + slot)

        def state_at(slot):
            dev.event_sync(GRAPH_EVENT_SLOT + slot)
            return _lib.DtState.from_buffer_copy(bytes(host_state.array.view(np.uint8)[slot * C.sizeof(_lib.DtState):
                                                                                       (slot + 1) * C.sizeof(_lib.DtState)]))

        if _after_handover is not None:
            _after_handover(params, grid)
        cycle, batch, final = gdt.cycle, 0, None
        start_cycle, start_in_origin = gdt.cycle, grid.data["rho"].ptr == origin
        try:
            while final is None:
                for _ in range(GRAPH_BATCH):
                    launch_cycle(cycle)
                    cycle += 1
                read_state(batch & 1)
                if batch > 0:
                    prev = state_at((batch - 1) & 1)
                    if prev.done:
                        final = prev
                batch += 1
                if final is None and cycle - start_cycle > params.maxcycle + 2 * GRAPH_BATCH:
                    last = state_at((batch - 1) & 1)
                    if not last.done:
                        solver_error("time", f"the device-resident time loop did not finish within maxcycle = {params.maxcycle} "
                                             f"cycles (device state: cycle {last.cycle}, time {last.time}, dt {last.current_dt})")
                    final = last
            last = state_at((batch - 1) & 1)
            final = last if last.done else final
        except BaseException:
            params.wait()
            host_state.free()
            raise
        finally:
            params.wait()
            for g in graphs.values():
                dev._L.armon_hip_graph_destroy(g)
            state.free()
        if final.invalid:
            host_state.free()
            solver_error("time", f"Invalid time step for cycle {final.invalid_cycle}: {final.invalid_value}")
        ran = final.cycle - start_cycle
        in_origin = start_in_origin if (ran * swaps_per_cycle) % 2 == 0 else not start_in_origin
        if (grid.data["rho"].ptr == origin) != in_origin:
            grid.swap_state()
        gdt.cycle, gdt.time, gdt.current_dt = int(final.cycle), T(final.time), T(final.current_dt)
        grid.graph_report = {"graphs": len(graphs), "cycles_replayed": int(ran), "cycles_enqueued": cycle - start_cycle}
        host_state.free()
    params.wait()
    return report_run(params, gdt, _time.perf_counter_ns() - t1)


def cycle_ends(params, gdt):
    return (gdt.cycle + 1 >= params.maxcycle or (not params.cst_dt and gdt.current_dt == 0)
            or params.T(gdt.time + gdt.current_dt) >= params.T(params.maxtime))


def report_run(params, gdt, solve_time):
    cells = params.N[0] * params.N[1]
    grind_time = solve_time / max(gdt.cycle * cells, 1)
    if params.is_root and params.silent < 3:
        print(" ")
        print(f"Total time:  {solve_time / 1e9:.5f} sec")
        print(f"Grind time:  {grind_time / 1e3:.5f} µs/cell/cycle")
        print(f"Cells/sec:   {1 / grind_time * 1e3:.5f} Mega cells/sec")
        print(f"Cycles:      {gdt.cycle}")
        print(f"Last cycle:  {gdt.time:.18f} sec, Δt={gdt.current_dt:.18f} sec")
    return float(gdt.time), float(gdt.current_dt), gdt.cycle, 1 / grind_time, solve_time


def time_loop(params, grid):
    if graph_cycles_usable(params):
        return time_loop_graph(params, grid)
    grid.global_dt.reset()
    grid.dt_inflight.clear()
    gdt = grid.global_dt
    if params.restart_from is not None:
        grid.load_state(params.restart_from)
    if params.start_from_exact is not None:
        grid.fill_exact(time=params.start_from_exact, samples=params.error_norms_samples)
        gdt.time = params.T(params.start_from_exact)
        if params.check_result or params.silent <= 1:
            params.initial_mass, params.initial_energy = conservation_vars(params, grid)
    params.wait()
    t1 = _time.perf_counter_ns()
    maxtime = params.T(params.maxtime)
    saved_at, save_ns = -1, 0
    compared_at, stopped = -1, False
    grid.state_diffs = []
    profiled_at, grid.profiles = -1, []
    normed_at, grid.error_norms_taken = -1, []
    imaged_at, grid.images = -1, []
    hist, dt_used, grid.history = None, 0.0, None
    if params.history_step != 0:
        from .history import HistoryRun
        hist = HistoryRun(grid, params)
        hist.start(gdt)
    while gdt.time < maxtime and gdt.cycle < params.maxcycle:
        ends = cycle_ends(params, gdt)
        frame_due = params.animation_step != 0 and gdt.cycle % params.animation_step == 0
        if solver_cycle(params, grid, last_cycle=ends or frame_due):
            break
        dt_used = float(gdt.current_dt)
        gdt.next_cycle()
        if hist is not None and gdt.cycle % params.history_step == 0:
            hist.sample(gdt, dt_used)
        if frame_due:
            from .io import write_animation_frame
            params.wait()
            write_animation_frame(params, grid)
        if params.silent <= 1:
            params.wait()
            mass, energy = conservation_vars(params, grid)
            if params.is_root:
                dM = abs(params.initial_mass - mass) / params.initial_mass * 100
                dE = abs(params.initial_energy - energy) / params.initial_energy * 100
                print(f"Cycle {gdt.cycle:4d}: dt = {gdt.current_dt:.18f}, t = {gdt.time:.18f}, "
                      f"|ΔM| = {dM:#8.6g}%, |ΔE| = {dE:#8.6g}%")
        if params.checkpoint_step != 0 and gdt.cycle % params.checkpoint_step == 0:
            from .checkpoint import checkpoint_path
            if hist is not None:
                hist.flush()
# ... 95 lines not shown
```

### include/armon_hip.h

```cpp
#ifndef ARMON_HIP_H
#define ARMON_HIP_H

#include <stddef.h>
#include <stdint.h>

#if defined(ARMON_BUILDING_LIB)
#define ARMON_API __attribute__((visibility("default")))
#else
#define ARMON_API
#endif

#ifdef __cplusplus
extern "C" {
#endif

typedef enum {
    ARMON_OK = 0,
    ARMON_ERR_INVALID_ARG = 1,
    ARMON_ERR_HIP = 2,
    ARMON_ERR_NO_DEVICE = 3,
    ARMON_ERR_INVALID_DT = 4
} armon_status;

enum { ARMON_LIMITER_NONE = 0, ARMON_LIMITER_MINMOD = 1, ARMON_LIMITER_SUPERBEE = 2 };
// ... 240 lines not shown

ARMON_API int armon_hip_exact_fill(armon_ctx*, int64_t row_length, int nghost, int64_t nx, int64_t ny,
        double* rho, double* u, double* v, double* E, int64_t col0, int64_t row0, int64_t wnx,
        int64_t wny, int64_t global_col0, int64_t global_row0, const armon_exact_spec* spec);
ARMON_API int armon_hip_exact_fill_f32(armon_ctx*, int64_t row_length, int nghost, int64_t nx, int64_t ny,
        float* rho, float* u, float* v, float* E, int64_t col0, int64_t row0, int64_t wnx,
        int64_t wny, int64_t global_col0, int64_t global_row0, const armon_exact_spec* spec);

enum { ARMON_HISTORY_RHO_MIN = 0, ARMON_HISTORY_RHO_MAX = 1, ARMON_HISTORY_P_MIN = 2, ARMON_HISTORY_P_MAX = 3,
       ARMON_HISTORY_E_MIN = 4, ARMON_HISTORY_E_MAX = 5, ARMON_HISTORY_Q2_MAX = 6, ARMON_HISTORY_MACH2_MAX = 7 };
typedef struct {
    uint64_t n;
    uint64_t n_bad;
    int64_t  sum[6][3];
    uint64_t ext[8][2];
    uint64_t reserved[4];
} armon_history_record;
typedef struct {
    int32_t eos, reserved;
    double  gamma;
    int64_t global_nx;
    int32_t scale_exp[6];
} armon_history_spec;
#define ARMON_HISTORY_MAX_GAUGES 64
typedef struct armon_history armon_history;

ARMON_API int armon_hip_history_create(armon_ctx*, int capacity, int max_gauges, armon_history** out);
ARMON_API int armon_hip_history_destroy(armon_ctx*, armon_history*);
ARMON_API int armon_hip_history_set_gauges(armon_ctx*, armon_history*, const int64_t* cells, int n);

ARMON_API int armon_hip_history_sample(armon_ctx*, armon_history*, int slot, const armon_history_spec* spec, int64_t row_length,
        int nghost, int64_t nx, int64_t ny, const double* rho, const double* u, const double* v, const double* E, int64_t col0,
        int64_t row0, int64_t wnx, int64_t wny, int64_t global_col0, int64_t global_row0);
ARMON_API int armon_hip_history_sample_f32(armon_ctx*, armon_history*, int slot, const armon_history_spec* spec, int64_t row_length,
        int nghost, int64_t nx, int64_t ny, const float* rho, const float* u, const float* v, const float* E, int64_t col0,
        int64_t row0, int64_t wnx, int64_t wny, int64_t global_col0, int64_t global_row0);

ARMON_API int armon_hip_history_read(armon_ctx*, armon_history*, int first_slot, int count, armon_history_record* records_host,
        double* gauges_host);

typedef struct {
    float *x, *y, *rho, *u, *v, *E, *p, *c, *g, *us, *ps, *work_1, *work_2, *work_3, *work_4, *mask;
} armon_block_data_f32;

ARMON_API int armon_hip_perfect_gas_EOS_f32(armon_ctx*, armon_range, float gamma,
        const float* rho, const float* E, const float* u, const float* v, float* p, float* c, float* g);
ARMON_API int armon_hip_bizarrium_EOS_f32(armon_ctx*, armon_range,
        const float* rho, const float* u, const float* v, const float* E, float* p, float* c, float* g);
ARMON_API int armon_hip_acoustic_f32(armon_ctx*, armon_range, int64_t s, float* us, float* ps,
        const float* rho, const float* ua, const float* p, const float* c);
ARMON_API int armon_hip_acoustic_GAD_f32(armon_ctx*, armon_range, int64_t s, float dt, float dx, float* us, float* ps,
        const float* rho, const float* ua, const float* p, const float* c, int limiter);
ARMON_API int armon_hip_cell_update_f32(armon_ctx*, armon_range, int64_t s, float dx, float dt,
        const float* us, const float* ps, float* rho, float* ua, float* E);
ARMON_API int armon_hip_advection_first_order_f32(armon_ctx*, armon_range, int64_t s, float dt,
        const float* us, const float* rho, const float* u, const float* v, const float* E,
        float* adv_rho, float* adv_urho, float* adv_vrho, float* adv_Erho);
ARMON_API int armon_hip_advection_second_order_f32(armon_ctx*, armon_range, int64_t s, float dx, float dt,
        const float* us, const float* rho, const float* u, const float* v, const float* E,
        float* adv_rho, float* adv_urho, float* adv_vrho, float* adv_Erho);
ARMON_API int armon_hip_euler_projection_f32(armon_ctx*, armon_range, int64_t s, float dx, float dt,
        const float* us, float* rho, float* u, float* v, float* E,
        const float* adv_rho, const float* adv_urho, const float* adv_vrho, const float* adv_Erho);
ARMON_API int armon_hip_boundary_conditions_f32(armon_ctx*, armon_range, int64_t incr, int nghost,
        float u_factor, float v_factor, float* rho, float* u, float* v, float* p, float* c, float* g, float* E);
ARMON_API int armon_hip_pack_to_array_f32(armon_ctx*, armon_range, int nghost, int64_t face,
        float* array, int nvars, const float* const* vars);
ARMON_API int armon_hip_unpack_from_array_f32(armon_ctx*, armon_range, int nghost, int64_t face,
        const float* array, int nvars, float* const* vars);
ARMON_API int armon_hip_dtCFL_async_f32(armon_ctx*, armon_range, float dx, float dy,
        const float* u, const float* v, const float* c, float* result_dev);
ARMON_API int armon_hip_dtCFL_f32(armon_ctx*, armon_range, float dx, float dy,
        const float* u, const float* v, const float* c, float* result_host);
ARMON_API int armon_hip_conservation_vars_f32(armon_ctx*, armon_range, float ds,
        const float* rho, const float* E, float out_host[2]);
ARMON_API int armon_hip_init_test_f32(armon_ctx*, armon_range, int test, int64_t row_length, int64_t col_length,
        int nghost, const int64_t global_pos[2], const int64_t global_N[2],
        const float origin[2], const float dX[2], float sedov_r, const armon_block_data_f32* data);
ARMON_API int armon_hip_coarsen_f32(armon_ctx*, int64_t row_length, int nghost, int64_t nx, int64_t ny, int64_t fx, int64_t fy,
        const float* rho, const float* u, const float* v, const float* E, const float* p, float* out_dev);
ARMON_API int armon_hip_derive_f32(armon_ctx*, int64_t row_length, int nghost, int64_t nx, int64_t ny, int64_t fx, int64_t fy,
        const float* rho, const float* u, const float* v, const float* E, const armon_derive_spec* spec, float* out_dev);
ARMON_API int armon_hip_gather_strided_f32(armon_ctx*, int64_t n_cells, int nvars, const float* const* vars,
        int64_t start, int64_t stride, int64_t count, float* out_dev);
ARMON_API int armon_hip_state_pack_f32(armon_ctx*, int64_t row_length, int nghost, int64_t nx, int64_t ny, int nvars,
        const float* const* vars, int64_t col0, int64_t row0, int64_t wnx, int64_t wny, int64_t global_first,
        int64_t global_nx, float* dense_dev, uint64_t* digest_dev);
ARMON_API int armon_hip_state_unpack_f32(armon_ctx*, int64_t row_length, int nghost, int64_t nx, int64_t ny, int nvars,
        float* const* vars, int64_t col0, int64_t row0, int64_t wnx, int64_t wny, int64_t global_first,
        int64_t global_nx, const float* dense_dev, uint64_t* digest_dev);
ARMON_API int armon_hip_plane_encode_f32(armon_ctx*, const float* dense_dev, int nplanes, int64_t rows, int64_t wnx,
        void* out_dev, uint64_t plane_capacity, uint64_t* sizes_dev);
ARMON_API int armon_hip_plane_decode_f32(armon_ctx*, const void* chunk_dev, uint64_t chunk_bytes, int64_t rows, int64_t wnx,
        int64_t col0, int64_t row0, int64_t snx, int64_t sny, float* out_dev, uint32_t* status_dev);

struct armon_dt_state;
typedef struct {
    int32_t axis;
    int32_t scheme;
    int32_t limiter;
    int32_t projection;
    int32_t eos;
    int32_t nghost;
    int32_t bc_low, bc_high;
    int32_t exact;
    int32_t x_kernel;
    int64_t nx, ny;
    double  dt, dx;
    double  gamma;
    double  u_factor_low, v_factor_low, u_factor_high, v_factor_high;
    const double *rho_in, *u_in, *v_in, *E_in;
    double *rho_out, *u_out, *v_out, *E_out;
    double *p_out;
    double *c_out;
    double *dt_cfl_out;
    double  cfl_dx, cfl_dy;
    int64_t out_lo, out_hi;
    int32_t dt_accumulate;
    int32_t reserved;
    struct armon_dt_state* dt_state;
} armon_sweep_desc;

ARMON_API int armon_hip_sweep(armon_ctx*, const armon_sweep_desc*);

typedef struct armon_dt_state {
    double  current_dt;
    double  time;
    double  L_prev;
    int64_t cycle;
    int32_t done;
    int32_t invalid;
    int32_t emit_p;
    int32_t pad;
    int64_t invalid_cycle;
    double  invalid_value;
    int32_t auto_step, cst_dt;
    int64_t maxcycle;
    double  cfl, maxtime, Dt;
} armon_dt_state;

ARMON_API int armon_hip_dt_state_step(armon_ctx*, armon_dt_state* state_dev, const double* L_new_dev, double cfl,
                                      double maxtime, int64_t maxcycle, int cst_dt, double Dt);
ARMON_API int armon_hip_dt_state_step_f32(armon_ctx*, armon_dt_state* state_dev, const float* L_new_dev, double cfl,
                                          double maxtime, int64_t maxcycle, int cst_dt, double Dt);

typedef struct armon_graph armon_graph;
ARMON_API int armon_hip_graph_begin(armon_ctx*);
ARMON_API int armon_hip_graph_end(armon_ctx*, armon_graph** graph);
ARMON_API int armon_hip_graph_launch(armon_ctx*, armon_graph* graph);
ARMON_API int armon_hip_graph_destroy(armon_graph* graph);

ARMON_API int armon_hip_cycle_xy(armon_ctx*, const armon_sweep_desc* x_desc, const armon_sweep_desc* y_desc);

ARMON_API int armon_hip_tune_placement(armon_ctx*, const armon_sweep_desc* x_desc, const armon_sweep_desc* y_desc,
        void* const* pool, int n_pool, size_t bytes, int tries, int picks[8], double* times_ms);

ARMON_API int armon_hip_choose_placement(armon_ctx*, const armon_sweep_desc* x_desc, const armon_sweep_desc* y_desc,
        void* const* pool, int n_pool, size_t bytes, int tries, double tolerance, int picks[8], double* times_ms,
        int* tries_done);

typedef struct {
    int32_t axis, scheme, limiter, projection, eos, nghost;
    int32_t bc_low, bc_high;
    int32_t exact, x_kernel;
    int64_t nx, ny;
    double  dt, dx, gamma;
    double  u_factor_low, v_factor_low, u_factor_high, v_factor_high;
    const float *rho_in, *u_in, *v_in, *E_in;
    float *rho_out, *u_out, *v_out, *E_out;
    float *p_out, *c_out;
    float *dt_cfl_out;
    double  cfl_dx, cfl_dy;
    int64_t out_lo, out_hi;
    int32_t dt_accumulate, reserved;
    struct armon_dt_state* dt_state;
} armon_sweep_desc_f32;

ARMON_API int armon_hip_sweep_f32(armon_ctx*, const armon_sweep_desc_f32*);
ARMON_API int armon_hip_tune_placement_f32(armon_ctx*, const armon_sweep_desc_f32* x_desc, const armon_sweep_desc_f32* y_desc,
        void* const* pool, int n_pool, size_t bytes, int tries, int picks[8], double* times_ms);
ARMON_API int armon_hip_choose_placement_f32(armon_ctx*, const armon_sweep_desc_f32* x_desc, const armon_sweep_desc_f32* y_desc,
        void* const* pool, int n_pool, size_t bytes, int tries, double tolerance, int picks[8], double* times_ms,
        int* tries_done);


typedef struct armon_mgpu armon_mgpu;
#define ARMON_MGPU_ID_BYTES 256

ARMON_API int armon_hip_mgpu_init(int px, int py, const int* device_ids, armon_mgpu** group);
ARMON_API int armon_hip_mgpu_unique_id(void* id);
ARMON_API int armon_hip_mgpu_init_rank(int px, int py, int rank, int device_id, void* stream, const void* id,
                                       armon_mgpu** group);
ARMON_API int armon_hip_mgpu_prepare_rank(int px, int py, int rank, int device_id, void* stream, armon_mgpu** group);
ARMON_API int armon_hip_mgpu_connect(armon_mgpu* group, const void* id);
ARMON_API int armon_hip_mgpu_destroy(armon_mgpu* group);
ARMON_API int armon_hip_mgpu_set_periodic(armon_mgpu* group, int periodic_x, int periodic_y);
ARMON_API int armon_hip_mgpu_force_peer_copy(armon_mgpu* group, int on);
ARMON_API int armon_hip_mgpu_set_chaos(armon_mgpu* group, unsigned max_delay_us, uint64_t seed);
ARMON_API int armon_hip_mgpu_n_local(armon_mgpu* group);
ARMON_API armon_ctx* armon_hip_mgpu_ctx(armon_mgpu* group, int local_tile);
ARMON_API int armon_hip_mgpu_tile_info(armon_mgpu* group, int local_tile, int* rank, int coords[2], int neighbours[4]);

typedef struct {
    int64_t nx, ny;
    int32_t nghost, nvars;
    void*   vars[8];
} armon_halo_desc;

ARMON_API int armon_hip_halo_exchange_start(armon_mgpu*, int axis, const armon_halo_desc* tiles);
ARMON_API int armon_hip_halo_exchange_finish(armon_mgpu*, int axis, const armon_halo_desc* tiles);
ARMON_API int armon_hip_halo_exchange(armon_mgpu*, int axis, const armon_halo_desc* tiles);
ARMON_API int armon_hip_halo_exchange_start_f32(armon_mgpu*, int axis, const armon_halo_desc* tiles);
ARMON_API int armon_hip_halo_exchange_finish_f32(armon_mgpu*, int axis, const armon_halo_desc* tiles);
ARMON_API int armon_hip_halo_exchange_f32(armon_mgpu*, int axis, const armon_halo_desc* tiles);

ARMON_API armon_ctx* armon_hip_mgpu_edge_ctx(armon_mgpu* group, int local_tile);
ARMON_API void* armon_hip_mgpu_edge_dt(armon_mgpu* group, int local_tile);
ARMON_API int armon_hip_halo_exchange_finish_edge(armon_mgpu*, int axis, const armon_halo_desc* tiles);
ARMON_API int armon_hip_halo_exchange_finish_edge_f32(armon_mgpu*, int axis, const armon_halo_desc* tiles);
ARMON_API int armon_hip_mgpu_edge_join(armon_mgpu*, double* const* dt_dev);
ARMON_API int armon_hip_mgpu_edge_join_f32(armon_mgpu*, float* const* dt_dev);

ARMON_API int armon_hip_dt_allreduce(armon_mgpu*, double* const* dt_dev);
ARMON_API int armon_hip_dt_allreduce_f32(armon_mgpu*, float* const* dt_dev);

typedef struct {
    int32_t n_sweeps, emit_p, emit_dt, overlap;
    int32_t axis[4];
    double  dt[4];
    int32_t next_axis, event_slot;
    armon_ctx* event_ctx;
    void*   dt_host;
    int32_t dt_event_slot;
    int32_t reserved;
} armon_cycle_plan;
typedef struct { armon_sweep_desc x, y; } armon_tile_cycle;
typedef struct { armon_sweep_desc_f32 x, y; } armon_tile_cycle_f32;
ARMON_API int armon_hip_mgpu_cycle(armon_mgpu*, const armon_cycle_plan* plan, const armon_tile_cycle* tiles);
ARMON_API int armon_hip_mgpu_cycle_f32(armon_mgpu*, const armon_cycle_plan* plan, const armon_tile_cycle_f32* tiles);
ARMON_API int armon_hip_mgpu_drain(armon_mgpu*, const armon_tile_cycle* tiles);
ARMON_API int armon_hip_mgpu_drain_f32(armon_mgpu*, const armon_tile_cycle_f32* tiles);
ARMON_API int armon_hip_mgpu_sync(armon_mgpu*);
ARMON_API int armon_hip_mgpu_set_threads(armon_mgpu*, int on);

ARMON_API int armon_hip_mgpu_allreduce_host(armon_mgpu*, int op, int count, double* values);

ARMON_API int armon_hip_halo_ranges(int64_t nx, int64_t ny, int nghost, int side, armon_range* border,
                                    armon_range* ghost, int64_t* face);

#ifdef __cplusplus
}
#endif
#endif
```

Baseline: 96860 Mcells/s.

## Pad intermediate X-sweep output to cache-line pitch and add nontemporal Y loads

Adds a paired X+Y sweep path where the X sweep writes its intermediate state with rows padded to a 128-byte line pitch and the Y sweep reads that padded layout. The aim is aligned row starts for the Y sweep's strided column access, which lets a nontemporal buffer-load variant of the Y kernel be used. State arrays get extra capacity for the padding, and placement tuning and graph capture now go through the pair. The cost is extra memory plus more host-side plumbing with several conditions under which the pair path is taken.

```diff
diff --git a/armon.jl_amd/_lib.py b/armon.jl_amd/_lib.py
--- a/armon.jl_amd/_lib.py
+++ b/armon.jl_amd/_lib.py
@@ -217,6 +217,8 @@
     "armon_hip_tune_placement": (_ci, [_vp, C.POINTER(SweepDesc), C.POINTER(SweepDesc), C.POINTER(_vp), _ci,
                                        C.c_size_t, _ci, C.POINTER(_ci * 8), C.POINTER(_dbl)]),
     "armon_hip_cycle_xy": (_ci, [_vp, C.POINTER(SweepDesc), C.POINTER(SweepDesc)]),
+    "armon_hip_sweep_pair_pitch": (C.c_int64, [C.c_int64, _ci]),
+    "armon_hip_sweep_pair": (_ci, [_vp, C.POINTER(SweepDesc), C.POINTER(SweepDesc), C.c_size_t]),
     "armon_hip_choose_placement": (_ci, [_vp, C.POINTER(SweepDesc), C.POINTER(SweepDesc), C.POINTER(_vp), _ci,
                                          C.c_size_t, _ci, _dbl, C.POINTER(_ci * 8), C.POINTER(_dbl), C.POINTER(_ci)]),
     "armon_hip_mgpu_init": (_ci, [_ci, _ci, C.POINTER(_ci), C.POINTER(_vp)]),
@@ -284,13 +286,15 @@
 _add_f32_signatures()
 
 
-def load_at(path):
+def load_at(path, missing_ok=()):
     if not os.path.exists(path):
         raise RuntimeError(
             f"{path} is missing: build it with `python armon.jl_amd/build.py` "
             "(there is no CPU fallback for the device backend)")
     L = C.CDLL(path)
     for name, (res, args) in SIGNATURES.items():
+        if name in missing_ok and not hasattr(L, name):
+            continue
         fn = getattr(L, name)
         fn.restype = res
         fn.argtypes = args
diff --git a/armon.jl_amd/blocking.py b/armon.jl_amd/blocking.py
--- a/armon.jl_amd/blocking.py
+++ b/armon.jl_amd/blocking.py
@@ -125,6 +125,14 @@
         return Range(self.col.first - 1, self.col.step, len(self.col), self.row.first - 1, len(self.row))
 
 
+LINE_BYTES = 128
+
+
+def line_pitch(nx, nghost, itemsize=8):
+    per_line = LINE_BYTES // itemsize
+    return -(-(nx + 2 * nghost) // per_line) * per_line
+
+
 @dataclass(frozen=True)
 class BlockSize:
     size: tuple
@@ -137,6 +145,12 @@
     @property
     def n_cells(self):
         return self.size[0] * self.size[1]
+
+    def line_pitch(self, itemsize=8):
+        return line_pitch(self.real_size[0], self.ghosts, itemsize)
+
+    def line_cells(self, itemsize=8):
+        return self.line_pitch(itemsize) * self.size[1]
 
     def domain_range(self, bottom_left=(0, 0), top_right=(0, 0)):
         g, row = self.ghosts, self.size[0]
diff --git a/armon.jl_amd/csrc/common.hpp b/armon.jl_amd/csrc/common.hpp
--- a/armon.jl_amd/csrc/common.hpp
+++ b/armon.jl_amd/csrc/common.hpp
@@ -29,6 +29,8 @@
     int tune_x_rows = 0;
     int tune_copy_nt = 0;
     int tune_y_sx = 0;
+    int tune_y_nt = 0;
+    int tune_pair_only = 0;
     int tune_profile_wgs = 0;
     int64_t seg_nx = -1, seg_ny = -1;
     int seg_lag = -1, seg_cols = -1, seg_value = 0;
diff --git a/armon.jl_amd/csrc/context.hip b/armon.jl_amd/csrc/context.hip
--- a/armon.jl_amd/csrc/context.hip
+++ b/armon.jl_amd/csrc/context.hip
@@ -93,7 +93,7 @@
     }
     int rc = ensure_partials(ctx, 8192);
     if (rc != ARMON_OK) { armon_hip_destroy(ctx); return rc; }
-    for (const char* knob : {"ARMON_XS_NITER", "ARMON_Y_SEG", "ARMON_SWEEP_ALIGN", "ARMON_Y_COLS1", "ARMON_X_XCD", "ARMON_X_ROWS", "ARMON_Y_SX", "ARMON_COPY_NT"}) {
+    for (const char* knob : {"ARMON_XS_NITER", "ARMON_Y_SEG", "ARMON_SWEEP_ALIGN", "ARMON_Y_COLS1", "ARMON_X_XCD", "ARMON_X_ROWS", "ARMON_Y_SX", "ARMON_Y_NT", "ARMON_COPY_NT"}) {
         const char* v = getenv(knob);
         if (v && *v) (void)armon_hip_set_tuning(ctx, knob, atoi(v));
     }
@@ -111,6 +111,8 @@
     else if (!strcmp(knob, "ARMON_X_XCD")) ctx->tune_x_xcd = value < 0 ? -1 : (value > 0);
     else if (!strcmp(knob, "ARMON_X_ROWS")) ctx->tune_x_rows = (value == 1 || value == 2) ? value : 0;
     else if (!strcmp(knob, "ARMON_Y_SX")) ctx->tune_y_sx = (value == 1 || value == 2) ? value : 0;
+    else if (!strcmp(knob, "ARMON_Y_NT")) ctx->tune_y_nt = value == 2 ? 2 : 0;
+    else if (!strcmp(knob, "ARMON_PAIR_ONLY")) ctx->tune_pair_only = (value == 1 || value == 2) ? value : 0;
     else if (!strcmp(knob, "ARMON_COPY_NT")) ctx->tune_copy_nt = value & 3;
     else if (!strcmp(knob, "PROFILE_WGS")) ctx->tune_profile_wgs = value > 0 ? value : 0;
     else ARMON_REQUIRE(false, "unknown tuning knob '%s'", knob);
@@ -127,6 +129,8 @@
     else if (!strcmp(knob, "ARMON_X_XCD")) *value = ctx->tune_x_xcd;
     else if (!strcmp(knob, "ARMON_X_ROWS")) *value = ctx->tune_x_rows;
     else if (!strcmp(knob, "ARMON_Y_SX")) *value = ctx->tune_y_sx;
+    else if (!strcmp(knob, "ARMON_Y_NT")) *value = ctx->tune_y_nt;
+    else if (!strcmp(knob, "ARMON_PAIR_ONLY")) *value = ctx->tune_pair_only;
     else if (!strcmp(knob, "ARMON_COPY_NT")) *value = ctx->tune_copy_nt;
     else if (!strcmp(knob, "PROFILE_WGS")) *value = ctx->tune_profile_wgs;
     else if (!strcmp(knob, "Y_RUN_ROWS")) *value = ctx->tune_y_seg > 0 ? ctx->tune_y_seg : ctx->seg_value;
diff --git a/armon.jl_amd/csrc/fused_sweep.hpp b/armon.jl_amd/csrc/fused_sweep.hpp
--- a/armon.jl_amd/csrc/fused_sweep.hpp
+++ b/armon.jl_amd/csrc/fused_sweep.hpp
@@ -13,18 +13,23 @@
     int cols = 1;
     int block = kYBlock;
     bool sx = false;
+    bool nt = false;
 };
-y_shape y_launch_shape(const armon_ctx* ctx, const ARMON_SWEEP_DESC* d)
+y_shape y_launch_shape(const armon_ctx* ctx, const ARMON_SWEEP_DESC* d, int64_t in_len, int64_t out_len)
 {
     y_shape s;
     if (std::is_same<real, float>::value && !d->exact && d->nx % 2 == 0 && d->nghost % 2 == 0 && d->nx >= 2 && !ctx->tune_y_cols1)
         s.cols = 2;
     if (ctx->tune_align != 0 && ctx->tune_y_sx != 2 && !d->exact) {
         const uintptr_t outs = (uintptr_t)d->rho_out | (uintptr_t)d->u_out | (uintptr_t)d->v_out | (uintptr_t)d->E_out;
-        const int64_t row_len = d->nx + 2 * (int64_t)d->nghost;
-        s.sx = outs % 64 == 0 && ((row_len * (int64_t)sizeof(real)) % 64 != 0 || ctx->tune_y_sx == 1);
+        s.sx = outs % 64 == 0 && ((out_len * (int64_t)sizeof(real)) % 64 != 0 || ctx->tune_y_sx == 1);
     }
     s.block = s.sx ? kYSxBlock : kYBlock;
+    {
+        const uintptr_t ins = (uintptr_t)d->rho_in | (uintptr_t)d->u_in | (uintptr_t)d->v_in | (uintptr_t)d->E_in;
+        s.nt = ctx->tune_align != 0 && ctx->tune_y_nt != 2 && s.cols == 1 && !s.sx && ins % 128 == 0 &&
+               (in_len * (int64_t)sizeof(real)) % 128 == 0;
+    }
     return s;
 }
 
@@ -49,6 +54,12 @@
             if (ys.sx) {
                 hipLaunchKernelGGL((k_sweep_y<PIPE, TRACK, kYSxBlock, true>), grid, dim3(ys.block), 0, ctx->stream, a);
                 return check_launch("sweep_y (store exchange)");
+            }
+        }
+        if constexpr (y_nt_loads(PIPE::EOS, PIPE::kExact)) {
+            if (ys.nt) {
+                hipLaunchKernelGGL((k_sweep_y<PIPE, TRACK, kYBlock, false, 1, true>), grid, dim3(ys.block), 0, ctx->stream, a);
+                return check_launch("sweep_y (nt loads)");
             }
         }
         hipLaunchKernelGGL((k_sweep_y<PIPE, TRACK>), grid, dim3(ys.block), 0, ctx->stream, a);
@@ -178,7 +189,7 @@
 
 }
 
-extern "C" int ARMON_SWEEP_FN(armon_ctx* ctx, const ARMON_SWEEP_DESC* d)
+static int sweep_pitched(armon_ctx* ctx, const ARMON_SWEEP_DESC* d, int64_t in_len, int64_t out_len)
 {
     ARMON_REQUIRE(ctx && d, "NULL argument");
     ARMON_REQUIRE(d->axis == ARMON_AXIS_X || d->axis == ARMON_AXIS_Y, "invalid axis %d", d->axis);
@@ -218,7 +229,8 @@
     sweep_args a;
     a.nx = d->nx;
     a.ny = d->ny;
-    a.row_len = d->nx + 2 * (int64_t)d->nghost;
+    a.row_len = in_len;
+    a.out_len = out_len;
     a.g = d->nghost;
     a.bc_low = d->bc_low;
     a.bc_high = d->bc_high;
@@ -245,7 +257,7 @@
     a.c_out = d->c_out;
     a.st = d->dt_state;
     const bool align = ctx->tune_align != 0;
-    const y_shape ys = X ? y_shape{} : y_launch_shape(ctx, d);
+    const y_shape ys = X ? y_shape{} : y_launch_shape(ctx, d, in_len, out_len);
     a.y_sx = ys.sx;
     if (X) {
         a.seg = 512;
@@ -261,7 +273,7 @@
         }
         a.seg = ctx->seg_value;
     }
-    ARMON_REQUIRE(X || a.row_len * (int64_t)sizeof(real) * (a.seg + 2 * lag + 16) < (1ll << 32),
+    ARMON_REQUIRE(X || (in_len > out_len ? in_len : out_len) * (int64_t)sizeof(real) * (a.seg + 2 * lag + 16) < (1ll << 32),
                   "block too wide for 32-bit row offsets (%lld cells per row, runs of %d rows)", (long long)d->nx, a.seg);
     a.x_kernel = d->x_kernel;
     a.o_lo = 0;
@@ -284,7 +296,7 @@
         const uintptr_t bases = (uintptr_t)d->rho_in | (uintptr_t)d->u_in | (uintptr_t)d->v_in | (uintptr_t)d->E_in |
                                 (uintptr_t)d->rho_out | (uintptr_t)d->u_out | (uintptr_t)d->v_out | (uintptr_t)d->E_out |
                                 (uintptr_t)d->p_out | (uintptr_t)d->c_out;
-        a.x_row_align = X && align && d->x_kernel == 0 && ctx->tune_xs_niter <= 1 && a.row_len % (64 / (int64_t)sizeof(real)) != 0 &&
+        a.x_row_align = X && align && d->x_kernel == 0 && ctx->tune_xs_niter <= 1 && a.out_len % (64 / (int64_t)sizeof(real)) != 0 &&
                         bases % 64 == 0;
     }
 #endif
@@ -327,6 +339,45 @@
 #endif
 }
 
+extern "C" int ARMON_SWEEP_FN(armon_ctx* ctx, const ARMON_SWEEP_DESC* d)
+{
+    ARMON_REQUIRE(ctx && d, "NULL argument");
+    const int64_t pitch = d->nx + 2 * (int64_t)d->nghost;
+    return sweep_pitched(ctx, d, pitch, pitch);
+}
+
+#ifdef ARMON_PAIR_FN
+extern "C" int64_t ARMON_PAIR_PITCH_FN(int64_t nx, int nghost)
+{
+    const int64_t line = 128 / (int64_t)sizeof(real);
+    return (nx + 2 * (int64_t)nghost + line - 1) / line * line;
+}
+
+extern "C" int ARMON_PAIR_FN(armon_ctx* ctx, const ARMON_SWEEP_DESC* x, const ARMON_SWEEP_DESC* y, size_t mid_bytes)
+{
+    ARMON_REQUIRE(ctx && x && y, "NULL argument");
+    ARMON_REQUIRE(x->axis == ARMON_AXIS_X && y->axis == ARMON_AXIS_Y, "the pair is an X sweep followed by a Y sweep");
+    ARMON_REQUIRE(x->nx == y->nx && x->ny == y->ny && x->nghost == y->nghost && x->nx > 0 && x->ny > 0 && x->nghost >= 0,
+                  "the two descriptors describe different blocks");
+    ARMON_REQUIRE(x->rho_out == y->rho_in && x->u_out == y->u_in && x->v_out == y->v_in && x->E_out == y->E_in && x->rho_out,
+                  "the Y sweep must read the arrays the X sweep writes");
+    ARMON_REQUIRE(y->bc_low && y->bc_high, "a block with a remote Y side cannot use the pair (its ghost rows come from a neighbour)");
+    ARMON_REQUIRE(x->out_hi == 0 && y->out_hi == 0, "the pair runs whole sweeps");
+    ARMON_REQUIRE(!x->p_out && !x->c_out && !x->dt_cfl_out, "the X sweep of the pair has no output of its own");
+    ARMON_REQUIRE(x->x_kernel == 0, "x_kernel form %d cannot write the intermediate layout", x->x_kernel);
+    const int64_t pitch = x->nx + 2 * (int64_t)x->nghost, mid = ARMON_PAIR_PITCH_FN(x->nx, x->nghost);
+    ARMON_REQUIRE((uint64_t)mid_bytes >= (uint64_t)(mid * (x->ny + 2 * (int64_t)x->nghost)) * sizeof(real),
+                  "the intermediate arrays hold %zu bytes, rows of %lld cells need %lld", mid_bytes, (long long)mid,
+                  (long long)(mid * (x->ny + 2 * (int64_t)x->nghost) * (int64_t)sizeof(real)));
+    if (ctx->tune_pair_only != 2) {
+        const int rc = sweep_pitched(ctx, x, pitch, mid);
+        if (rc != ARMON_OK) return rc;
+    }
+    if (ctx->tune_pair_only != 1) return sweep_pitched(ctx, y, mid, pitch);
+    return ARMON_OK;
+}
+#endif
+
 #if defined(ARMON_CYCLE_FN) && !defined(ARMON_ALT_KERNELS)
 extern "C" int ARMON_CYCLE_FN(armon_ctx* ctx, const ARMON_SWEEP_DESC* x, const ARMON_SWEEP_DESC* y)
 {
diff --git a/armon.jl_amd/csrc/fused_sweep_f64.hip b/armon.jl_amd/csrc/fused_sweep_f64.hip
--- a/armon.jl_amd/csrc/fused_sweep_f64.hip
+++ b/armon.jl_amd/csrc/fused_sweep_f64.hip
@@ -2,4 +2,6 @@
 #define ARMON_SWEEP_FN armon_hip_sweep
 #define ARMON_SWEEP_DESC armon_sweep_desc
 #define ARMON_CYCLE_FN armon_hip_cycle_xy
+#define ARMON_PAIR_FN armon_hip_sweep_pair
+#define ARMON_PAIR_PITCH_FN armon_hip_sweep_pair_pitch
 #include "fused_sweep.hpp"
diff --git a/armon.jl_amd/csrc/placement.hip b/armon.jl_amd/csrc/placement.hip
--- a/armon.jl_amd/csrc/placement.hip
+++ b/armon.jl_amd/csrc/placement.hip
@@ -14,6 +14,28 @@
     const size_t i = (size_t)blockIdx.x * 256 + threadIdx.x;
     if (i < n) p[i] = value;
 }
+
+struct cycle_f64 {
+    size_t bytes;
+    int operator()(armon_ctx* ctx, const armon_sweep_desc* x, const armon_sweep_desc* y) const
+    {
+        const int64_t rows = x->ny + 2 * (int64_t)x->nghost;
+        const bool pair = x->axis == ARMON_AXIS_X && y->axis == ARMON_AXIS_Y && x->nx == y->nx && x->ny == y->ny &&
+                          x->nghost == y->nghost && x->nx > 0 && x->ny > 0 && x->nghost >= 0 && y->bc_low && y->bc_high &&
+                          x->out_hi == 0 && y->out_hi == 0 && !x->p_out && !x->c_out && !x->dt_cfl_out && x->x_kernel == 0 &&
+                          (uint64_t)bytes >= (uint64_t)(armon_hip_sweep_pair_pitch(x->nx, x->nghost) * rows) * sizeof(double);
+        if (pair) return armon_hip_sweep_pair(ctx, x, y, bytes);
+        const int rc = armon_hip_sweep(ctx, x);
+        return rc == ARMON_OK ? armon_hip_sweep(ctx, y) : rc;
+    }
+};
+struct cycle_f32 {
+    int operator()(armon_ctx* ctx, const armon_sweep_desc_f32* x, const armon_sweep_desc_f32* y) const
+    {
+        const int rc = armon_hip_sweep_f32(ctx, x);
+        return rc == ARMON_OK ? armon_hip_sweep_f32(ctx, y) : rc;
+    }
+};
 
 template <class DESC, class SWEEP, class PREPARE, class STOP>
 int placement_search(armon_ctx* ctx, SWEEP sweep, const DESC* x_desc, const DESC* y_desc, void* const* pool, int n_pool,
@@ -51,8 +73,7 @@
         double ms_min = 1e300;
         for (int rep = 0; rep < 3; rep++) {
             PLACEMENT_TRY(hipEventRecord(e0, ctx->stream));
-            rc = sweep(ctx, &dx);
-            if (rc == ARMON_OK) rc = sweep(ctx, &dy);
+            rc = sweep(ctx, &dx, &dy);
             if (rc != ARMON_OK) { cleanup(); return rc; }
             PLACEMENT_TRY(hipEventRecord(e1, ctx->stream));
             PLACEMENT_TRY(hipEventSynchronize(e1));
@@ -155,20 +176,20 @@
 extern "C" int armon_hip_tune_placement(armon_ctx* ctx, const armon_sweep_desc* x_desc, const armon_sweep_desc* y_desc,
                                         void* const* pool, int n_pool, size_t bytes, int tries, int* picks, double* times_ms)
 {
-    return tune_placement(ctx, armon_hip_sweep, x_desc, y_desc, pool, n_pool, bytes, tries, picks, times_ms);
+    return tune_placement(ctx, cycle_f64{bytes}, x_desc, y_desc, pool, n_pool, bytes, tries, picks, times_ms);
 }
 
 extern "C" int armon_hip_tune_placement_f32(armon_ctx* ctx, const armon_sweep_desc_f32* x_desc, const armon_sweep_desc_f32* y_desc,
                                             void* const* pool, int n_pool, size_t bytes, int tries, int* picks, double* times_ms)
 {
-    return tune_placement(ctx, armon_hip_sweep_f32, x_desc, y_desc, pool, n_pool, bytes, tries, picks, times_ms);
+    return tune_placement(ctx, cycle_f32{}, x_desc, y_desc, pool, n_pool, bytes, tries, picks, times_ms);
 }
 
 extern "C" int armon_hip_choose_placement(armon_ctx* ctx, const armon_sweep_desc* x_desc, const armon_sweep_desc* y_desc,
                                           void* const* pool, int n_pool, size_t bytes, int tries, double tolerance, int* picks,
                                           double* times_ms, int* tries_done)
 {
-    return choose_placement<double>(ctx, armon_hip_sweep, x_desc, y_desc, pool, n_pool, bytes, tries, tolerance, picks, times_ms,
+    return choose_placement<double>(ctx, cycle_f64{bytes}, x_desc, y_desc, pool, n_pool, bytes, tries, tolerance, picks, times_ms,
                                     tries_done);
 }
 
@@ -176,6 +197,6 @@
                                               void* const* pool, int n_pool, size_t bytes, int tries, double tolerance, int* picks,
                                               double* times_ms, int* tries_done)
 {
-    return choose_placement<float>(ctx, armon_hip_sweep_f32, x_desc, y_desc, pool, n_pool, bytes, tries, tolerance, picks,
+    return choose_placement<float>(ctx, cycle_f32{}, x_desc, y_desc, pool, n_pool, bytes, tries, tolerance, picks,
                                    times_ms, tries_done);
 }
diff --git a/armon.jl_amd/csrc/sweep_device.hpp b/armon.jl_amd/csrc/sweep_device.hpp
--- a/armon.jl_amd/csrc/sweep_device.hpp
+++ b/armon.jl_amd/csrc/sweep_device.hpp
@@ -54,6 +54,7 @@
 
 struct sweep_args {
     int64_t nx, ny, row_len;
+    int64_t out_len;
     int32_t g;
     int32_t bc_low, bc_high;
     int32_t emit;
@@ -135,6 +136,11 @@
     const v2u v = __builtin_amdgcn_raw_buffer_load_b64(r, voff, soff, kAuxLoad);
     return __builtin_bit_cast(double, v);
 }
+__device__ __forceinline__ double buf_load_nt(rsrc_t r, unsigned voff, unsigned soff)
+{
+    const v2u v = __builtin_amdgcn_raw_buffer_load_b64(r, voff, soff, kAuxLoad | 2);
+    return __builtin_bit_cast(double, v);
+}
 template <>
 __device__ __forceinline__ float buf_load<float>(rsrc_t r, unsigned voff, unsigned soff)
 {
diff --git a/armon.jl_amd/csrc/sweep_x_kernel.hpp b/armon.jl_amd/csrc/sweep_x_kernel.hpp
--- a/armon.jl_amd/csrc/sweep_x_kernel.hpp
+++ b/armon.jl_amd/csrc/sweep_x_kernel.hpp
@@ -40,14 +40,17 @@
                                   : ((int64_t)vby * kXSRows + threadIdx.y) * RW + (ROW ? (threadIdx.x >> 4) : 0);
     const bool row_ok = row_r < a.ny;
     const int64_t row = row_ok ? row_r : a.ny - 1;
-    const int64_t row_off = (row + a.g) * a.row_len + a.g;
-    const real* in[4] = {a.rho_in + row_off, a.ua_in + row_off, a.ut_in + row_off, a.E_in + row_off};
+    const int64_t row_in = (row + a.g) * a.row_len + a.g;
+    const int64_t row_off = (row + a.g) * a.out_len + a.g;
+    const real* in[4] = {a.rho_in + row_in, a.ua_in + row_in, a.ut_in + row_in, a.E_in + row_in};
     real* out[4] = {a.rho_out + row_off, a.ua_out + row_off, a.ut_out + row_off, a.E_out + row_off};
-    bool vec_ok = (K == 2) && (a.row_len % 2 == 0) && ((a.x_first + a.g) % 2 == 0);
+    bool vec_ok = (K == 2) && (a.out_len % 2 == 0) && ((a.x_first + a.g) % 2 == 0);
+    bool vec_in = (K == 2) && (a.row_len % 2 == 0) && ((a.x_first + a.g) % 2 == 0);
     int64_t x_first = a.x_first;
     if (ROW == 0 && a.x_row_align) {
         x_first = a.o_lo - __builtin_amdgcn_readfirstlane((int)(row_off + a.o_lo) & (64 / (int)sizeof(real) - 1));
         vec_ok = (K == 2);
+        vec_in = (K == 2) && __builtin_amdgcn_readfirstlane((int)(row_in + x_first) & 1) == 0;
     }
 
     SW sw{a.dt, a.dx, a.gamma, a.inv_dx, a.dt_dx};
@@ -63,7 +66,7 @@
         const int64_t cb = w_first + (int64_t)it * STRIDE - HALO;
         const int64_t j0 = cb + (int64_t)lane * K;
         const bool interior = cb >= 0 && cb + WIDTH <= a.nx;
-        if (interior && (K == 1 || vec_ok)) {
+        if (interior && (K == 1 || vec_in)) {
             if (K == 2) {
                 constexpr bool NT = x_nt_loads(EOS, EXACT);
                 const vec2 r = ld2<NT>(in[0] + j0);
@@ -173,7 +176,7 @@
 __device__ __forceinline__ void preload_x_args(const sweep_args& a, int niter)
 {
 #if ARMON_X_PRELOAD
-    asm volatile("" ::"s"(a.nx), "s"(a.ny), "s"(a.row_len), "s"(a.g), "s"(a.bc_low), "s"(a.bc_high), "s"(a.emit), "s"(a.o_lo),
+    asm volatile("" ::"s"(a.nx), "s"(a.ny), "s"(a.row_len), "s"(a.out_len), "s"(a.g), "s"(a.bc_low), "s"(a.bc_high), "s"(a.emit), "s"(a.o_lo),
                  "s"(a.o_hi), "s"(a.x_first), "s"(a.xcd_remap), "s"(a.x_wg_along_x), "s"(a.x_row_align), "s"(niter), "s"(a.gx), "s"(a.gy));
     asm volatile("" ::"s"(a.dt), "s"(a.dx), "s"(a.gamma), "s"(a.inv_dx), "s"(a.dt_dx), "s"(a.rho_in), "s"(a.ua_in), "s"(a.ut_in),
                  "s"(a.E_in), "s"(a.rho_out), "s"(a.ua_out), "s"(a.ut_out), "s"(a.E_out));
diff --git a/armon.jl_amd/csrc/sweep_y_kernel.hpp b/armon.jl_amd/csrc/sweep_y_kernel.hpp
--- a/armon.jl_amd/csrc/sweep_y_kernel.hpp
+++ b/armon.jl_amd/csrc/sweep_y_kernel.hpp
@@ -23,7 +23,12 @@
     using V = real;
     using pipe_t = PIPE;
     using lds_t = real;
-    static __device__ __forceinline__ V load(rsrc_t r, unsigned voff, unsigned soff) { return buf_load<real>(r, voff, soff); }
+    template <bool NT = false>
+    static __device__ __forceinline__ V load(rsrc_t r, unsigned voff, unsigned soff)
+    {
+        if constexpr (NT && std::is_same<real, double>::value) return buf_load_nt(r, voff, soff);
+        else return buf_load<real>(r, voff, soff);
+    }
     static __device__ __forceinline__ void store(rsrc_t r, unsigned voff, unsigned soff, V v) { buf_store(r, voff, soff, v); }
     static __device__ __forceinline__ void track(cfl_track& t, const V& u, const V& v, const V& c) { t.add(u, v, c); }
 };
@@ -40,7 +45,15 @@
     }
 };
 
-template <class PIPE, bool TRACK, int BLOCK = kYBlock, bool SX = false, int COLS = 1>
+constexpr bool y_nt_loads(int eos, bool exact)
+{
+#ifdef ARMON_Y_NT_ALL
+    return sizeof(real) == 8;
+#endif
+    return sizeof(real) == 8 && eos == ARMON_EOS_PERFECT_GAS && !exact;
+}
+
+template <class PIPE, bool TRACK, int BLOCK = kYBlock, bool SX = false, int COLS = 1, bool NTL = false>
 __global__ void __launch_bounds__(BLOCK, ARMON_Y_WAVES)
 k_sweep_y(sweep_args a)
 {
@@ -59,8 +72,8 @@
     const int jb = o0 - LAG, je = o1 + LAG;
 
     const unsigned colb = (unsigned)(x + g) * (unsigned)sizeof(real);
-    const unsigned pitchb = (unsigned)a.row_len * (unsigned)sizeof(real);
-    const int64_t in_base = (int64_t)(jb + g) * a.row_len, out_base = (int64_t)(o0 + g) * a.row_len;
+    const unsigned pitchb = (unsigned)a.row_len * (unsigned)sizeof(real), opitchb = (unsigned)a.out_len * (unsigned)sizeof(real);
+    const int64_t in_base = (int64_t)(jb + g) * a.row_len, out_base = (int64_t)(o0 + g) * a.out_len;
     const rsrc_t r_rho = make_rsrc(a.rho_in + in_base), r_ua = make_rsrc(a.ua_in + in_base);
     const rsrc_t r_ut = make_rsrc(a.ut_in + in_base), r_E = make_rsrc(a.E_in + in_base);
     const rsrc_t w_rho = make_rsrc(a.rho_out + out_base), w_ua = make_rsrc(a.ua_out + out_base);
@@ -71,14 +84,15 @@
 
     int lj = jb;
     unsigned lo_off = 0;
-    unsigned so_off = (unsigned)(jb - LAG - o0) * pitchb;
+    unsigned so_off = (unsigned)(jb - LAG - o0) * opitchb;
 
     __shared__ typename lane_t::lds_t sx_lds[SX ? 2 : 1][SX ? 4 : 1][SX ? BLOCK : 1];
     static_assert((BLOCK & (BLOCK - 1)) == 0, "the store exchange wraps columns with a mask");
+    static_assert(!NTL || (COLS == 1 && !SX), "non-temporal row loads: the one-column march without the store exchange");
     constexpr int kSec = 64 / (COLS * (int)sizeof(real));
     const int c0 = (int)(blockIdx.x * BLOCK) * COLS - a.xshift;
-    int sx_r = (int)((((int64_t)(jb - LAG + g) * a.row_len + g + c0) >> (COLS - 1)) & (kSec - 1));
-    const int sx_dr = (int)((a.row_len >> (COLS - 1)) & (kSec - 1));
+    int sx_r = (int)((((int64_t)(jb - LAG + g) * a.out_len + g + c0) >> (COLS - 1)) & (kSec - 1));
+    const int sx_dr = (int)((a.out_len >> (COLS - 1)) & (kSec - 1));
     int sx_buf = 0;
 
     auto load = [&](auto slot, auto checked) {
@@ -119,19 +133,19 @@
                 const unsigned off = (unsigned)(src - jb) * pitchb;
                 const real fa = m_lo ? a.fa_low : (m_hi ? a.fa_high : real(1));
                 const real ft = m_lo ? a.ft_low : (m_hi ? a.ft_high : real(1));
-                dst.rho = lane_t::load(r_rho, colb, off);
-                dst.ua = lane_t::load(r_ua, colb, off) * fa;
-                dst.ut = lane_t::load(r_ut, colb, off) * ft;
-                dst.E = lane_t::load(r_E, colb, off);
+                dst.rho = lane_t::template load<NTL>(r_rho, colb, off);
+                dst.ua = lane_t::template load<NTL>(r_ua, colb, off) * fa;
+                dst.ut = lane_t::template load<NTL>(r_ut, colb, off) * ft;
+                dst.E = lane_t::template load<NTL>(r_E, colb, off);
                 if (lj + 1 < je) {
                     lj++;
                     lo_off += pitchb;
                 }
             } else {
-                dst.rho = lane_t::load(r_rho, colb, lo_off);
-                dst.ua = lane_t::load(r_ua, colb, lo_off);
-                dst.ut = lane_t::load(r_ut, colb, lo_off);
-                dst.E = lane_t::load(r_E, colb, lo_off);
+                dst.rho = lane_t::template load<NTL>(r_rho, colb, lo_off);
+                dst.ua = lane_t::template load<NTL>(r_ua, colb, lo_off);
+                dst.ut = lane_t::template load<NTL>(r_ut, colb, lo_off);
+                dst.E = lane_t::template load<NTL>(r_E, colb, lo_off);
                 lj++;
                 lo_off += pitchb;
             }
@@ -159,7 +173,7 @@
         const int o = j - LAG;
         if (CHECKED) {
             if (a.emit && j >= o0 && j < o1 && active) {
-                const unsigned off = so_off + LAG * pitchb;
+                const unsigned off = so_off + LAG * opitchb;
                 if (a.emit & 1) lane_t::store(make_rsrc(a.p_out + out_base), colb, off, p);
                 if (a.emit & 2) lane_t::store(make_rsrc(a.c_out + out_base), colb, off, c);
             }
@@ -205,7 +219,7 @@
             }
             if (TRACK) lane_t::track(cfl, out.ut, out.ua, c_lag);
         }
-        so_off += pitchb;
+        so_off += opitchb;
         sx_r = (sx_r + sx_dr) & (kSec - 1);
     };
     auto run = [&](auto checked, int t0, int t1) {
diff --git a/armon.jl_amd/device.py b/armon.jl_amd/device.py
--- a/armon.jl_amd/device.py
+++ b/armon.jl_amd/device.py
@@ -91,8 +91,8 @@
         check(self._L.armon_hip_event_elapsed_ms(self.ctx, int(a), int(b), C.byref(ms)))
         return ms.value
 
-    def empty(self, n, dtype=np.float64):
-        return DeviceArray(self, n, dtype)
+    def empty(self, n, dtype=np.float64, capacity=None):
+        return DeviceArray(self, n, dtype, capacity)
 
     def zeros(self, n, dtype=np.float64):
         a = DeviceArray(self, n, dtype)
@@ -108,13 +108,14 @@
 
 class DeviceArray:
 
-    def __init__(self, device, n, dtype=np.float64):
+    def __init__(self, device, n, dtype=np.float64, capacity=None):
         self.device = device
         self.n = int(n)
         self.dtype = np.dtype(dtype)
         self.nbytes = self.n * self.dtype.itemsize
+        self._capacity_bytes = max(self.n, int(capacity or 0)) * self.dtype.itemsize
         p = C.c_void_p()
-        check(device._L.armon_hip_malloc(device.ctx, self.nbytes, C.byref(p)))
+        check(device._L.armon_hip_malloc(device.ctx, self.capacity_bytes, C.byref(p)))
         self.ptr = p.value or 0
 
     @classmethod
@@ -131,6 +132,10 @@
         return self.n
 
     @property
+    def capacity_bytes(self):
+        return getattr(self, "_capacity_bytes", self.nbytes)
+
+    @property
     def __cuda_array_interface__(self):
         return {"shape": (self.n,), "typestr": self.dtype.str, "data": (self.ptr, False), "version": 2}
 
diff --git a/armon.jl_amd/solver.py b/armon.jl_amd/solver.py
--- a/armon.jl_amd/solver.py
+++ b/armon.jl_amd/solver.py
@@ -106,7 +106,8 @@
         import weakref
         self._grid_ref = weakref.ref(grid)
         for f in names:
-            self[f] = grid.params.device.empty(grid.size.n_cells, grid.params.data_type)
+            self[f] = grid.params.device.empty(grid.size.n_cells, grid.params.data_type,
+                                               capacity=grid.pair_cells if f in STATE_VARS else None)
 
     def __missing__(self, key):
         if key not in FIELDS:
@@ -124,6 +125,13 @@
         return a
 
 
+def pair_usable(params):
+    return bool(params.use_fused_sweep and np.dtype(params.data_type).itemsize == 8 and params.axis_splitting == "Sequential"
+                and not params.use_MPI and all(n == PROC_NULL for n in params.neighbours.values())
+                and int(getattr(params, "x_kernel", 0)) == 0
+                and params.block_size.n_cells * np.dtype(params.data_type).itemsize >= params.placement_min_bytes)
+
+
 class BlockGrid:
 
     def __init__(self, params):
@@ -134,8 +142,9 @@
         dt_ = params.data_type
         self.initialised = False
         self.lazy = set()
+        self.pair_cells = self.size.line_cells(np.dtype(dt_).itemsize) if pair_usable(params) else None
         self.data = _Fields(self, FUSED_FIELDS if params.use_fused_sweep else FIELDS)
-        self.alt = {f: dev.empty(n, dt_) for f in STATE_VARS} if params.use_fused_sweep else None
+        self.alt = {f: dev.empty(n, dt_, capacity=self.pair_cells) for f in STATE_VARS} if params.use_fused_sweep else None
         self.placement = None
         self.global_dt = GlobalTimeStep(params)
         self.dt_scalar = dev.zeros(2, dt_)
@@ -189,9 +198,11 @@
         dt = 1e-3 * dx
         n, dt_ = self.data["rho"].n, self.data["rho"].dtype
         pool = [self.data[f] for f in STATE_VARS] + [self.alt[f] for f in STATE_VARS]
+        cap = min(v.capacity_bytes for v in pool) // dt_.itemsize
+        cap_bytes = cap * dt_.itemsize
         try:
             for _ in range(spare):
-                pool.append(dev.empty(n, dt_))
+                pool.append(dev.empty(n, dt_, capacity=cap))
         except _lib.SolverException:
             for v in pool[8:]:
                 v.free()
@@ -209,10 +220,10 @@
             picks, times, done = (C.c_int * 8)(), (C.c_double * tries)(), C.c_int(tries)
             try:
                 if keep_state:
-                    check(params.fn("tune_placement")(dev.ctx, C.byref(d_x), C.byref(d_y), ptrs, len(pool), nbytes, tries,
+                    check(params.fn("tune_placement")(dev.ctx, C.byref(d_x), C.byref(d_y), ptrs, len(pool), cap_bytes, tries,
                                                       C.byref(picks), times))
                 else:
-                    check(params.fn("choose_placement")(dev.ctx, C.byref(d_x), C.byref(d_y), ptrs, len(pool), nbytes,
+                    check(params.fn("choose_placement")(dev.ctx, C.byref(d_x), C.byref(d_y), ptrs, len(pool), cap_bytes,
                                                         tries, 0.004, C.byref(picks), times, C.byref(done)))
             except _lib.SolverException:
                 for k, f in enumerate(STATE_VARS):
@@ -230,7 +241,7 @@
             if free < (spare + 2) * nbytes:
                 break
             try:
-                pool = best + [dev.empty(n, dt_) for _ in range(spare)]
+                pool = best + [dev.empty(n, dt_, capacity=cap) for _ in range(spare)]
             except _lib.SolverException:
                 break
         for k, f in enumerate(STATE_VARS):
@@ -358,7 +369,8 @@
 
     def memory_required(self):
         n = self.size.n_cells * np.dtype(self.params.data_type).itemsize
-        return n * (len(self.data) + (4 if self.alt else 0))
+        pad = sum(v.capacity_bytes - v.nbytes for v in list(self.data.values()) + (list(self.alt.values()) if self.alt else []))
+        return n * (len(self.data) + (4 if self.alt else 0)) + pad
 
 
 
@@ -589,6 +601,16 @@
         grid.swap_state()
 
 
+def pair_cycle(params, grid):
+    return (grid.pair_cells is not None and not params.kernel_callbacks and pair_usable(params)
+            and min(grid.alt[f].capacity_bytes for f in STATE_VARS) >= grid.pair_cells * np.dtype(params.data_type).itemsize)
+
+
+def fused_pair(params, grid, d_x, d_y):
+    mid = min(v.capacity_bytes for v in list(grid.alt.values()) + [grid.data[f] for f in STATE_VARS])
+    check(params.fn("sweep_pair")(params.device.ctx, C.byref(d_x), C.byref(d_y), mid))
+
+
 def sweep_desc(params, grid, axis, dt, dx, emit_p=False, emit_c=False, emit_dt=False, out_range=None,
                dt_accumulate=False):
     d = SweepDesc()
@@ -777,6 +799,19 @@
         grid.comm.native_cycle(gdt, last_cycle)
         return False
     sweeps = split_axes(params.axis_splitting, gdt.cycle)
+    if params.use_fused_sweep and pair_cycle(params, grid):
+        dt = gdt.current_dt
+        d_x = sweep_desc(params, grid, Axis.X, dt * params.T(sweeps[0][1]), params.cell_size(0))
+        grid.swap_state()
+        d_y = sweep_desc(params, grid, Axis.Y, dt * params.T(sweeps[1][1]), params.cell_size(1), emit_p=last_cycle,
+                         emit_dt=not params.cst_dt)
+        grid.swap_state()
+        fused_pair(params, grid, d_x, d_y)
+        if not params.cst_dt:
+            post_dt_readback(params, grid)
+            if deferred:
+                gdt.update_dt(take_dt_readback(params, grid, gdt.cycle - 1))
+        return False
     for k, (axis, dt_factor) in enumerate(sweeps):
         i_ax = int(axis) - 1
         dx = params.cell_size(i_ax)
@@ -885,8 +920,12 @@
         dummy.free()
 
         def enqueue_cycle(parity):
-            for d in _graph_sweep_descs(params, grid, parity, state.ptr):
-                check(params.fn("sweep")(dev.ctx, C.byref(d)))
+            descs = _graph_sweep_descs(params, grid, parity, state.ptr)
+            if pair_cycle(params, grid):
+                fused_pair(params, grid, *descs)
+            else:
+                for d in descs:
+                    check(params.fn("sweep")(dev.ctx, C.byref(d)))
             if not auto:
                 check(step(dev.ctx, C.c_void_p(state.ptr), L_new, float(params.cfl), float(params.maxtime), params.maxcycle,
                            int(params.cst_dt), float(params.Dt)))
diff --git a/include/armon_hip.h b/include/armon_hip.h
--- a/include/armon_hip.h
+++ b/include/armon_hip.h
@@ -416,6 +416,9 @@
 
 ARMON_API int armon_hip_cycle_xy(armon_ctx*, const armon_sweep_desc* x_desc, const armon_sweep_desc* y_desc);
 
+ARMON_API int64_t armon_hip_sweep_pair_pitch(int64_t nx, int nghost);
+ARMON_API int armon_hip_sweep_pair(armon_ctx*, const armon_sweep_desc* x_desc, const armon_sweep_desc* y_desc, size_t mid_bytes);
+
 ARMON_API int armon_hip_tune_placement(armon_ctx*, const armon_sweep_desc* x_desc, const armon_sweep_desc* y_desc,
         void* const* pool, int n_pool, size_t bytes, int tries, int picks[8], double* times_ms);
 
```

Result: faster. 97850 Mcells/s, median of 6 (+1.0%).
